# aurianer/DLA-Future

Measured on AMD Instinct MI355X. Metric: fp64 Cholesky TFlop/s, higher is better.
Workload: dtype f64

## Files before the change

### dla_future_amd/__init__.py

```python
from .capi import (DLAFDescriptor, LibraryNotBuilt, lib, lib_path, type_char, version)
from .cholesky import (DeviceMatrix, GeneralDeviceMatrix, Grid, cholesky_factorization, finalize, generalized_to_standard,
                       initialize, make_descriptor, potrf_trace, pxhegst, pxpotrf, pxpotrs, pxtrsm, set_random_hermitian_positive_definite, tile_gemm, tile_herk, tile_potrf,
                       tile_trsm, triangular_solver, triangular_solver_device, potrs_device, release_workspace_pool, solver_profile,
                       update_launch_stats)
from . import distribution
from .eigensolver import (band_to_tridiagonal, bt_band_to_tridiagonal, bt_reduction_to_band,
                          bt_reduction_to_band_device, eigensolver_min_band, eigensolver_profile, get_band_size, hermitian_eigensolver,
                          hermitian_generalized_eigensolver, red2band_panel_stats, red2band_profile, reduction_to_band,
                          reduction_to_band_device, tridiagonal_eigensolver)

__all__ = ["band_to_tridiagonal", "bt_band_to_tridiagonal", "eigensolver_profile", "hermitian_eigensolver",
           "hermitian_generalized_eigensolver", "tridiagonal_eigensolver", "bt_reduction_to_band", "bt_reduction_to_band_device", "get_band_size", "eigensolver_min_band", "red2band_profile",
           "reduction_to_band", "reduction_to_band_device", "DLAFDescriptor", "DeviceMatrix", "GeneralDeviceMatrix", "Grid", "LibraryNotBuilt", "cholesky_factorization", "distribution",
           "finalize", "generalized_to_standard", "initialize", "lib", "lib_path", "make_descriptor", "pxhegst", "pxpotrf", "pxpotrs", "pxtrsm",
           "set_random_hermitian_positive_definite", "solver_profile", "tile_gemm", "tile_herk", "tile_potrf", "tile_trsm",
           "triangular_solver", "triangular_solver_device", "potrs_device", "type_char", "version"]
```

### dla_future_amd/capi.py

```python
from __future__ import annotations

import ctypes as C
import os

import numpy as np

_HERE = os.path.dirname(os.path.abspath(__file__))


class LibraryNotBuilt(RuntimeError):
    pass


def lib_path() -> str:
    return os.environ.get("DLAF_MI355X_LIB") or os.path.join(_HERE, "lib", "libdlaf_mi355x.so")


class DLAFDescriptor(C.Structure):
    _fields_ = [("m", C.c_int), ("n", C.c_int), ("mb", C.c_int), ("nb", C.c_int), ("isrc", C.c_int),
                ("jsrc", C.c_int), ("i", C.c_int), ("j", C.c_int), ("ld", C.c_int)]


BCAST_FN = C.CFUNCTYPE(C.c_int, C.c_void_p, C.c_int, C.c_int, C.c_void_p, C.c_size_t)
BARRIER_FN = C.CFUNCTYPE(C.c_int, C.c_void_p)

_TYPE_CHARS = {np.dtype(np.float32): "s", np.dtype(np.float64): "d", np.dtype(np.complex64): "c",
               np.dtype(np.complex128): "z"}


def type_char(dtype) -> str:
    try:
        return _TYPE_CHARS[np.dtype(dtype)]
    except KeyError:
        raise TypeError(f"unsupported element type {dtype}: expected float32/64 or complex64/128") from None


_vp, _i, _l, _ch = C.c_void_p, C.c_int, C.c_long, C.c_char
_IP = C.POINTER(C.c_int)
SIGNATURES = {
    "dlaf_initialize": (None, [_i, C.POINTER(C.c_char_p), _i, C.POINTER(C.c_char_p)]),
    "dlaf_finalize": (None, []),
    "dlaf_free_grid": (None, [_i]),
    "make_dlaf_descriptor": (DLAFDescriptor, [_i, _i, _i, _i, _IP]),
    "dlaf_cholesky_factorization_s": (_i, [_i, _ch, _vp, DLAFDescriptor]),
    "dlaf_cholesky_factorization_d": (_i, [_i, _ch, _vp, DLAFDescriptor]),
    "dlaf_cholesky_factorization_c": (_i, [_i, _ch, _vp, DLAFDescriptor]),
    "dlaf_cholesky_factorization_z": (_i, [_i, _ch, _vp, DLAFDescriptor]),
    "dlaf_pspotrf": (None, [_ch, _i, _vp, _i, _i, _IP, _IP]),
    "dlaf_pdpotrf": (None, [_ch, _i, _vp, _i, _i, _IP, _IP]),
    "dlaf_pcpotrf": (None, [_ch, _i, _vp, _i, _i, _IP, _IP]),
    "dlaf_pzpotrf": (None, [_ch, _i, _vp, _i, _i, _IP, _IP]),
    "dlaf_mi355x_version": (C.c_char_p, []),
    "dlaf_mi355x_create_grid_single": (_i, []),
    "dlaf_mi355x_rccl_unique_id": (None, [_vp]),
    "dlaf_mi355x_create_grid_rccl": (_i, [_vp, _i, _i, _i, _i, _ch]),
    "dlaf_mi355x_create_grid_host": (_i, [_i, _i, _i, _i, _ch, BCAST_FN, BARRIER_FN, _vp]),
    "dlaf_mi355x_grid_host_bcast": (_i, [_i, _i, _i, _vp, C.c_size_t]),
    "dlaf_mi355x_grid_info": (_i, [_i, _IP, _IP, _IP, _IP]),
    "dlaf_mi355x_grid_barrier": (_i, [_i]),
    "dlaf_mi355x_grid_selftest": (_i, [_i, C.c_size_t]),
    "dlaf_mi355x_matrix_create": (_i, [_i, _ch, _ch, DLAFDescriptor, C.POINTER(_vp)]),
    "dlaf_mi355x_matrix_destroy": (None, [_vp]),
    "dlaf_mi355x_matrix_upload": (_i, [_vp, _vp, _i]),
    "dlaf_mi355x_matrix_download": (_i, [_vp, _vp, _i]),
    "dlaf_mi355x_matrix_copy": (_i, [_vp, _vp]),
    "dlaf_mi355x_matrix_fetch_tile": (_i, [_vp, _l, _l, _vp, _i]),
    "dlaf_mi355x_grid_on_free": (_i, [_i, _vp, _vp]),
    "dlaf_mi355x_grid_rekey": (_i, [_i, _i]),
    "dlaf_mi355x_grid_comm_log": (_i, [_i, _i]),
    "dlaf_mi355x_grid_comm_log_read": (_l, [_i, C.POINTER(C.c_long), _l]),
    "dlaf_mi355x_matrix_local_info": (_i, [_vp]),
    "dlaf_mi355x_potrf_trace": (_i, [C.POINTER(C.c_ulonglong)]),
    "dlaf_mi355x_update_launch_stats": (_i, [C.POINTER(C.c_long), C.POINTER(C.c_long)]),
    "dlaf_mi355x_cholesky_start": (_i, [_vp]),
    "dlaf_mi355x_cholesky_wait": (_i, [_vp]),
    "dlaf_mi355x_cholesky_factorization_device": (_i, [_vp]),
    "dlaf_mi355x_cholesky_residual": (_i, [_vp, _vp, C.POINTER(C.c_double), C.POINTER(C.c_double)]),
    "dlaf_mi355x_matrix_trsm_profile": (_i, [_vp, _i, C.POINTER(C.c_double), C.POINTER(C.c_double), C.POINTER(C.c_double)]),
    "dlaf_mi355x_matrix_profile": (_i, [_vp, _i, C.POINTER(C.c_double), C.POINTER(C.c_long),
                                        C.POINTER(C.c_double), C.POINTER(C.c_double)]),
    "dlaf_mi355x_triangular_solver_s": (_i, [_i, _ch, _ch, _ch, _ch, _vp, _vp, DLAFDescriptor, _vp, DLAFDescriptor]),
    "dlaf_mi355x_triangular_solver_d": (_i, [_i, _ch, _ch, _ch, _ch, _vp, _vp, DLAFDescriptor, _vp, DLAFDescriptor]),
    "dlaf_mi355x_triangular_solver_c": (_i, [_i, _ch, _ch, _ch, _ch, _vp, _vp, DLAFDescriptor, _vp, DLAFDescriptor]),
    "dlaf_mi355x_triangular_solver_z": (_i, [_i, _ch, _ch, _ch, _ch, _vp, _vp, DLAFDescriptor, _vp, DLAFDescriptor]),
    "dlaf_mi355x_pstrsm": (None, [_ch, _ch, _ch, _ch, _i, _i, _vp, _vp, _i, _i, _IP, _vp, _i, _i, _IP]),
    "dlaf_mi355x_pdtrsm": (None, [_ch, _ch, _ch, _ch, _i, _i, _vp, _vp, _i, _i, _IP, _vp, _i, _i, _IP]),
    "dlaf_mi355x_pctrsm": (None, [_ch, _ch, _ch, _ch, _i, _i, _vp, _vp, _i, _i, _IP, _vp, _i, _i, _IP]),
    "dlaf_mi355x_pztrsm": (None, [_ch, _ch, _ch, _ch, _i, _i, _vp, _vp, _i, _i, _IP, _vp, _i, _i, _IP]),
    "dlaf_mi355x_pspotrs": (None, [_ch, _i, _i, _vp, _i, _i, _IP, _vp, _i, _i, _IP, _IP]),
    "dlaf_mi355x_pdpotrs": (None, [_ch, _i, _i, _vp, _i, _i, _IP, _vp, _i, _i, _IP, _IP]),
    "dlaf_mi355x_pcpotrs": (None, [_ch, _i, _i, _vp, _i, _i, _IP, _vp, _i, _i, _IP, _IP]),
    "dlaf_mi355x_pzpotrs": (None, [_ch, _i, _i, _vp, _i, _i, _IP, _vp, _i, _i, _IP, _IP]),
    "dlaf_mi355x_solver_profile": (_i, [C.POINTER(C.c_double), C.POINTER(C.c_double)]),
    "dlaf_mi355x_gmatrix_create": (_i, [_i, _ch, DLAFDescriptor, C.POINTER(_vp)]),
    "dlaf_mi355x_gmatrix_destroy": (None, [_vp]),
    "dlaf_mi355x_gmatrix_upload": (_i, [_vp, _vp, _i]),
    "dlaf_mi355x_gmatrix_download": (_i, [_vp, _vp, _i]),
    "dlaf_mi355x_triangular_solver_device": (_i, [_ch, _ch, _ch, _ch, _vp, _vp, _vp]),
    "dlaf_mi355x_potrs_device": (_i, [_ch, _vp, _vp]),
    "dlaf_mi355x_generalized_to_standard_s": (_i, [_i, _ch, _vp, DLAFDescriptor, _vp, DLAFDescriptor]),
    "dlaf_mi355x_generalized_to_standard_d": (_i, [_i, _ch, _vp, DLAFDescriptor, _vp, DLAFDescriptor]),
    "dlaf_mi355x_generalized_to_standard_c": (_i, [_i, _ch, _vp, DLAFDescriptor, _vp, DLAFDescriptor]),
    "dlaf_mi355x_generalized_to_standard_z": (_i, [_i, _ch, _vp, DLAFDescriptor, _vp, DLAFDescriptor]),
    "dlaf_mi355x_pshegst": (None, [_i, _ch, _i, _vp, _i, _i, _IP, _vp, _i, _i, _IP, _vp, _IP]),
    "dlaf_mi355x_pdhegst": (None, [_i, _ch, _i, _vp, _i, _i, _IP, _vp, _i, _i, _IP, _vp, _IP]),
    "dlaf_mi355x_pchegst": (None, [_i, _ch, _i, _vp, _i, _i, _IP, _vp, _i, _i, _IP, _vp, _IP]),
    "dlaf_mi355x_pzhegst": (None, [_i, _ch, _i, _vp, _i, _i, _IP, _vp, _i, _i, _IP, _vp, _IP]),
    "dlaf_mi355x_generalized_to_standard_device": (_i, [_vp, _vp]),
    "dlaf_mi355x_reduction_to_band_s": (_i, [_i, _vp, DLAFDescriptor, _i, _vp]),
    "dlaf_mi355x_reduction_to_band_d": (_i, [_i, _vp, DLAFDescriptor, _i, _vp]),
    "dlaf_mi355x_reduction_to_band_c": (_i, [_i, _vp, DLAFDescriptor, _i, _vp]),
    "dlaf_mi355x_reduction_to_band_z": (_i, [_i, _vp, DLAFDescriptor, _i, _vp]),
    "dlaf_mi355x_reduction_to_band_device": (_i, [_vp, _i, _vp]),
    "dlaf_mi355x_bt_reduction_to_band_s": (_i, [_i, _i, _vp, DLAFDescriptor, _vp, DLAFDescriptor, _vp]),
    "dlaf_mi355x_bt_reduction_to_band_d": (_i, [_i, _i, _vp, DLAFDescriptor, _vp, DLAFDescriptor, _vp]),
    "dlaf_mi355x_bt_reduction_to_band_c": (_i, [_i, _i, _vp, DLAFDescriptor, _vp, DLAFDescriptor, _vp]),
    "dlaf_mi355x_bt_reduction_to_band_z": (_i, [_i, _i, _vp, DLAFDescriptor, _vp, DLAFDescriptor, _vp]),
    "dlaf_mi355x_bt_reduction_to_band_device": (_i, [_i, _vp, _vp, _vp]),
    "dlaf_mi355x_band_to_tridiagonal_s": (_i, [_i, _vp, DLAFDescriptor, _i, _vp, _vp, _vp, _i]),
    "dlaf_mi355x_bt_band_to_tridiagonal_s": (_i, [_i, _i, _i, _vp, _i, _vp, _i]),
    "dlaf_mi355x_band_to_tridiagonal_d": (_i, [_i, _vp, DLAFDescriptor, _i, _vp, _vp, _vp, _i]),
    "dlaf_mi355x_bt_band_to_tridiagonal_d": (_i, [_i, _i, _i, _vp, _i, _vp, _i]),
    "dlaf_mi355x_band_to_tridiagonal_c": (_i, [_i, _vp, DLAFDescriptor, _i, _vp, _vp, _vp, _i]),
    "dlaf_mi355x_bt_band_to_tridiagonal_c": (_i, [_i, _i, _i, _vp, _i, _vp, _i]),
    "dlaf_mi355x_band_to_tridiagonal_z": (_i, [_i, _vp, DLAFDescriptor, _i, _vp, _vp, _vp, _i]),
    "dlaf_mi355x_bt_band_to_tridiagonal_z": (_i, [_i, _i, _i, _vp, _i, _vp, _i]),
    "dlaf_symmetric_eigensolver_s": (_i, [_i, _ch, _vp, DLAFDescriptor, _vp, _vp, DLAFDescriptor]),
    "dlaf_symmetric_generalized_eigensolver_s": (_i, [_i, _ch, _vp, DLAFDescriptor, _vp, DLAFDescriptor, _vp, _vp, DLAFDescriptor]),
    "dlaf_symmetric_generalized_eigensolver_factorized_s": (_i, [_i, _ch, _vp, DLAFDescriptor, _vp, DLAFDescriptor, _vp, _vp, DLAFDescriptor]),
    "dlaf_symmetric_eigensolver_d": (_i, [_i, _ch, _vp, DLAFDescriptor, _vp, _vp, DLAFDescriptor]),
    "dlaf_symmetric_generalized_eigensolver_d": (_i, [_i, _ch, _vp, DLAFDescriptor, _vp, DLAFDescriptor, _vp, _vp, DLAFDescriptor]),
    "dlaf_symmetric_generalized_eigensolver_factorized_d": (_i, [_i, _ch, _vp, DLAFDescriptor, _vp, DLAFDescriptor, _vp, _vp, DLAFDescriptor]),
    "dlaf_hermitian_eigensolver_c": (_i, [_i, _ch, _vp, DLAFDescriptor, _vp, _vp, DLAFDescriptor]),
    "dlaf_hermitian_generalized_eigensolver_c": (_i, [_i, _ch, _vp, DLAFDescriptor, _vp, DLAFDescriptor, _vp, _vp, DLAFDescriptor]),
    "dlaf_hermitian_generalized_eigensolver_factorized_c": (_i, [_i, _ch, _vp, DLAFDescriptor, _vp, DLAFDescriptor, _vp, _vp, DLAFDescriptor]),
    "dlaf_hermitian_eigensolver_z": (_i, [_i, _ch, _vp, DLAFDescriptor, _vp, _vp, DLAFDescriptor]),
    "dlaf_hermitian_generalized_eigensolver_z": (_i, [_i, _ch, _vp, DLAFDescriptor, _vp, DLAFDescriptor, _vp, _vp, DLAFDescriptor]),
    "dlaf_hermitian_generalized_eigensolver_factorized_z": (_i, [_i, _ch, _vp, DLAFDescriptor, _vp, DLAFDescriptor, _vp, _vp, DLAFDescriptor]),
    "dlaf_pssyevd": (None, [_ch, _i, _vp, _i, _i, _IP, _vp, _vp, _i, _i, _IP, _IP]),
    "dlaf_pdsyevd": (None, [_ch, _i, _vp, _i, _i, _IP, _vp, _vp, _i, _i, _IP, _IP]),
    "dlaf_pcheevd": (None, [_ch, _i, _vp, _i, _i, _IP, _vp, _vp, _i, _i, _IP, _IP]),
    "dlaf_pzheevd": (None, [_ch, _i, _vp, _i, _i, _IP, _vp, _vp, _i, _i, _IP, _IP]),
    "dlaf_pssygvd": (None, [_ch, _i, _vp, _i, _i, _IP, _vp, _i, _i, _IP, _vp, _vp, _i, _i, _IP, _IP]),
    "dlaf_pssygvd_factorized": (None, [_ch, _i, _vp, _i, _i, _IP, _vp, _i, _i, _IP, _vp, _vp, _i, _i, _IP, _IP]),
    "dlaf_pdsygvd": (None, [_ch, _i, _vp, _i, _i, _IP, _vp, _i, _i, _IP, _vp, _vp, _i, _i, _IP, _IP]),
    "dlaf_pdsygvd_factorized": (None, [_ch, _i, _vp, _i, _i, _IP, _vp, _i, _i, _IP, _vp, _vp, _i, _i, _IP, _IP]),
    "dlaf_pchegvd": (None, [_ch, _i, _vp, _i, _i, _IP, _vp, _i, _i, _IP, _vp, _vp, _i, _i, _IP, _IP]),
    "dlaf_pchegvd_factorized": (None, [_ch, _i, _vp, _i, _i, _IP, _vp, _i, _i, _IP, _vp, _vp, _i, _i, _IP, _IP]),
    "dlaf_pzhegvd": (None, [_ch, _i, _vp, _i, _i, _IP, _vp, _i, _i, _IP, _vp, _vp, _i, _i, _IP, _IP]),
    "dlaf_pzhegvd_factorized": (None, [_ch, _i, _vp, _i, _i, _IP, _vp, _i, _i, _IP, _vp, _vp, _i, _i, _IP, _IP]),
    "dlaf_mi355x_tridiagonal_eigensolver_s": (_i, [_i, _i, _vp, _vp, _vp, _vp, _i]),
    "dlaf_mi355x_tridiagonal_eigensolver_d": (_i, [_i, _i, _vp, _vp, _vp, _vp, _i]),
    "dlaf_mi355x_eigensolver_profile": (_i, [C.POINTER(C.c_double)]),
    "dlaf_mi355x_get_band_size": (_i, [_i]),
    "dlaf_mi355x_red2band_panel_stats": (_i, [C.POINTER(C.c_long), C.POINTER(C.c_long)]),
    "dlaf_mi355x_workspace_pool_release": (C.c_long, []),
    "dlaf_mi355x_get_eigensolver_min_band": (_i, []),
    "dlaf_mi355x_set_eigensolver_min_band": (None, [_i]),
    "dlaf_mi355x_red2band_profile": (_i, [C.POINTER(C.c_double), C.POINTER(C.c_double)]),
    "dlaf_mi355x_set_random_hpd": (_i, [_i, _ch, _vp, DLAFDescriptor, _i]),
    "dlaf_mi355x_tile_potrf": (_i, [_ch, _ch, _i, _vp, _i]),
    "dlaf_mi355x_tile_trsm": (_i, [_ch, _ch, _i, _i, _vp, _i, _vp, _i]),
    "dlaf_mi355x_tile_herk": (_i, [_ch, _ch, _i, _i, _vp, _i, _vp, _i]),
    "dlaf_mi355x_tile_gemm": (_i, [_ch, _ch, _i, _i, _i, _vp, _i, _vp, _i, _vp, _i]),
    "dlaf_mi355x_dist_owner": (_i, [_l, _i, _i]),
    "dlaf_mi355x_dist_local_tile": (_l, [_l, _i, _i, _i]),
    "dlaf_mi355x_dist_next_local_tile": (_l, [_l, _i, _i, _i]),
    "dlaf_mi355x_dist_global_tile": (_l, [_l, _i, _i, _i]),
    "dlaf_mi355x_dist_local_size": (_l, [_l, _i, _i, _i, _i]),
    "dlaf_mi355x_dist_local_tiles": (_l, [_l, _i, _i, _i, _i]),
}

_lib = None


def lib() -> C.CDLL:
    global _lib
    if _lib is not None:
        return _lib
    if os.environ.get("DLAF_MI355X_NO_TORCH", "0") != "1":
        try:
            import torch
        except Exception:
            pass
    path = lib_path()
    if not os.path.exists(path):
        raise LibraryNotBuilt(f"{path} is missing: run `python -c 'import __graft_entry__ as g; g.build()'` "
                              "(hipcc --offload-arch=gfx950); dla_future_amd has no CPU fallback")
    L = C.CDLL(path, mode=C.RTLD_GLOBAL)
    for name, (res, args) in SIGNATURES.items():
        f = getattr(L, name)
        f.restype = res
        f.argtypes = args
    _lib = L
    return L


def version() -> str:
    return lib().dlaf_mi355x_version().decode()
```

### dla_future_amd/cholesky.py

```python
from __future__ import annotations

import ctypes as C

import numpy as np

from .capi import BARRIER_FN, BCAST_FN, DLAFDescriptor, lib, type_char


def initialize(print_config: bool = False) -> None:
    args = [b"dlaf"] + ([b"--dlaf:print-config"] if print_config else [])
    argv = (C.c_char_p * len(args))(*args)
    lib().dlaf_initialize(0, None, len(args), argv)


def finalize() -> None:
    lib().dlaf_finalize()


def make_descriptor(n: int, nb: int, ld: int, isrc: int = 0, jsrc: int = 0) -> DLAFDescriptor:
    return DLAFDescriptor(n, n, nb, nb, isrc, jsrc, 0, 0, max(1, ld))


def _ld_of(a: np.ndarray) -> int:
    if a.ndim != 2:
        raise ValueError("expected a 2-D array")
    if a.size and a.strides[0] != a.itemsize:
        raise ValueError("local matrices must be column-major (Fortran order)")
    return max(1, a.strides[1] // a.itemsize) if a.shape[1] > 1 else max(1, a.shape[0])


def _ptr(a):
    return a.ctypes.data_as(C.c_void_p) if a is not None and a.size else None


class Grid:

    def __init__(self, context: int, nranks: int, rank: int, keep=None):
        if context < 0:
            raise ValueError("grid creation failed (bad shape/rank?)")
        self.context = context
        self.nranks = nranks
        self.rank = rank
        self._keep = keep
        r = [C.c_int() for _ in range(4)]
        lib().dlaf_mi355x_grid_info(context, *(C.byref(x) for x in r))
        self.nprow, self.npcol, self.myrow, self.mycol = (x.value for x in r)

    @classmethod
    def single(cls) -> "Grid":
        return cls(lib().dlaf_mi355x_create_grid_single(), 1, 0)

    @classmethod
    def rccl(cls, unique_id: bytes, nranks: int, rank: int, nprow: int, npcol: int, order: str = "R") -> "Grid":
        buf = C.create_string_buffer(bytes(unique_id), 128)
        ctx = lib().dlaf_mi355x_create_grid_rccl(buf, nranks, rank, nprow, npcol, order.encode())
        return cls(ctx, nranks, rank)

    @staticmethod
    def rccl_unique_id() -> bytes:
        buf = C.create_string_buffer(128)
        lib().dlaf_mi355x_rccl_unique_id(buf)
        return buf.raw

    @classmethod
    def from_torch(cls, nprow: int, npcol: int, order: str = "R") -> "Grid":
        import torch.distributed as dist
        rank, world = dist.get_rank(), dist.get_world_size()
        if world == 1:
            return cls.single()
        box = [cls.rccl_unique_id() if rank == 0 else None]
        dist.broadcast_object_list(box, src=0)
        return cls.rccl(box[0], world, rank, nprow, npcol, order)

    @classmethod
    def host(cls, nranks: int, rank: int, nprow: int, npcol: int, order: str, bcast, barrier=None) -> "Grid":

        def _bcast(_user, axis, root, buf, nbytes):
            try:
                mv = (C.c_char * nbytes).from_address(buf)
                bcast(axis, root, memoryview(mv).cast("B"))
                return 0
            except Exception as e:
                print(f"[dla_future_amd] host broadcast failed: {e!r}")
                return 1

        def _barrier(_user):
            if barrier is not None:
                barrier()
            return 0

        cb, cbar = BCAST_FN(_bcast), BARRIER_FN(_barrier)
        ctx = lib().dlaf_mi355x_create_grid_host(nranks, rank, nprow, npcol, order.encode(), cb, cbar, None)
        return cls(ctx, nranks, rank, keep=(cb, cbar))

    def barrier(self) -> None:
        lib().dlaf_mi355x_grid_barrier(self.context)

    def selftest(self, nbytes: int = 1 << 20) -> int:
        return int(lib().dlaf_mi355x_grid_selftest(self.context, nbytes))

    def comm_log(self, enable: bool = True) -> None:
        lib().dlaf_mi355x_grid_comm_log(self.context, 1 if enable else 0)

    def comm_log_events(self):
        n = lib().dlaf_mi355x_grid_comm_log_read(self.context, None, 0)
        buf = (C.c_long * (4 * max(1, n)))()
        lib().dlaf_mi355x_grid_comm_log_read(self.context, buf, n)
        return [tuple(buf[4 * i:4 * i + 4]) for i in range(n)]

    def free(self) -> None:
        if self.context >= 0:
            lib().dlaf_free_grid(self.context)
            self.context = -1

    def local_shape(self, n: int, nb: int, isrc: int = 0, jsrc: int = 0):
        from . import distribution as d
        return (d.local_size(n, nb, self.nprow, self.myrow, isrc), d.local_size(n, nb, self.npcol, self.mycol, jsrc))


def cholesky_factorization(grid: Grid, uplo: str, a: np.ndarray, nb: int, isrc: int = 0, jsrc: int = 0,
                           n: int | None = None) -> int:
    t = type_char(a.dtype)
    if n is None:
        if grid.nranks != 1:
            raise ValueError("the global size n is required on a distributed grid")
        n = a.shape[0]
    desc = make_descriptor(n, nb, _ld_of(a), isrc, jsrc)
    fn = getattr(lib(), f"dlaf_cholesky_factorization_{t}")
    return fn(grid.context, uplo.encode(), _ptr(a), desc)


def pxpotrf(uplo: str, n: int, a: np.ndarray, ia: int, ja: int, desca) -> int:
    t = type_char(a.dtype)
    d = (C.c_int * 9)(*[int(x) for x in desca])
    info = C.c_int(-999)
    getattr(lib(), f"dlaf_p{t}potrf")(uplo.encode(), n, _ptr(a), ia, ja, d, C.byref(info))
    return info.value


def triangular_solver(grid: Grid, side: str, uplo: str, op: str, diag: str, alpha, a: np.ndarray, b: np.ndarray,
                      nb: int, m: int | None = None, n: int | None = None, a_src=(0, 0), b_src=(0, 0),
                      b_block: tuple[int, int] | None = None) -> None:
    t = type_char(b.dtype)
    if a.dtype != b.dtype:
        raise ValueError("A and B must have the same element type")
    if m is None or n is None:
        if grid.nranks != 1:
            raise ValueError("the global size m x n of B is required on a distributed grid")
        m, n = b.shape
    na = m if side.upper() == "L" else n
    da = DLAFDescriptor(na, na, nb, nb, a_src[0], a_src[1], 0, 0, _ld_of(a))
    mb_b, nb_b = b_block if b_block is not None else (nb, nb)
    db = DLAFDescriptor(m, n, mb_b, nb_b, b_src[0], b_src[1], 0, 0, _ld_of(b))
    al = np.array([alpha], dtype=b.dtype)
    fn = getattr(lib(), f"dlaf_mi355x_triangular_solver_{t}")
    r = fn(grid.context, side.encode(), uplo.encode(), op.encode(), diag.encode(), _ptr(al), _ptr(a), da, _ptr(b), db)
    if r != 0:
        raise ValueError(f"dlaf_mi355x_triangular_solver_{t} failed with {r}")


def pxpotrs(uplo: str, n: int, nrhs: int, a: np.ndarray, ia: int, ja: int, desca, b: np.ndarray, ib: int, jb: int,
            descb) -> int:
    t = type_char(b.dtype)
    da = (C.c_int * 9)(*[int(x) for x in desca])
    db = (C.c_int * 9)(*[int(x) for x in descb])
    info = C.c_int(-999)
    getattr(lib(), f"dlaf_mi355x_p{t}potrs")(uplo.encode(), n, nrhs, _ptr(a), ia, ja, da, _ptr(b), ib, jb, db,
                                             C.byref(info))
    return info.value


def generalized_to_standard(grid: Grid, uplo: str, a: np.ndarray, b: np.ndarray, nb: int, isrc: int = 0, jsrc: int = 0,
                            n: int | None = None) -> int:
    t = type_char(a.dtype)
    if a.dtype != b.dtype:
        raise ValueError("A and B must have the same element type")
    if n is None:
        if grid.nranks != 1:
            raise ValueError("the global size n is required on a distributed grid")
        n = a.shape[0]
    da = make_descriptor(n, nb, _ld_of(a), isrc, jsrc)
    db = make_descriptor(n, nb, _ld_of(b), isrc, jsrc)
    return getattr(lib(), f"dlaf_mi355x_generalized_to_standard_{t}")(grid.context, uplo.encode(), _ptr(a), da, _ptr(b), db)


def pxhegst(ibtype: int, uplo: str, n: int, a: np.ndarray, ia: int, ja: int, desca, b: np.ndarray, ib: int, jb: int,
            descb):
    t = type_char(a.dtype)
    da = (C.c_int * 9)(*[int(x) for x in desca])
    db = (C.c_int * 9)(*[int(x) for x in descb])
    scale = (C.c_float if t in "sc" else C.c_double)(-1)
    info = C.c_int(-999)
    getattr(lib(), f"dlaf_mi355x_p{t}hegst")(ibtype, uplo.encode(), n, _ptr(a), ia, ja, da, _ptr(b), ib, jb, db,
                                             C.byref(scale), C.byref(info))
    return scale.value, info.value


def solver_profile():
    ms, fl = C.c_double(0), C.c_double(0)
    lib().dlaf_mi355x_solver_profile(C.byref(ms), C.byref(fl))
    return ms.value, fl.value


def pxtrsm(side: str, uplo: str, op: str, diag: str, m: int, n: int, alpha, a: np.ndarray, ia: int, ja: int, desca,
           b: np.ndarray, ib: int, jb: int, descb) -> None:
    t = type_char(b.dtype)
    da = (C.c_int * 9)(*[int(x) for x in desca])
    db = (C.c_int * 9)(*[int(x) for x in descb])
    al = np.array([alpha], dtype=b.dtype)
    getattr(lib(), f"dlaf_mi355x_p{t}trsm")(side.encode(), uplo.encode(), op.encode(), diag.encode(), m, n, _ptr(al),
                                            _ptr(a), ia, ja, da, _ptr(b), ib, jb, db)


def set_random_hermitian_positive_definite(grid: Grid, a: np.ndarray, n: int, nb: int, isrc: int = 0,
                                           jsrc: int = 0, nthreads: int = 0) -> None:
    desc = make_descriptor(n, nb, _ld_of(a), isrc, jsrc)
    r = lib().dlaf_mi355x_set_random_hpd(grid.context, type_char(a.dtype).encode(), _ptr(a), desc, nthreads)
    if r != 0:
        raise ValueError(f"dlaf_mi355x_set_random_hpd failed with {r}")


def potrf_trace():
    out = (C.c_ulonglong * 32)()
    return list(out) if lib().dlaf_mi355x_potrf_trace(out) == 0 else None


def release_workspace_pool() -> int:
    return int(lib().dlaf_mi355x_workspace_pool_release())


def update_launch_stats():
    a, b = C.c_long(0), C.c_long(0)
    lib().dlaf_mi355x_update_launch_stats(C.byref(a), C.byref(b))
    return a.value, b.value


class DeviceMatrix:

    def __init__(self, grid: Grid, dtype, uplo: str, n: int, nb: int, isrc: int = 0, jsrc: int = 0):
        self.grid, self.dtype, self.uplo, self.n, self.nb = grid, np.dtype(dtype), uplo, n, nb
        self._h = C.c_void_p()
        desc = make_descriptor(n, nb, 1, isrc, jsrc)
        r = lib().dlaf_mi355x_matrix_create(grid.context, type_char(dtype).encode(), uplo.encode(), desc,
                                            C.byref(self._h))
        if r != 0:
            raise ValueError(f"dlaf_mi355x_matrix_create failed with {r}")

    def upload(self, a: np.ndarray) -> None:
        assert a.dtype == self.dtype
        lib().dlaf_mi355x_matrix_upload(self._h, _ptr(a), _ld_of(a))

    def download(self, a: np.ndarray) -> None:
        assert a.dtype == self.dtype
        lib().dlaf_mi355x_matrix_download(self._h, _ptr(a), _ld_of(a))

    def fetch_tile(self, gi: int, gj: int):
        rows = min(self.nb, self.n - gi * self.nb)
        cols = min(self.nb, self.n - gj * self.nb)
        out = np.zeros((rows, cols), dtype=self.dtype, order="F")
        r = lib().dlaf_mi355x_matrix_fetch_tile(self._h, gi, gj, _ptr(out), max(1, rows))
        if r < 0:
            raise ValueError(f"dlaf_mi355x_matrix_fetch_tile failed with {r}")
        return out if r == 0 else None

    def copy_from(self, other: "DeviceMatrix") -> None:
        r = lib().dlaf_mi355x_matrix_copy(self._h, other._h)
        if r != 0:
            raise ValueError("matrices are not conformable")

    def factorize(self) -> int:
        return lib().dlaf_mi355x_cholesky_factorization_device(self._h)

    def generalized_to_standard(self, factor_of_b: "DeviceMatrix") -> int:
        return lib().dlaf_mi355x_generalized_to_standard_device(self._h, factor_of_b._h)

    def start(self) -> None:
        lib().dlaf_mi355x_cholesky_start(self._h)

    def wait(self) -> int:
        return lib().dlaf_mi355x_cholesky_wait(self._h)

    def local_info(self) -> int:
        return lib().dlaf_mi355x_matrix_local_info(self._h)

    def residual_against(self, factor: "DeviceMatrix"):
        d, a = C.c_double(), C.c_double()
        r = lib().dlaf_mi355x_cholesky_residual(self._h, factor._h, C.byref(d), C.byref(a))
        if r != 0:
            raise ValueError("matrices are not conformable")
        return d.value, a.value

    PROFILE_KINDS = {"update_bulk": 0, "update_lookahead": 1, "trsm_panel": 2, "potrf_tile": 3}

    def profile(self, kind: str) -> dict:
        ms, n, fl, by = C.c_double(), C.c_long(), C.c_double(), C.c_double()
        lib().dlaf_mi355x_matrix_profile(self._h, self.PROFILE_KINDS[kind], C.byref(ms), C.byref(n), C.byref(fl),
                                         C.byref(by))
        return {"ms": ms.value, "launches": n.value, "flops": fl.value, "bytes": by.value}

    def trsm_profile(self, reps: int = 5) -> dict:
        ms, fl, by = C.c_double(), C.c_double(), C.c_double()
        lib().dlaf_mi355x_matrix_trsm_profile(self._h, reps, C.byref(ms), C.byref(fl), C.byref(by))
        return {"ms": ms.value, "flops": fl.value, "bytes": by.value}

    def close(self) -> None:
        if self._h:
            lib().dlaf_mi355x_matrix_destroy(self._h)
            self._h = C.c_void_p()

    def __del__(self):
        try:
            self.close()
        except Exception:
            pass


class GeneralDeviceMatrix:

    def __init__(self, grid: Grid, dtype, m: int, n: int, nb: int, isrc: int = 0, jsrc: int = 0):
        self.grid, self.dtype, self.m, self.n, self.nb = grid, np.dtype(dtype), m, n, nb
        self._h = C.c_void_p()
        desc = DLAFDescriptor(m, n, nb, nb, isrc, jsrc, 0, 0, 1)
        r = lib().dlaf_mi355x_gmatrix_create(grid.context, type_char(dtype).encode(), desc, C.byref(self._h))
        if r != 0:
            raise ValueError(f"dlaf_mi355x_gmatrix_create failed with {r}")

    def upload(self, a: np.ndarray) -> None:
        assert a.dtype == self.dtype
        lib().dlaf_mi355x_gmatrix_upload(self._h, _ptr(a), _ld_of(a))

    def download(self, a: np.ndarray) -> None:
        assert a.dtype == self.dtype
        lib().dlaf_mi355x_gmatrix_download(self._h, _ptr(a), _ld_of(a))

    def close(self) -> None:
        if self._h:
            lib().dlaf_mi355x_gmatrix_destroy(self._h)
            self._h = C.c_void_p()

    def __del__(self):
        try:
            self.close()
        except Exception:
            pass


def triangular_solver_device(side: str, uplo: str, op: str, diag: str, alpha, a: DeviceMatrix, b: GeneralDeviceMatrix) -> None:
    al = np.array([alpha], dtype=b.dtype)
    r = lib().dlaf_mi355x_triangular_solver_device(side.encode(), uplo.encode(), op.encode(), diag.encode(), _ptr(al),
                                                   a._h, b._h)
    if r != 0:
        raise ValueError(f"dlaf_mi355x_triangular_solver_device failed with {r}")


def potrs_device(uplo: str, factor: DeviceMatrix, b: GeneralDeviceMatrix) -> None:
    r = lib().dlaf_mi355x_potrs_device(uplo.encode(), factor._h, b._h)
    if r != 0:
        raise ValueError(f"dlaf_mi355x_potrs_device failed with {r}")


def tile_potrf(uplo: str, a: np.ndarray) -> int:
    return lib().dlaf_mi355x_tile_potrf(type_char(a.dtype).encode(), uplo.encode(), a.shape[0], _ptr(a), _ld_of(a))


def tile_trsm(uplo: str, a: np.ndarray, b: np.ndarray) -> None:
    m, n = b.shape
    lib().dlaf_mi355x_tile_trsm(type_char(b.dtype).encode(), uplo.encode(), m, n, _ptr(a), _ld_of(a), _ptr(b),
                                _ld_of(b))


def tile_herk(uplo: str, a: np.ndarray, c: np.ndarray) -> None:
    n = c.shape[0]
    k = a.shape[1] if uplo in "Ll" else a.shape[0]
    lib().dlaf_mi355x_tile_herk(type_char(c.dtype).encode(), uplo.encode(), n, k, _ptr(a), _ld_of(a), _ptr(c),
                                _ld_of(c))


def tile_gemm(uplo: str, a: np.ndarray, b: np.ndarray, c: np.ndarray) -> None:
    m, n = c.shape
    k = a.shape[1] if uplo in "Ll" else a.shape[0]
    lib().dlaf_mi355x_tile_gemm(type_char(c.dtype).encode(), uplo.encode(), m, n, k, _ptr(a), _ld_of(a), _ptr(b),
                                _ld_of(b), _ptr(c), _ld_of(c))
```

### dla_future_amd/csrc/device/device_api.hpp

```cpp
#pragma once
#include <hip/hip_runtime.h>

#include "common.hpp"

namespace dlaf_mi355x {

inline hipError_t zero_device_now(void* p, size_t bytes) {
  hipError_t e = hipMemsetAsync(p, 0, bytes, nullptr);
  if (e == hipSuccess)
    e = hipStreamSynchronize(nullptr);
  return e;
}


constexpr int kDiagBlock = 64;
constexpr int kInfoSchedulingFailure = -1000000;

template <class T>
struct UpdateArgs {
  T* c;
  long c_tsr, c_tsc;
  int ldc;
  const T* a;
  long a_ts;
  int lda;
  const T* b;
  long b_ts;
  int ldb;
  int il0, il1, jl0, jl1;
  int nb, K;
  int pr, ri, pc, ci;
  int nt, last_rows;
  const int* info;
  int rect = 0;
  int nt_c = 0, last_cols = 0;
  int b_period = 1;
  long b_ts2 = 0;
  int b_jl0 = -1;
  int K1 = 0;
  const T* a2 = nullptr;
  const T* b2 = nullptr;
  int her2k = 0;
};
template <class T>
void launch_update(const UpdateArgs<T>& args, hipStream_t stream, int role = 0, long max_blocks = 0,
                   unsigned* counters = nullptr, bool counters_are_zero = false, long excl_slots = 0);
template <class T>
int update_blocks_per_cu();

template <class T>
struct TrsmArgs {
  T* b;
  long b_ts;
  int ldb;
  int il0, il1;
  int pr, ri;
  int nb, nt, last_rows;
  const T* l;
  int ldl;
  const T* winv;
  int n;
  const int* info;
  int upper = 0;
  int prio = 0;
};
template <class T>
void launch_trsm(const TrsmArgs<T>& args, hipStream_t stream);

template <class T>
void launch_potrf_diag(T* a, int lda, int jb, T* winv_block, int* info, int info_base, hipStream_t stream,
                       bool factor = true, bool upper = false, bool unit = false);

template <class T>
void launch_invert_diag_blocks(const T* tile, int ld, int kb, T* winv, int* info, hipStream_t stream, bool upper,
                               bool unit);

template <class T>
void launch_potrf_coop(T* tile, int ld, int kb, T* winv, int* info, int info_base, unsigned* sync,
                       hipStream_t stream, bool sync_is_zero = false, bool count_strips = true);
void update_launch_stats(long* persistent, long* exclusive);
unsigned long long* potrf_coop_trace_buffer();
inline size_t potrf_coop_sync_words(int kb) {
  const size_t g = (size_t) ((kb + kDiagBlock - 1) / kDiagBlock);
  return g + g * g;
}

template <class T>
struct LayoutArgs {
  T* tiles;
  T* cm;
  long ld_cm;
  int ltr, ltc;
  int nb;
  long rows, cols;
  int pr, ri, pc, ci;
  int transpose;
  int full = 0, conj = 0, scale = 0;
  T alpha{};
  int jl_first = 0, jl_count = 0;
  int rev_rows = 0, rev_cols = 0;
};
template <class T>
void launch_to_tiles(const LayoutArgs<T>& args, hipStream_t stream);
template <class T>
void launch_from_tiles(const LayoutArgs<T>& args, hipStream_t stream);

template <class T>
void launch_copy2d(T* dst, long ldd, const T* src, long lds, int rows, int cols, int transpose, int mask,
                   hipStream_t stream);

template <class T>
void launch_tile_xform(T* dst, long ldd, long dstride, const T* src, long lds, long sstride, int rows, int cols,
                       int count, int mode, double scale, hipStream_t stream);

template <class T>
void launch_tile_xform_alpha(T* dst, long ldd, long dstride, const T* src, long lds, long sstride, int rows, int cols,
                             int count, int mode, T alpha, bool use_alpha, hipStream_t stream);

template <class T>
void launch_max_norm(const T* tiles, int ltr, int ltc, int nb, long rows, long cols, int pr, int ri, int pc, int ci,
                     double* out, hipStream_t stream);
template <class T>
void launch_zero_upper_diag(T* tiles, int ltr, int ltc, int nb, int pr, int ri, int pc, int ci, hipStream_t stream);

void device_kernels_init();

}
```

### dla_future_amd/csrc/device/kernels_update.hip

```cpp
#include <algorithm>
#include <cstdio>
#include <cstdlib>
#include <cstring>
#include <type_traits>
#include <utility>
#include <vector>

#include "device_api.hpp"
#include "mma_core.hpp"

namespace dlaf_mi355x {

template <class T>
struct UpdateCfg;
template <>
struct UpdateCfg<float> {
  using type = BlockCfg<float, 128, 128, 64, 64, 16>;
  static constexpr int min_waves = 2;
};
template <>
struct UpdateCfg<double> {
#if defined(DLAF_UPD_BIG)
  using type = BlockCfg<double, 256, 128, 64, 64, 16, true, DLAF_UPD_BIG, 512>;
  static constexpr int min_waves = 2;
#elif defined(DLAF_UPD_WIDE4)
  using type = BlockCfg<double, 256, 128, 128, 64, 16, true, DLAF_UPD_WIDE4, 256>;
  static constexpr int min_waves = 1;
#elif defined(DLAF_UPD_BK) && defined(DLAF_UPD_ST)
  using type = BlockCfg<double, 128, 128, 64, 64, DLAF_UPD_BK, true, DLAF_UPD_ST>;
  static constexpr int min_waves = 2;
#else
  using type = BlockCfg<double, 128, 128, 64, 64, 16, true, 2>;
  static constexpr int min_waves = 2;
#endif
};
template <>
struct UpdateCfg<cfloat> {
  using type = BlockCfg<cfloat, 128, 128, 64, 64, 16>;
  static constexpr int min_waves = 2;
};
template <>
struct UpdateCfg<cdouble> {
  using type = BlockCfg<cdouble, 128, 64, 64, 32, 8, true, 3>;
  static constexpr int min_waves = 2;
};

constexpr int kMaxPatchCols = 256;

struct UpdateMap {
  int ps;
  int psc;
  int PR;
  int tri;
  int PC;
  int colstart[kMaxPatchCols + 1];
  int xcd;
  int RB, CB;
  int bpt_m, bpt_n;
  long total;
  int persist;
  unsigned* counters;
  int lockstep;
  unsigned kphase_ticks;
  int excl_rank;
  unsigned excl_budget;
  int steal;
  int* cu_busy;
};

__device__ unsigned char g_cu_rank[8][256];

__global__ void cu_probe_kernel(unsigned* seen) {
  extern __shared__ unsigned char probe_lds[];
  if (threadIdx.x == 0) {
    unsigned xcc;
    const unsigned key = phys_cu_key(xcc);
    atomicOr(&seen[xcc * 8 + (key >> 5)], 1u << (key & 31));
    probe_lds[0] = (unsigned char) key;
  }
  for (int i = 0; i < 64; ++i)
    __builtin_amdgcn_s_sleep(64);
}

template <class T, bool VEC, bool UTAIL = false, int PART = 0>
__device__ __forceinline__ void update_block(const UpdateArgs<T>& p, const UpdateMap& mp, long w,
                                             real_t<T>* __restrict__ lds, int s0 = 0) {
  using Cfg = typename UpdateCfg<T>::type;
  using R = real_t<T>;

  const int ps = mp.ps, psc = mp.psc;
  const long patch = w >> (ps + psc);
  const int q = (int) (w & ((1 << (ps + psc)) - 1));
  int pi, pj;
  if (mp.tri) {
    int lo = 0, hi = mp.PC;
    while (hi - lo > 1) {
      const int mid = (lo + hi) >> 1;
      if (mp.colstart[mid] <= patch)
        lo = mid;
      else
        hi = mid;
    }
    pj = lo;
    const int cnt = mp.colstart[pj + 1] - mp.colstart[pj];
    pi = mp.PR - cnt + (int) (patch - mp.colstart[pj]);
  }
  else {
    pi = (int) (patch % mp.PR);
    pj = (int) (patch / mp.PR);
  }
  const int br = (pi << ps) + (q & ((1 << ps) - 1));
  const int bc = (pj << psc) + (q >> ps);
  if (br >= mp.RB || bc >= mp.CB)
    return;
  const int il = p.il0 + br / mp.bpt_m, sbr = br % mp.bpt_m;
  const int jl = p.jl0 + bc / mp.bpt_n, sbc = bc % mp.bpt_n;
  const int gi = il * p.pr + p.ri, gj = jl * p.pc + p.ci;
  if (!p.rect && gi < gj)
    return;
  const int rows_tile = (gi == p.nt - 1) ? p.last_rows : p.nb;
  const int cols_tile = p.rect ? ((gj == p.nt_c - 1) ? p.last_cols : p.nb) : ((gj == p.nt - 1) ? p.last_rows : p.nb);
  const int m0 = sbr * Cfg::BM, n0 = sbc * Cfg::BN;
  if (m0 >= rows_tile || n0 >= cols_tile)
    return;
  const bool diag = !p.rect && (gi == gj);
  const int mrows = min(Cfg::BM, rows_tile - m0), ncols = min(Cfg::BN, cols_tile - n0);
  if (diag && m0 + mrows - 1 < n0)
    return;

  const T* A = p.a + (long) (il - p.il0) * p.a_ts + m0;
  const int jt = jl - (p.b_jl0 >= 0 ? p.b_jl0 : p.jl0);
  const long boff = (long) (jt % p.b_period) * p.b_ts2 + (long) (jt / p.b_period) * p.b_ts;
  const long aoff = (long) (il - p.il0) * p.a_ts;
  const T* B;
  const T* B2 = nullptr;
  const long ldb = diag ? p.lda : p.ldb;
  if (!diag) {
    B = p.b + boff + n0;
    if (p.K1 > 0)
      B2 = p.b2 + boff + n0;
  }
  else if (!p.her2k) {
    B = p.a + aoff + n0;
    if (p.K1 > 0)
      B2 = p.a2 + aoff + n0;
  }
  else {
    B = p.a2 + aoff + n0;
    B2 = p.a + aoff + n0;
  }
  int K1 = 1 << 30;
  const T* A2 = nullptr;
  if (p.K1 > 0) {
    K1 = p.K1;
    A2 = p.a2 + aoff + m0 - (long) K1 * p.lda;
    B2 -= (long) K1 * ldb;
  }
#ifdef DLAF_DBG_STRIP_PACKED
  const long lda_x = Cfg::BM, ldb_x = Cfg::BN;
  A = p.a + aoff + (long) (m0 / Cfg::BM) * Cfg::BM * p.nb;
  B = (diag ? p.a + aoff : p.b + boff) + (long) (n0 / Cfg::BN) * Cfg::BN * p.nb;
#define DLAF_LDA_X lda_x
#define DLAF_LDB_X ldb_x
#else
#define DLAF_LDA_X p.lda
#define DLAF_LDB_X ldb
#endif
#ifdef DLAF_DBG_SAME_STRIPS
  A = p.a;
  B = p.b;
#endif
  T* C = p.c + (long) il * p.c_tsr + (long) jl * p.c_tsc + m0 + (long) n0 * p.ldc;

  auto uniform = [](const T* q) {
    const unsigned long long v = reinterpret_cast<unsigned long long>(q);
    const unsigned lo = (unsigned) __builtin_amdgcn_readfirstlane((int) (unsigned) v);
    const unsigned hi = (unsigned) __builtin_amdgcn_readfirstlane((int) (unsigned) (v >> 32));
    return reinterpret_cast<const T*>(((unsigned long long) hi << 32) | lo);
  };
#if DLAF_GLDS_SCALAR_ADDR
  A = uniform(A);
  B = uniform(B);
  A2 = uniform(A2);
  B2 = uniform(B2);
#endif
  const bool full = (mrows == Cfg::BM) && (ncols == Cfg::BN) && (p.K % Cfg::BK == 0) && (p.K1 % Cfg::BK == 0);
  if constexpr (PART != 0) {
    const bool interior = full && !(diag && m0 < n0 + ncols - 1) && VEC && ((p.ldc * (long) sizeof(T)) % 16 == 0) &&
                          (reinterpret_cast<uintptr_t>(C) % 16 == 0);
    if ((PART == 1) != interior)
      return;
  }
  Acc<Cfg> acc;
#ifndef DLAF_UPD_PRELOAD
#define DLAF_UPD_PRELOAD 1
#endif
  if constexpr (DLAF_UPD_PRELOAD && Cfg::PAIRED && !Cfg::CX && sizeof(R) == 8 && VEC && !UTAIL) {
    const bool unmasked = full && !(diag && m0 < n0 + ncols - 1);
    if (unmasked && ((p.ldc * (long) sizeof(T)) % 16 == 0) && (reinterpret_cast<uintptr_t>(C) % 16 == 0)) {
      typedef R r2 __attribute__((ext_vector_type(2)));
      const int lane_ = threadIdx.x & 63, wave_ = __builtin_amdgcn_readfirstlane(threadIdx.x >> 6);
      const int wm_ = wave_ % Cfg::WAVES_M, wn_ = wave_ / Cfg::WAVES_M;
      const int g_ = lane_ >> 4, c_ = lane_ & 15;
      const unsigned lane_off = (unsigned) sizeof(T) * (unsigned) (2 * c_ + 2 * g_ * (int) p.ldc);
      T* Cw = C + wm_ * Cfg::WM + (long) (wn_ * Cfg::WN) * p.ldc;
      auto at = [](T* base, unsigned byte_off) {
        return reinterpret_cast<r2*>(reinterpret_cast<char*>(base) + byte_off);
      };
      static_assert(Cfg::TN % 2 == 0, "paired accumulator columns");
#pragma unroll
      for (int j = 0; j < Cfg::TN; ++j)
#pragma unroll
        for (int v = 0; v < 4; ++v) {
          T* col = Cw + (long) ((j >> 1) * 32 + 8 * v + (j & 1)) * p.ldc;
#pragma unroll
          for (int q = 0; q < Cfg::TM / 2; ++q) {
            const r2 cv = *at(col + q * 32, lane_off);
            acc.re[2 * q][j][v] = cv[0];
            acc.re[2 * q + 1][j][v] = cv[1];
          }
        }
      gemm_nt_block<Cfg, T, VEC, false, UTAIL, true>(A, DLAF_LDA_X, mrows, B, DLAF_LDB_X, ncols, p.K, lds, acc, K1, A2,
                                                     B2);
#pragma unroll
      for (int j = 0; j < Cfg::TN; ++j)
#pragma unroll
        for (int v = 0; v < 4; ++v) {
          T* col = Cw + (long) ((j >> 1) * 32 + 8 * v + (j & 1)) * p.ldc;
#pragma unroll
          for (int q = 0; q < Cfg::TM / 2; ++q)
            *at(col + q * 32, lane_off) = r2{acc.re[2 * q][j][v], acc.re[2 * q + 1][j][v]};
        }
      return;
    }
  }
  acc.clear();
  if constexpr (PART == 1) {
    gemm_nt_block<Cfg, T, VEC, false, UTAIL>(A, DLAF_LDA_X, mrows, B, DLAF_LDB_X, ncols, p.K, lds, acc, K1, A2, B2,
                                             s0);
  }
  else {
    if (full)
      gemm_nt_block<Cfg, T, VEC, false, UTAIL>(A, DLAF_LDA_X, mrows, B, DLAF_LDB_X, ncols, p.K, lds, acc, K1, A2, B2,
                                               s0);
    else
      gemm_nt_block<Cfg, T, false, true>(A, p.lda, mrows, B, ldb, ncols, p.K, lds, acc, K1, A2, B2);
  }

#ifdef DLAF_DBG_SKIP_EPILOGUE
  {
    R sum = 0;
    for (int i = 0; i < Cfg::TM; ++i)
      for (int j = 0; j < Cfg::TN; ++j)
        for (int v = 0; v < 4; ++v)
          sum += acc.re[i][j][v];
    if (sum == R(12345.678))
      C[0] = make_el<T>(sum, 0);
    return;
  }
#endif
  const int lane = threadIdx.x & 63, wave = threadIdx.x >> 6;
  const int wm = wave % Cfg::WAVES_M, wn = wave / Cfg::WAVES_M;
  const int g = lane >> 4, c = lane & 15;
  const bool masked = PART == 1 ? false : (!full || (diag && m0 < n0 + ncols - 1));
  if constexpr (Cfg::PAIRED) {
    typedef R r2 __attribute__((ext_vector_type(2)));
    const bool wide = PART == 1 ? true
                                : (!masked && VEC && ((p.ldc * (long) sizeof(T)) % 16 == 0) &&
                                   (reinterpret_cast<uintptr_t>(C) % 16 == 0));
#ifndef DLAF_EPI_COLS
#define DLAF_EPI_COLS 4
#endif
    if (wide) {
      constexpr int NB = DLAF_EPI_COLS;
#pragma unroll
      for (int i0 = 0; i0 < Cfg::TN * 4; i0 += NB) {
        r2 cv[NB][Cfg::TM / 2];
#pragma unroll
        for (int ii = 0; ii < NB; ++ii) {
          const int j = (i0 + ii) / 4, v = (i0 + ii) % 4;
          const T* col = C + (long) (wn * Cfg::WN + acc_n<Cfg>(j, g, v)) * p.ldc;
#pragma unroll
          for (int q = 0; q < Cfg::TM / 2; ++q)
            cv[ii][q] = *reinterpret_cast<const r2*>(col + wm * Cfg::WM + q * 32 + 2 * c);
        }
#pragma unroll
        for (int ii = 0; ii < NB; ++ii) {
          const int j = (i0 + ii) / 4, v = (i0 + ii) % 4;
          T* col = C + (long) (wn * Cfg::WN + acc_n<Cfg>(j, g, v)) * p.ldc;
#pragma unroll
          for (int q = 0; q < Cfg::TM / 2; ++q) {
            cv[ii][q][0] -= acc.re[2 * q][j][v];
            cv[ii][q][1] -= acc.re[2 * q + 1][j][v];
            *reinterpret_cast<r2*>(col + wm * Cfg::WM + q * 32 + 2 * c) = cv[ii][q];
          }
        }
      }
    }
    else {
#pragma unroll
      for (int j = 0; j < Cfg::TN; ++j) {
#pragma unroll
        for (int v = 0; v < 4; ++v) {
          const int nl = wn * Cfg::WN + acc_n<Cfg>(j, g, v);
          T* col = C + (long) nl * p.ldc;
#pragma unroll
          for (int i = 0; i < Cfg::TM; ++i) {
            const int ml = wm * Cfg::WM + acc_m<Cfg>(i, c);
            if (!masked || (ml < mrows && nl < ncols && (!diag || (m0 + ml) >= (n0 + nl))))
              col[ml] = col[ml] - acc.re[i][j][v];
          }
        }
      }
    }
  }
  else if (!masked) {
#pragma unroll
    for (int j = 0; j < Cfg::TN; ++j) {
      T cv[4][Cfg::TM];
#pragma unroll
      for (int v = 0; v < 4; ++v) {
        const T* col = C + (long) (wn * Cfg::WN + acc_n<Cfg>(j, g, v)) * p.ldc;
#pragma unroll
        for (int i = 0; i < Cfg::TM; ++i)
          cv[v][i] = col[wm * Cfg::WM + acc_m<Cfg>(i, c)];
      }
#pragma unroll
      for (int v = 0; v < 4; ++v) {
        T* col = C + (long) (wn * Cfg::WN + acc_n<Cfg>(j, g, v)) * p.ldc;
#pragma unroll
        for (int i = 0; i < Cfg::TM; ++i) {
          if constexpr (Cfg::CX)
            col[wm * Cfg::WM + acc_m<Cfg>(i, c)] = T{cv[v][i].re - acc.re[i][j][v], cv[v][i].im - acc.im[i][j][v]};
          else
            col[wm * Cfg::WM + acc_m<Cfg>(i, c)] = cv[v][i] - acc.re[i][j][v];
        }
      }
    }
  }
  else {
#pragma unroll
    for (int j = 0; j < Cfg::TN; ++j) {
#pragma unroll
      for (int v = 0; v < 4; ++v) {
        const int nl = wn * Cfg::WN + acc_n<Cfg>(j, g, v);
        T* col = C + (long) nl * p.ldc;
#pragma unroll
        for (int i = 0; i < Cfg::TM; ++i) {
          const int ml = wm * Cfg::WM + acc_m<Cfg>(i, c);
          if (ml < mrows && nl < ncols && (!diag || (m0 + ml) >= (n0 + nl))) {
            const T cv = col[ml];
            if constexpr (Cfg::CX) {
              T r{cv.re - acc.re[i][j][v], cv.im - acc.im[i][j][v]};
              if (diag && (m0 + ml) == (n0 + nl))
                r.im = R(0);
              col[ml] = r;
            }
            else {
              col[ml] = cv - acc.re[i][j][v];
            }
          }
        }
      }
    }
  }
}

template <class T, bool VEC, int ROLE>
__global__ __launch_bounds__(UpdateCfg<T>::type::THREADS, UpdateCfg<T>::min_waves) void update_kernel(UpdateArgs<T> p,
                                                                                                     UpdateMap mp) {
  using R = real_t<T>;
  extern __shared__ __attribute__((aligned(16))) unsigned char lds_raw[];
  R* lds = reinterpret_cast<R*>(lds_raw);
  if (*p.info != 0)
    return;
  if (!mp.persist) {
    const long v = blockIdx.x;
    const long w = mp.xcd ? (v & 7) * (mp.total >> 3) + (v >> 3) : v;
#ifdef DLAF_UPD_LEAN
    update_block<T, VEC, false, (ROLE == 0 ? 1 : 0)>(p, mp, w, lds);
#else
    update_block<T, VEC>(p, mp, w, lds);
#endif
    return;
  }
  __shared__ unsigned next_item;
  const int nq = mp.xcd ? 8 : 1;
  const long per_q = mp.total / nq;
  const int q0 = mp.xcd ? (int) (blockIdx.x & 7) : 0;
  const unsigned W = gridDim.x / nq;
  if (mp.excl_rank > 0) {
    __shared__ int leave;
    if (threadIdx.x == 0) {
      unsigned xcc;
      const unsigned key = phys_cu_key(xcc);
      leave = 0;
      if ((int) g_cu_rank[xcc][key] < mp.excl_rank)
        leave = atomicAdd(&mp.counters[15], 1u) < mp.excl_budget ? 1 : 0;
    }
    __syncthreads();
    if (leave)
      return;
  }
  __shared__ int next_s0;
  const int nslab = p.K / UpdateCfg<T>::type::BK;
  int q = q0, tried = 1;
  int* my_busy = nullptr;
  if (mp.cu_busy != nullptr && threadIdx.x == 0) {
    unsigned xcc;
    const unsigned key = phys_cu_key(xcc);
    my_busy = mp.cu_busy + (xcc * 256u + key);
  }
  for (;;) {
    if (threadIdx.x == 0) {
      if (my_busy != nullptr) {
        int spins = 0;
        while (__hip_atomic_load(my_busy, __ATOMIC_RELAXED, __HIP_MEMORY_SCOPE_AGENT) > 0 && ++spins < 4000)
          __builtin_amdgcn_s_sleep(64);
      }
      next_item = atomicAdd(&mp.counters[q], 1u);
      next_s0 = (mp.kphase_ticks != 0 && nslab > 1) ? (int) ((wall_clock64() / mp.kphase_ticks) % (unsigned) nslab) : 0;
    }
    __syncthreads();
#if DLAF_GLDS_SCALAR_ADDR
    const long i = (long) (unsigned) __builtin_amdgcn_readfirstlane((int) next_item);
    const int s0 = __builtin_amdgcn_readfirstlane(next_s0);
#else
    const long i = next_item;
    const int s0 = next_s0;
#endif
    __syncthreads();
    if (i >= per_q) {
      if (!mp.steal || tried >= nq)
        break;
      ++tried;
      q = (q + 1) % nq;
      continue;
    }
    if (mp.lockstep) {
      if (threadIdx.x == 0) {
        const unsigned need = (unsigned) (i / W) * W;
        long spins = 0;
        while (__hip_atomic_load(&mp.counters[8 + q], __ATOMIC_RELAXED, __HIP_MEMORY_SCOPE_AGENT) < need && ++spins < 2000000)
          __builtin_amdgcn_s_sleep(8);
      }
      __syncthreads();
    }
#ifdef DLAF_UPD_LEAN
    update_block<T, VEC, ROLE == 0, (ROLE == 0 ? 1 : 0)>(p, mp, (long) q * per_q + i, lds, s0);
#else
    update_block<T, VEC, ROLE == 0>(p, mp, (long) q * per_q + i, lds, s0);
#endif
    if (mp.lockstep && threadIdx.x == 0)
      __hip_atomic_fetch_add(&mp.counters[8 + q], 1u, __ATOMIC_RELAXED, __HIP_MEMORY_SCOPE_AGENT);
  }
}

static bool update_lockstep() {
  static const bool on = [] {
    const char* e = std::getenv("DLAF_MI355X_LOCKSTEP");
    return e ? std::atoi(e) != 0 : false;
  }();
  return on;
}

template <class T>
static unsigned kphase_ticks(int resident) {
  using Cfg = typename UpdateCfg<T>::type;
  static const double rate = [] {
    const char* on = std::getenv("DLAF_MI355X_KPHASE");
    if (on == nullptr || std::atoi(on) == 0)
      return 0.0;
    if (const char* e = std::getenv("DLAF_MI355X_KPHASE_RATE"))
      return std::atof(e) * 1e12;
    return (sizeof(real_t<T>) == 8 ? 66.5e12 : 120e12);
  }();
  static const double khz = [] {
    int dev = 0, v = 0;
    (void) hipGetDevice(&dev);
    if (hipDeviceGetAttribute(&v, hipDeviceAttributeWallClockRate, dev) != hipSuccess || v <= 0)
      v = 100000;
    return (double) v;
  }();
  if (rate <= 0 || resident <= 0)
    return 0;
  const double flops = (TypeInfo<T>::is_complex ? 8.0 : 2.0) * Cfg::BM * Cfg::BN * Cfg::BK;
  const double seconds = flops / (rate / resident);
  const double ticks = seconds * khz * 1e3;
  return ticks < 1 ? 1u : (unsigned) (ticks + 0.5);
}

template <class T>
static bool aligned16(const void* ptr, long stride_elems) {
  return (reinterpret_cast<uintptr_t>(ptr) % 16 == 0) && ((stride_elems * (long) sizeof(T)) % 16 == 0);
}

static int* g_cu_busy = nullptr;
int* cu_busy_table() {
  static const bool on = [] {
    const char* e = std::getenv("DLAF_MI355X_POTRF_YIELD");
    return e ? std::atoi(e) != 0 : true;
  }();
  if (on && g_cu_busy == nullptr) {
    if (hipMalloc(reinterpret_cast<void**>(&g_cu_busy), 8 * 256 * sizeof(int)) != hipSuccess ||
        zero_device_now(g_cu_busy, 8 * 256 * sizeof(int)) != hipSuccess) {
      (void) hipGetLastError();
      g_cu_busy = nullptr;
    }
  }
  return g_cu_busy;
}

static int g_probe_xcds = 0, g_probe_cus_per_xcd = 0, g_probe_engines = 1;

static long g_launch_stats[2] = {0, 0};
void update_launch_stats(long* persistent, long* exclusive) {
  *persistent = g_launch_stats[0];
  *exclusive = g_launch_stats[1];
}

static bool update_steal() {
  static const bool on = [] {
    const char* e = std::getenv("DLAF_MI355X_STEAL");
    return e ? std::atoi(e) != 0 : true;
  }();
  return on;
}

template <class T>
void launch_update(const UpdateArgs<T>& a, hipStream_t stream, int role, long max_blocks, unsigned* counters,
                   bool counters_are_zero, long excl_slots) {
  using Cfg = typename UpdateCfg<T>::type;
  if (a.il1 <= a.il0 || a.jl1 <= a.jl0 || a.K <= 0 || a.nb <= 0)
    return;
  UpdateMap mp;
  mp.bpt_m = (a.nb + Cfg::BM - 1) / Cfg::BM;
  mp.bpt_n = (a.nb + Cfg::BN - 1) / Cfg::BN;
  mp.RB = (a.il1 - a.il0) * mp.bpt_m;
  mp.CB = (a.jl1 - a.jl0) * mp.bpt_n;
  static_assert(Cfg::BM % Cfg::BN == 0 && ((Cfg::BM / Cfg::BN) & (Cfg::BM / Cfg::BN - 1)) == 0, "BM = 2^s * BN");
  constexpr int kAspectShift = (Cfg::BM / Cfg::BN == 1) ? 0 : (Cfg::BM / Cfg::BN == 2) ? 1 : 2;
  const bool big = (mp.RB >= 16 && mp.CB >= 16);
  mp.ps = big ? 3 : 0;
  mp.psc = big ? 3 + kAspectShift : 0;
  mp.PR = (mp.RB + (1 << mp.ps) - 1) >> mp.ps;
  mp.PC = (mp.CB + (1 << mp.psc) - 1) >> mp.psc;
  long npatch = (long) mp.PR * mp.PC;
  mp.tri = 0;
  if (mp.PC <= kMaxPatchCols) {
    mp.tri = 1;
    mp.colstart[0] = 0;
    for (int pj = 0; pj < mp.PC; ++pj) {
      const int jl_min = a.jl0 + (pj << mp.psc) / mp.bpt_n;
      const long gj_min = (long) jl_min * a.pc + a.ci;
      long il_first = (gj_min - a.ri + a.pr - 1) / a.pr;
      if (gj_min <= a.ri || a.rect)
        il_first = 0;
      if (il_first < a.il0)
        il_first = a.il0;
      int cnt = 0;
      if (il_first < a.il1) {
        const int pi0 = (int) (((il_first - a.il0) * mp.bpt_m) >> mp.ps);
        cnt = mp.PR - pi0;
      }
      mp.colstart[pj + 1] = mp.colstart[pj] + cnt;
    }
    npatch = mp.colstart[mp.PC];
    if (npatch == 0)
      return;
  }
  mp.total = npatch << (mp.ps + mp.psc);
  mp.xcd = (mp.ps > 0) ? 1 : 0;
  long grid = mp.total;
  mp.persist = 0;
  mp.lockstep = 0;
  mp.kphase_ticks = 0;
  mp.counters = nullptr;
  mp.excl_rank = 0;
  mp.excl_budget = 0;
  mp.steal = 0;
  long excl_rank = 0;
  if (excl_slots > 0) {
    static const int per_cu = update_blocks_per_cu<T>();
    const long round = (long) per_cu * g_probe_xcds * g_probe_engines;
    if (g_probe_xcds > 0 && !update_lockstep() && excl_slots % round == 0 &&
        (excl_slots / round) * g_probe_engines <= g_probe_cus_per_xcd / 2)
      excl_rank = (excl_slots / round) * g_probe_engines;
    else {
      max_blocks = std::max<long>(8, max_blocks - excl_slots);
      excl_slots = 0;
    }
  }
  if (max_blocks > 0 && counters != nullptr && mp.total > max_blocks) {
    grid = mp.xcd ? (max_blocks / 8) * 8 : max_blocks;
    if (grid < 8)
      grid = 8;
    mp.persist = 1;
    mp.counters = counters;
    mp.lockstep = update_lockstep() ? 1 : 0;
    mp.kphase_ticks = kphase_ticks<T>((int) (grid));
    mp.steal = (update_steal() && !mp.lockstep) ? 1 : 0;
    mp.cu_busy = (role == 0) ? g_cu_busy : nullptr;
    ++g_launch_stats[0];
    if (excl_rank > 0) {
      mp.excl_rank = (int) excl_rank;
      mp.excl_budget = (unsigned) excl_slots;
      ++g_launch_stats[1];
    }
    if (!counters_are_zero)
      (void) hipMemsetAsync(counters, 0, 16 * sizeof(unsigned), stream);
  }
  const bool vec = aligned16<T>(a.a, a.lda) && aligned16<T>(a.a, a.a_ts) && aligned16<T>(a.b, a.ldb) &&
                   aligned16<T>(a.b, a.b_ts) && aligned16<T>(a.b, a.b_ts2) &&
                   (a.K1 == 0 || (aligned16<T>(a.a2, 0) && aligned16<T>(a.b2, 0)));
  auto go = [&](auto vtag, auto rtag) {
    constexpr bool V = decltype(vtag)::value;
    constexpr int RL = decltype(rtag)::value;
    hipLaunchKernelGGL((update_kernel<T, V, RL>), dim3((unsigned) grid), dim3(Cfg::THREADS), Cfg::LDS_BYTES, stream, a, mp);
  };
  auto by_role = [&](auto vtag) {
    switch (role) {
      case 0: go(vtag, std::integral_constant<int, 0>{}); break;
      case 1: go(vtag, std::integral_constant<int, 1>{}); break;
      case 3: go(vtag, std::integral_constant<int, 3>{}); break;
      default: go(vtag, std::integral_constant<int, 2>{}); break;
    }
  };
  if (vec)
    by_role(std::true_type{});
  else
    by_role(std::false_type{});
}

template <class T>
int update_blocks_per_cu() {
  using Cfg = typename UpdateCfg<T>::type;
  int n = 0;
  if (hipOccupancyMaxActiveBlocksPerMultiprocessor(&n, reinterpret_cast<const void*>(&update_kernel<T, true, 0>), Cfg::THREADS,
                                                   Cfg::LDS_BYTES) != hipSuccess || n < 1)
    n = 1;
  return n;
}

template <class T>
static void update_init_one() {
  using Cfg = typename UpdateCfg<T>::type;
#define SET_ONE(V, RL)                                                                         \
  (void) hipFuncSetAttribute(reinterpret_cast<const void*>(&update_kernel<T, V, RL>),           \
                             hipFuncAttributeMaxDynamicSharedMemorySize, Cfg::LDS_BYTES)
  SET_ONE(true, 0);
  SET_ONE(true, 1);
  SET_ONE(true, 2);
  SET_ONE(true, 3);
  SET_ONE(false, 0);
  SET_ONE(false, 1);
  SET_ONE(false, 2);
  SET_ONE(false, 3);
#undef SET_ONE
}

static void probe_compute_units() {
  const bool verbose = [] {
    const char* e = std::getenv("DLAF_MI355X_PROBE_VERBOSE");
    return e && std::atoi(e) != 0;
  }();
  auto note = [&](const char* what, hipError_t err) {
    if (verbose)
      std::fprintf(stderr, "[dlaf_mi355x] compute-unit probe: %s: %s\n", what, hipGetErrorString(err));
    (void) hipGetLastError();
  };
  unsigned* seen = nullptr;
  hipError_t err = hipMalloc(reinterpret_cast<void**>(&seen), 64 * sizeof(unsigned));
  if (err != hipSuccess)
    return note("hipMalloc", err);
  unsigned h[64] = {};
  err = hipMemset(seen, 0, sizeof(h));
  if (err == hipSuccess) {
    hipLaunchKernelGGL(cu_probe_kernel, dim3(8192), dim3(64), 48 * 1024, nullptr, seen);
    err = hipGetLastError();
  }
  if (err == hipSuccess)
    err = hipMemcpy(h, seen, sizeof(h), hipMemcpyDeviceToHost);
  (void) hipFree(seen);
  if (err != hipSuccess)
    return note("probe launch", err);
  static unsigned char rank[8][256];
  std::memset(rank, 255, sizeof(rank));
  int xcds = 0, min_cus = 1 << 30, max_engines = 0;
  for (int x = 0; x < 8; ++x) {
    std::vector<unsigned> keys;
    for (unsigned key = 0; key < 256; ++key)
      if (h[x * 8 + (key >> 5)] >> (key & 31) & 1u)
        keys.push_back(key);
    if (keys.empty())
      continue;
    ++xcds;
    min_cus = std::min<int>(min_cus, (int) keys.size());
    std::vector<unsigned> ord(keys.size());
    int engines = 0;
    for (size_t i = 0; i < keys.size(); ++i) {
      unsigned n = 0;
      bool first = true;
      for (size_t j = 0; j < keys.size(); ++j)
        if ((keys[j] >> 4) == (keys[i] >> 4)) {
          if ((keys[j] & 15u) < (keys[i] & 15u))
            ++n;
          if (j < i)
            first = false;
        }
      ord[i] = n;
      engines += first ? 1 : 0;
    }
    std::vector<size_t> idx(keys.size());
    for (size_t i = 0; i < idx.size(); ++i)
      idx[i] = i;
    std::sort(idx.begin(), idx.end(), [&](size_t a, size_t b) {
      return std::make_pair(ord[a], keys[a] >> 4) < std::make_pair(ord[b], keys[b] >> 4);
    });
    for (size_t r = 0; r < idx.size(); ++r)
      rank[x][keys[idx[r]]] = (unsigned char) std::min<size_t>(r, 254);
    max_engines = std::max(max_engines, engines);
    {
      std::vector<unsigned> sorted(keys.size());
      for (size_t r = 0; r < idx.size(); ++r)
        sorted[r] = keys[idx[r]];
      keys.swap(sorted);
    }
    if (verbose) {
      std::fprintf(stderr, "[dlaf_mi355x] compute-unit probe: XCD %d: %zu compute units:", x, keys.size());
      for (unsigned k : keys)
        std::fprintf(stderr, " %u.%u.%u", k >> 5, (k >> 4) & 1u, k & 15u);
      std::fprintf(stderr, "\n");
    }
  }
  if (xcds == 0)
    return note("no compute unit seen", hipSuccess);
  err = hipMemcpyToSymbol(HIP_SYMBOL(g_cu_rank), rank, sizeof(rank));
  if (err != hipSuccess)
    return note("hipMemcpyToSymbol", err);
  g_probe_xcds = xcds;
  g_probe_cus_per_xcd = min_cus;
  g_probe_engines = std::max(1, max_engines);
}

void update_kernels_init() {
  update_init_one<float>();
  update_init_one<double>();
  update_init_one<cfloat>();
  update_init_one<cdouble>();
  probe_compute_units();
  (void) cu_busy_table();
}

template void launch_update<float>(const UpdateArgs<float>&, hipStream_t, int, long, unsigned*, bool, long);
template int update_blocks_per_cu<float>();
template void launch_update<double>(const UpdateArgs<double>&, hipStream_t, int, long, unsigned*, bool, long);
template int update_blocks_per_cu<double>();
template void launch_update<cfloat>(const UpdateArgs<cfloat>&, hipStream_t, int, long, unsigned*, bool, long);
template int update_blocks_per_cu<cfloat>();
template void launch_update<cdouble>(const UpdateArgs<cdouble>&, hipStream_t, int, long, unsigned*, bool, long);
template int update_blocks_per_cu<cdouble>();

}
```

### dla_future_amd/csrc/host/c_api.cpp

```cpp
#define DLAF_MI355X_NO_MPI 1
#include <dlfcn.h>

#include <climits>
#include <complex>
#include <cstdio>
#include <cstdlib>
#include <cstring>
#include <memory>
#include <string>
#include <unordered_map>

#include <dlaf_c/eigensolver/eigensolver.h>
#include <dlaf_c/eigensolver/gen_eigensolver.h>
#include <dlaf_c/factorization/cholesky.h>
#include <dlaf_c/grid.h>
#include <dlaf_c/init.h>
#include <dlaf_mi355x/dlaf_mi355x.h>

#include "eigensolver.hpp"
#include "red2band.hpp"
#include "runtime.hpp"
#include "tile_matrix.hpp"

using namespace dlaf_mi355x;
// ... 573 lines not shown
    return -1;
  Grid& g = *it->second;
  if (!g.host_bcast)
    return g.nranks == 1 ? 0 : -2;
  return g.host_bcast(g.host_user, axis, root, host_buf, bytes);
}

#define DLAF_MI355X_TRSM_ENTRY(S, HT, CT)                                                                        \
  int dlaf_mi355x_triangular_solver_##S(int ctx, char side, char uplo, char op, char diag, const CT* alpha,      \
                                        const CT* a, DLAF_descriptor desca, CT* b, DLAF_descriptor descb) noexcept { \
    return triangular_solver_c<HT>(ctx, side, uplo, op, diag, reinterpret_cast<const HT*>(alpha),               \
                                   reinterpret_cast<const HT*>(a), desca, reinterpret_cast<HT*>(b), descb);     \
  }                                                                                                             \
  void dlaf_mi355x_p##S##trsm(char side, char uplo, char op, char diag, int m, int n, const CT* alpha, const CT* a, \
                              int ia, int ja, const int desca[9], CT* b, int ib, int jb, const int descb[9]) noexcept { \
    pxtrsm<HT>(side, uplo, op, diag, m, n, reinterpret_cast<const HT*>(alpha), reinterpret_cast<const HT*>(a), ia, \
               ja, desca, reinterpret_cast<HT*>(b), ib, jb, descb);                                              \
  }
#define DLAF_MI355X_POTRS_ENTRY(S, HT, CT)                                                                       \
  void dlaf_mi355x_p##S##potrs(char uplo, int n, int nrhs, const CT* a, int ia, int ja, const int desca[9], CT* b,  \
                               int ib, int jb, const int descb[9], int* info) noexcept {                        \
    pxpotrs<HT>(uplo, n, nrhs, reinterpret_cast<const HT*>(a), ia, ja, desca, reinterpret_cast<HT*>(b), ib, jb,  \
                descb, info);                                                                                   \
  }
DLAF_MI355X_POTRS_ENTRY(s, float, float)
DLAF_MI355X_POTRS_ENTRY(d, double, double)
DLAF_MI355X_POTRS_ENTRY(c, std::complex<float>, dlaf_complex_c)
DLAF_MI355X_POTRS_ENTRY(z, std::complex<double>, dlaf_complex_z)
#undef DLAF_MI355X_POTRS_ENTRY
DLAF_MI355X_TRSM_ENTRY(s, float, float)
DLAF_MI355X_TRSM_ENTRY(d, double, double)
DLAF_MI355X_TRSM_ENTRY(c, std::complex<float>, dlaf_complex_c)
DLAF_MI355X_TRSM_ENTRY(z, std::complex<double>, dlaf_complex_z)
#undef DLAF_MI355X_TRSM_ENTRY

#define DLAF_MI355X_HEGST_ENTRY(S, HT, CT, RT)                                                                    \
  int dlaf_mi355x_generalized_to_standard_##S(int ctx, char uplo, CT* a, DLAF_descriptor desca, const CT* b,       \
                                              DLAF_descriptor descb) noexcept {                                  \
    return gen_to_std_c<HT>(ctx, uplo, reinterpret_cast<HT*>(a), desca, reinterpret_cast<const HT*>(b), descb);    \
  }                                                                                                              \
  void dlaf_mi355x_p##S##hegst(int ibtype, char uplo, int n, CT* a, int ia, int ja, const int desca[9], const CT* b, \
                               int ib, int jb, const int descb[9], RT* scale, int* info) noexcept {               \
    pxhegst<HT, RT>(ibtype, uplo, n, reinterpret_cast<HT*>(a), ia, ja, desca, reinterpret_cast<const HT*>(b), ib, \
                    jb, descb, scale, info);                                                                     \
  }
DLAF_MI355X_HEGST_ENTRY(s, float, float, float)
DLAF_MI355X_HEGST_ENTRY(d, double, double, double)
DLAF_MI355X_HEGST_ENTRY(c, std::complex<float>, dlaf_complex_c, float)
DLAF_MI355X_HEGST_ENTRY(z, std::complex<double>, dlaf_complex_z, double)
#undef DLAF_MI355X_HEGST_ENTRY

#define DLAF_MI355X_R2B_ENTRY(S, HT, CT)                                                                          \
  int dlaf_mi355x_reduction_to_band_##S(int ctx, CT* a, DLAF_descriptor desca, int band, CT* taus) noexcept {     \
    return red2band_c<HT>(ctx, reinterpret_cast<HT*>(a), desca, band, reinterpret_cast<HT*>(taus));               \
  }                                                                                                              \
  int dlaf_mi355x_bt_reduction_to_band_##S(int ctx, int band, CT* c, DLAF_descriptor descc, const CT* v,          \
                                           DLAF_descriptor descv, const CT* taus) noexcept {                     \
    return bt_red2band_c<HT>(ctx, band, reinterpret_cast<HT*>(c), descc, reinterpret_cast<const HT*>(v), descv,   \
                             reinterpret_cast<const HT*>(taus));                                                 \
  }
DLAF_MI355X_R2B_ENTRY(s, float, float)
DLAF_MI355X_R2B_ENTRY(d, double, double)
DLAF_MI355X_R2B_ENTRY(c, std::complex<float>, dlaf_complex_c)
DLAF_MI355X_R2B_ENTRY(z, std::complex<double>, dlaf_complex_z)
#undef DLAF_MI355X_R2B_ENTRY


#define DLAF_MI355X_EIG_ENTRY(S, KIND, HT, CT, RT, PEV, PGV)                                                          \
  int dlaf_mi355x_band_to_tridiagonal_##S(int ctx, const CT* a, DLAF_descriptor desca, int band, RT* d, RT* e, CT* v, \
                                          int ldv) noexcept {                                                       \
    return band_to_tridiag_c<HT>(ctx, reinterpret_cast<const HT*>(a), desca, band, d, e, reinterpret_cast<HT*>(v), ldv); \
  }                                                                                                                  \
  int dlaf_mi355x_bt_band_to_tridiagonal_##S(int band, int n, int ncols, const CT* v, int ldv, CT* e, int lde) noexcept { \
    using DT = typename DevType<HT>::type;                                                                           \
    runtime_init();                                                                                                  \
    if (band < 2 || ldv < std::max(1, n) || lde < std::max(1, n))                                                    \
      fatal("[dlaf_mi355x] bt_band_to_tridiagonal: bad band_size / leading dimensions\n");                           \
    return bt_band_to_tridiag_host<DT>(n, band, reinterpret_cast<const DT*>(v), ldv, reinterpret_cast<DT*>(e), lde,   \
                                       ncols);                                                                       \
  }                                                                                                                  \
  int dlaf_##KIND##_eigensolver_##S(const int ctx, const char uplo, CT* a, const DLAF_descriptor desca, RT* w, CT* z, \
                                    const DLAF_descriptor descz) noexcept {                                          \
    return eigensolver_c<HT>(ctx, uplo, reinterpret_cast<HT*>(a), desca, w, reinterpret_cast<HT*>(z), descz);        \
  }                                                                                                                  \
  int dlaf_##KIND##_generalized_eigensolver_##S(const int ctx, const char uplo, CT* a, const DLAF_descriptor desca,   \
                                                CT* b, const DLAF_descriptor descb, RT* w, CT* z,                    \
                                                const DLAF_descriptor descz) noexcept {                              \
    return gen_eigensolver_c<HT>(ctx, uplo, reinterpret_cast<HT*>(a), desca, reinterpret_cast<HT*>(b), descb, w,      \
                                 reinterpret_cast<HT*>(z), descz, false);                                            \
  }                                                                                                                  \
  int dlaf_##KIND##_generalized_eigensolver_factorized_##S(const int ctx, const char uplo, CT* a,                     \
                                                           const DLAF_descriptor desca, CT* b,                       \
                                                           const DLAF_descriptor descb, RT* w, CT* z,                \
                                                           const DLAF_descriptor descz) noexcept {                   \
    return gen_eigensolver_c<HT>(ctx, uplo, reinterpret_cast<HT*>(a), desca, reinterpret_cast<HT*>(b), descb, w,      \
                                 reinterpret_cast<HT*>(z), descz, true);                                             \
  }                                                                                                                  \
  void dlaf_##PEV(const char uplo, const int n, CT* a, const int ia, const int ja, const int desca[9], RT* w, CT* z,  \
                  const int iz, const int jz, const int descz[9], int* info) noexcept {                              \
    pxheevd<HT>(uplo, n, reinterpret_cast<HT*>(a), ia, ja, desca, w, reinterpret_cast<HT*>(z), iz, jz, descz, info);  \
  }                                                                                                                  \
  void dlaf_##PGV(const char uplo, const int n, CT* a, const int ia, const int ja, const int desca[9], CT* b,         \
                  const int ib, const int jb, const int descb[9], RT* w, CT* z, const int iz, const int jz,          \
                  const int descz[9], int* info) noexcept {                                                          \
    pxhegvd<HT>(uplo, n, reinterpret_cast<HT*>(a), ia, ja, desca, reinterpret_cast<HT*>(b), ib, jb, descb, w,         \
                reinterpret_cast<HT*>(z), iz, jz, descz, info, false);                                               \
  }                                                                                                                  \
  void dlaf_##PGV##_factorized(const char uplo, const int n, CT* a, const int ia, const int ja, const int desca[9],   \
                               CT* b, const int ib, const int jb, const int descb[9], RT* w, CT* z, const int iz,    \
                               const int jz, const int descz[9], int* info) noexcept {                               \
    pxhegvd<HT>(uplo, n, reinterpret_cast<HT*>(a), ia, ja, desca, reinterpret_cast<HT*>(b), ib, jb, descb, w,         \
                reinterpret_cast<HT*>(z), iz, jz, descz, info, true);                                                \
  }
DLAF_MI355X_EIG_ENTRY(s, symmetric, float, float, float, pssyevd, pssygvd)
DLAF_MI355X_EIG_ENTRY(d, symmetric, double, double, double, pdsyevd, pdsygvd)
DLAF_MI355X_EIG_ENTRY(c, hermitian, std::complex<float>, dlaf_complex_c, float, pcheevd, pchegvd)
DLAF_MI355X_EIG_ENTRY(z, hermitian, std::complex<double>, dlaf_complex_z, double, pzheevd, pzhegvd)
#undef DLAF_MI355X_EIG_ENTRY

int dlaf_mi355x_tridiagonal_eigensolver_s(int n, int nb, const float* d, const float* e, float* w, float* z,
                                          int ldz) noexcept {
  runtime_init();
  return tridiag_solver_host<float>(n, nb, d, e, w, z, ldz);
}
int dlaf_mi355x_tridiagonal_eigensolver_d(int n, int nb, const double* d, const double* e, double* w, double* z,
                                          int ldz) noexcept {
  runtime_init();
  return tridiag_solver_host<double>(n, nb, d, e, w, z, ldz);
}
int dlaf_mi355x_eigensolver_profile(double ms[5]) noexcept {
  eigensolver_last_profile(ms);
  return 0;
}

int dlaf_mi355x_red2band_panel_stats(long* blocked, long* fallback) noexcept {
  red2band_last_panels(blocked, fallback);
  return 0;
}
long dlaf_mi355x_workspace_pool_release(void) noexcept {
  const long held = (long) pool_idle_bytes();
  pool_release();
  return held;
}
int dlaf_mi355x_get_eigensolver_min_band(void) noexcept {
  return eigensolver_min_band();
}
void dlaf_mi355x_set_eigensolver_min_band(int b_min) noexcept {
  set_eigensolver_min_band(b_min);
}
int dlaf_mi355x_get_band_size(int nb) noexcept {
  return get_band_size(nb);
}
int dlaf_mi355x_red2band_profile(double* ms, double* flops) noexcept {
  red2band_last_profile(ms, flops);
  return 0;
}

struct dlaf_mi355x_gmatrix_s {
  std::unique_ptr<MatrixBase> m;
  int ctx;
};

int dlaf_mi355x_gmatrix_create(int ctx, char type, DLAF_descriptor d, dlaf_mi355x_gmatrix_t* out) noexcept {
  if (!out)
    return -1;
  auto it = g_grids.find(ctx);
  if (it == g_grids.end())
    return -1;
  Grid* g = it->second.get();
  if (d.i != 0 || d.j != 0 || d.m < 0 || d.n < 0 || d.mb != d.nb || d.nb < 1)
    return -3;
  if (d.isrc < 0 || d.isrc >= g->nprow || d.jsrc < 0 || d.jsrc >= g->npcol)
    return -3;
  MatrixBase* m = general_matrix_create(g, type, d.m, d.n, d.nb, d.isrc, d.jsrc);
  if (!m)
    return -2;
  auto* h = new dlaf_mi355x_gmatrix_s;
  h->m.reset(m);
  h->ctx = ctx;
  *out = h;
  return 0;
}
void dlaf_mi355x_gmatrix_destroy(dlaf_mi355x_gmatrix_t h) noexcept {
  delete h;
}
int dlaf_mi355x_gmatrix_upload(dlaf_mi355x_gmatrix_t h, const void* host, int ld) noexcept {
  if (!h || !h->m)
    return -1;
  general_matrix_transfer(h->m.get(), const_cast<void*>(host), ld, true);
  return 0;
}
int dlaf_mi355x_gmatrix_download(dlaf_mi355x_gmatrix_t h, void* host, int ld) noexcept {
  if (!h || !h->m)
    return -1;
  general_matrix_transfer(h->m.get(), host, ld, false);
  return 0;
}
int dlaf_mi355x_triangular_solver_device(char side, char uplo, char op, char diag, const void* alpha,
                                         dlaf_mi355x_matrix_t a, dlaf_mi355x_gmatrix_t b) noexcept {
  if (!a || !a->m || !b || !b->m || a->ctx != b->ctx)
    return -1;
  auto is = [](char c, const char* set) { return c != 0 && std::strchr(set, c) != nullptr; };
  if (!is(side, "LlRr") || !is(uplo, "LlUu") || !is(op, "NnTtCc") || !is(diag, "NnUu"))
    fatal("[dlaf_mi355x] triangular solver: bad side/uplo/op/diag '%c' '%c' '%c' '%c'\n", side, uplo, op, diag);
  return triangular_solver_device(side, uplo, op, diag, alpha, a->m.get(), b->m.get());
}
int dlaf_mi355x_potrs_device(char uplo, dlaf_mi355x_matrix_t factor, dlaf_mi355x_gmatrix_t b) noexcept {
  if (!factor || !factor->m || !b || !b->m)
    return -1;
  const bool lower = (uplo == 'L' || uplo == 'l');
  const double one_d[2] = {1.0, 0.0};
  const float one_f[2] = {1.0f, 0.0f};
  const void* one = (factor->type == 's' || factor->type == 'c') ? (const void*) one_f : (const void*) one_d;
  int r = dlaf_mi355x_triangular_solver_device('L', uplo, lower ? 'N' : 'C', 'N', one, factor, b);
  if (r != 0)
    return r;
  return dlaf_mi355x_triangular_solver_device('L', uplo, lower ? 'C' : 'N', 'N', one, factor, b);
}

int dlaf_mi355x_solver_profile(double* ms, double* flops) noexcept {
  solver_last_profile(ms, flops);
  return 0;
}

int dlaf_mi355x_matrix_create(int ctx, char type, char uplo, DLAF_descriptor d, dlaf_mi355x_matrix_t* out) noexcept {
  if (!out)
    return -1;
  auto it = g_grids.find(ctx);
  if (it == g_grids.end())
    return -1;
  Grid* g = it->second.get();
  if (d.i != 0 || d.j != 0 || d.m != d.n || d.mb != d.nb || d.nb < 1 || d.m < 0)
    return -3;
  if (d.isrc < 0 || d.isrc >= g->nprow || d.jsrc < 0 || d.jsrc >= g->npcol)
    return -3;
  if (!(uplo == 'L' || uplo == 'l' || uplo == 'U' || uplo == 'u'))
    return -4;
  auto* h = new dlaf_mi355x_matrix_s;
  h->type = type;
  h->ctx = ctx;
  const int r = dispatch_type(type, [&](auto* tag) {
    using DT = std::remove_pointer_t<decltype(tag)>;
    auto m = std::make_unique<DeviceMatrix<DT>>();
    m->create(g, uplo, d.m, d.nb, d.isrc, d.jsrc);
    h->m = std::move(m);
    return 0;
  });
  if (r != 0) {
    delete h;
    return r;
  }
  *out = h;
  return 0;
}

void dlaf_mi355x_matrix_destroy(dlaf_mi355x_matrix_t m) noexcept {
  delete m;
}

#define WITH_MATRIX(handle, body)                                       \
  if (!(handle) || !(handle)->m)                                        \
    return -1;                                                          \
  return dispatch_type((handle)->type, [&](auto* tag) -> int {         \
    using DT = std::remove_pointer_t<decltype(tag)>;                    \
    auto& M = static_cast<DeviceMatrix<DT>&>(*(handle)->m);             \
    body                                                                \
  });

int dlaf_mi355x_matrix_upload(dlaf_mi355x_matrix_t h, const void* host, int ld) noexcept {
  WITH_MATRIX(h, M.upload(static_cast<const DT*>(host), ld); return 0;)
}
int dlaf_mi355x_matrix_download(dlaf_mi355x_matrix_t h, void* host, int ld) noexcept {
  WITH_MATRIX(h, M.download(static_cast<DT*>(host), ld); return 0;)
}
int dlaf_mi355x_matrix_copy(dlaf_mi355x_matrix_t dst, dlaf_mi355x_matrix_t src) noexcept {
  if (!src || !dst || src->type != dst->type)
    return -1;
  WITH_MATRIX(dst, M.copy_from(static_cast<DeviceMatrix<DT>&>(*src->m)); return 0;)
}
int dlaf_mi355x_matrix_fetch_tile(dlaf_mi355x_matrix_t h, long gi, long gj, void* host, int ld) noexcept {
  WITH_MATRIX(h, return M.fetch_tile(gi, gj, static_cast<DT*>(host), ld) ? 0 : 1;)
}
int dlaf_mi355x_cholesky_start(dlaf_mi355x_matrix_t h) noexcept {
  WITH_MATRIX(h, M.factorize_async(); return 0;)
}
int dlaf_mi355x_cholesky_wait(dlaf_mi355x_matrix_t h) noexcept {
  WITH_MATRIX(h, return M.wait();)
}
int dlaf_mi355x_cholesky_factorization_device(dlaf_mi355x_matrix_t h) noexcept {
  WITH_MATRIX(h, return M.factorize();)
}
int dlaf_mi355x_matrix_local_info(dlaf_mi355x_matrix_t h) noexcept {
  WITH_MATRIX(h, return M.local_info;)
}
int dlaf_mi355x_update_launch_stats(long* persistent, long* exclusive) noexcept {
  long a = 0, b = 0;
  update_launch_stats(&a, &b);
  if (persistent)
    *persistent = a;
  if (exclusive)
    *exclusive = b;
  return 0;
}
int dlaf_mi355x_potrf_trace(unsigned long long* out) noexcept {
  unsigned long long* tb = potrf_coop_trace_buffer();
  if (tb == nullptr || out == nullptr)
    return 1;
  (void) hipDeviceSynchronize();
  return hipMemcpy(out, tb, 32 * sizeof(unsigned long long), hipMemcpyDeviceToHost) == hipSuccess ? 0 : -1;
}

int dlaf_mi355x_cholesky_residual(dlaf_mi355x_matrix_t original, dlaf_mi355x_matrix_t factor, double* max_diff,
                                  double* max_a) noexcept {
  if (!original || !factor || original->type != factor->type)
    return -1;
  WITH_MATRIX(original, M.residual_of(static_cast<DeviceMatrix<DT>&>(*factor->m), max_diff, max_a); return 0;)
}

int dlaf_mi355x_generalized_to_standard_device(dlaf_mi355x_matrix_t a, dlaf_mi355x_matrix_t l) noexcept {
  if (!a || !l || a->type != l->type)
    return -1;
  WITH_MATRIX(a, return gen_to_std_device(M, static_cast<DeviceMatrix<DT>&>(*l->m));)
}

int dlaf_mi355x_reduction_to_band_device(dlaf_mi355x_matrix_t a, int band, void* taus) noexcept {
  WITH_MATRIX(a, return reduction_to_band_device(M, band, static_cast<DT*>(taus));)
}
int dlaf_mi355x_bt_reduction_to_band_device(int band, dlaf_mi355x_gmatrix_t c, dlaf_mi355x_matrix_t v,
                                            const void* taus) noexcept {
  if (!c || !c->m || !v || !v->m || c->m->type != v->type)
    return -1;
  WITH_MATRIX(v, return bt_reduction_to_band_device(band, static_cast<GeneralMatrix<DT>&>(*c->m).m, M,
                                                    static_cast<const DT*>(taus));)
}

int dlaf_mi355x_matrix_trsm_profile(dlaf_mi355x_matrix_t h, int reps, double* ms, double* flops, double* bytes) noexcept {
  WITH_MATRIX(h, const double t = M.trsm_profile(reps, flops, bytes); if (ms) *ms = t; return 0;)
}

int dlaf_mi355x_matrix_profile(dlaf_mi355x_matrix_t h, int kind, double* ms, long* launches, double* flops,
                               double* bytes) noexcept {
  if (kind < 0 || kind > 3)
    return -2;
  WITH_MATRIX(h, const auto& p = M.prof[kind]; if (ms) *ms = p.ms; if (launches) *launches = p.launches;
              if (flops) *flops = p.flops; if (bytes) *bytes = p.bytes; return 0;)
}

int dlaf_mi355x_set_random_hpd(int ctx, char type, void* host, DLAF_descriptor d, int nthreads) noexcept {
  auto it = g_grids.find(ctx);
  if (it == g_grids.end())
    return -1;
  const Grid& g = *it->second;
  if (d.m != d.n || d.mb != d.nb || d.nb < 1)
    return -3;
  Axis rows{d.m, d.nb, g.nprow, g.myrow, d.isrc}, cols{d.n, d.nb, g.npcol, g.mycol, d.jsrc};
  switch (type) {
    case 's': set_random_hpd_local(static_cast<float*>(host), d.ld, d.m, d.nb, rows, cols, nthreads); break;
    case 'd': set_random_hpd_local(static_cast<double*>(host), d.ld, d.m, d.nb, rows, cols, nthreads); break;
    case 'c': set_random_hpd_local(static_cast<std::complex<float>*>(host), d.ld, d.m, d.nb, rows, cols, nthreads); break;
    case 'z': set_random_hpd_local(static_cast<std::complex<double>*>(host), d.ld, d.m, d.nb, rows, cols, nthreads); break;
    default: return -2;
  }
  return 0;
}

int dlaf_mi355x_tile_potrf(char type, char uplo, int n, void* a, int lda) noexcept {
  return dispatch_type(type, [&](auto* tag) {
    using DT = std::remove_pointer_t<decltype(tag)>;
    return tile_potrf<DT>(uplo, n, static_cast<DT*>(a), lda);
  });
}
int dlaf_mi355x_tile_trsm(char type, char uplo, int m, int n, const void* a, int lda, void* b, int ldb) noexcept {
  return dispatch_type(type, [&](auto* tag) {
    using DT = std::remove_pointer_t<decltype(tag)>;
    tile_trsm<DT>(uplo, m, n, static_cast<const DT*>(a), lda, static_cast<DT*>(b), ldb);
    return 0;
  });
}
int dlaf_mi355x_tile_herk(char type, char uplo, int n, int k, const void* a, int lda, void* c, int ldc) noexcept {
  return dispatch_type(type, [&](auto* tag) {
    using DT = std::remove_pointer_t<decltype(tag)>;
    tile_herk<DT>(uplo, n, k, static_cast<const DT*>(a), lda, static_cast<DT*>(c), ldc);
    return 0;
  });
}
int dlaf_mi355x_tile_gemm(char type, char uplo, int m, int n, int k, const void* a, int lda, const void* b, int ldb,
                          void* c, int ldc) noexcept {
  return dispatch_type(type, [&](auto* tag) {
    using DT = std::remove_pointer_t<decltype(tag)>;
    tile_gemm<DT>(uplo, m, n, k, static_cast<const DT*>(a), lda, static_cast<const DT*>(b), ldb, static_cast<DT*>(c), ldc);
    return 0;
  });
}

int dlaf_mi355x_dist_owner(long gt, int gs, int src) noexcept {
  return Axis{0, 1, gs, 0, src}.owner(gt);
}
long dlaf_mi355x_dist_local_tile(long gt, int gs, int rank, int src) noexcept {
  return Axis{0, 1, gs, rank, src}.local_of(gt);
}
long dlaf_mi355x_dist_next_local_tile(long gt, int gs, int rank, int src) noexcept {
  return Axis{0, 1, gs, rank, src}.next_local(gt);
}
long dlaf_mi355x_dist_global_tile(long lt, int gs, int rank, int src) noexcept {
  return Axis{0, 1, gs, rank, src}.global_of(lt);
}
long dlaf_mi355x_dist_local_size(long n, int nb, int gs, int rank, int src) noexcept {
  return Axis{n, nb, gs, rank, src}.local_size();
}
long dlaf_mi355x_dist_local_tiles(long n, int nb, int gs, int rank, int src) noexcept {
  return Axis{n, nb, gs, rank, src}.local_tiles();
}


int dlaf_create_grid(void* comm, int nprow, int npcol, char order) noexcept {
  using fn = int (*)(void*, int, int, char);
  static const fn f = mpi_shim_symbol<fn>("dlaf_create_grid", &dlaf_create_grid);
  return f(comm, nprow, npcol, order);
}
char grid_ordering(void* comm, int nprow, int npcol, int myprow, int mypcol) noexcept {
  using fn = char (*)(void*, int, int, int, int);
  static const fn f = mpi_shim_symbol<fn>("grid_ordering", &grid_ordering);
  return f(comm, nprow, npcol, myprow, mypcol);
}
void dlaf_create_grid_from_blacs(int blacs_ctxt) noexcept {
  using fn = void (*)(int);
  static const fn f = mpi_shim_symbol<fn>("dlaf_create_grid_from_blacs", &dlaf_create_grid_from_blacs);
  f(blacs_ctxt);
}

}
```

### dla_future_amd/csrc/host/cholesky.cpp

```cpp
#include "runtime.hpp"

#include <algorithm>
#include <cstdlib>
#include <cstring>
#include <vector>

namespace dlaf_mi355x {

static bool potrf_use_chain() {
  static const bool chain = [] {
    const char* e = std::getenv("DLAF_MI355X_POTRF");
    return e && std::strcmp(e, "chain") == 0;
  }();
  return chain;
}

template <class T>
void potrf_tile(T* t, int ld, int kb, T* winv, int* info, int info_base, unsigned* sync, hipStream_t s) {
  constexpr int JB = kDiagBlock;
  if (!potrf_use_chain()) {
    launch_potrf_coop(t, ld, kb, winv, info, info_base, sync, s,  true,  true);
    return;
  }
  for (int j0 = 0; j0 < kb; j0 += JB) {
    const int jb = std::min(JB, kb - j0);
    T* djj = t + j0 + (size_t) j0 * ld;
    T* wj = winv + (size_t) (j0 / JB) * JB * JB;
    launch_potrf_diag(djj, ld, jb, wj, info, info_base + j0, s);
    const int rem = kb - j0 - jb;
    if (rem <= 0)
      break;
    T* sub = t + (j0 + jb) + (size_t) j0 * ld;
    TrsmArgs<T> ta;
    ta.b = sub;
    ta.b_ts = 0;
    ta.ldb = ld;
    ta.il0 = 0;
    ta.il1 = 1;
    ta.pr = 1;
    ta.ri = 0;
    ta.nb = rem;
    ta.nt = 1;
    ta.last_rows = rem;
    ta.l = djj;
    ta.ldl = ld;
    ta.winv = wj;
    ta.n = jb;
    ta.info = info;
    launch_trsm(ta, s);
    UpdateArgs<T> ua;
    ua.c = t + (j0 + jb) + (size_t) (j0 + jb) * ld;
    ua.c_tsr = ua.c_tsc = 0;
    ua.ldc = ld;
    ua.a = sub;
    ua.a_ts = 0;
    ua.lda = ld;
    ua.b = sub;
    ua.b_ts = 0;
    ua.ldb = ld;
    ua.il0 = ua.jl0 = 0;
    ua.il1 = ua.jl1 = 1;
    ua.nb = rem;
    ua.K = jb;
    ua.pr = ua.pc = 1;
    ua.ri = ua.ci = 0;
    ua.nt = 1;
    ua.last_rows = rem;
    ua.info = info;
    launch_update(ua, s, 2);
  }
}

static long gcd_l(long a, long b) {
  while (b) {
    const long t = a % b;
    a = b;
    b = t;
  }
  return a;
}

template <class T>
int DeviceMatrix<T>::bcast_transposed_panel(Transport* tr, CommAxis ax_col, const T* a_base, long il_n, long jl_n,
                                            T* dst, hipStream_t s, int& period, long& ts2) {
  const size_t tile_bytes = tile_elems * sizeof(T);
  const long ncols = ltc - jl_n;
  const long g = gcd_l(rows.P, cols.P);
  period = (int) (rows.P / g);
  const long lstep = cols.P / g;
  const long cap = ncols > 0 ? (ncols + period - 1) / period : 0;
  ts2 = cap * (long) tile_elems;
  int issued = 0;
  tr->group_begin();
  for (long c = 0; c < period && c < ncols; ++c) {
    const long jl_first = jl_n + c;
    const long gj_first = cols.global_of(jl_first);
    const int root_r = rows.owner(gj_first);
    long cnt = (ncols - c + period - 1) / period;
    if (cols.global_of(jl_first + (cnt - 1) * period) == nt - 1)
      --cnt;
    if (cnt <= 0)
      continue;
    T* d = dst + c * ts2;
    if (rows.rank == root_r) {
      const T* src = a_base + (size_t) (rows.local_of(gj_first) - il_n) * tile_elems;
      DLAF_HIP_CHECK(hipMemcpy2DAsync(d, tile_bytes, src, (size_t) lstep * tile_bytes, tile_bytes, (size_t) cnt,
                                      hipMemcpyDeviceToDevice, s));
    }
    tr->bcast(ax_col, root_r, rows.rank, d, d, (size_t) cnt * tile_bytes, s);
    ++issued;
  }
  tr->group_end();
  return issued;
}

namespace {

enum class Schedule { Pairs, Sidecar, Early, Classic };

Schedule choose_schedule(bool dist, int nb, bool complex_type) {
  const char* e = std::getenv("DLAF_MI355X_SCHEDULE");
  if (e == nullptr) {
    if (dist)
      return Schedule::Early;
    if (nb % 16 == 0)
      return Schedule::Pairs;
    return !complex_type && nb <= 768 ? Schedule::Sidecar : Schedule::Classic;
  }
  if (std::strcmp(e, "early") == 0)
    return Schedule::Early;
  if (!dist && std::strcmp(e, "pairs") == 0)
    return Schedule::Pairs;
  if (!dist && std::strcmp(e, "sidecar") == 0)
    return Schedule::Sidecar;
  return Schedule::Classic;
}

constexpr long kSidecarSlots = 32;

template <class T>
struct PairRates {
  static constexpr bool dbl = sizeof(real_t<T>) == 8;
  static constexpr double r_bulk = dbl ? 66e12 : 118e12;
  static constexpr double r_trsm_slot = (dbl ? 5e12 : 8e12) / 32.0;
  static constexpr double t_potrf_blk2 = 11.3e-6 * (TypeInfo<T>::is_complex ? 2.0 : 1.0);
};

template <class T>
struct Step {
  const T* a_base = nullptr;
  const T* b_base = nullptr;
  long b_ts = 0, il_n = 0, jl_n = 0;
  int b_period = 1;
  long b_ts2 = 0;
  const T* a2_base = nullptr;
  const T* b2_base = nullptr;
  int k1 = 0;
  int kb = 0;
  long rest0 = 0, split = 0;
  bool valid = false;

  static Step one_panel(int kb, long il_n, long jl_n, const T* a_base, size_t tile_elems) {
    Step st;
    st.valid = true;
    st.kb = kb;
    st.il_n = il_n;
    st.jl_n = jl_n;
    st.a_base = st.b_base = a_base;
    st.b_ts = (long) tile_elems;
    return st;
  }
  static Step two_panels(int k1, int k2, long n0, const T* a_base, const T* a2_base, size_t tile_elems) {
    Step st = one_panel(k1 + k2, n0, n0, a_base, tile_elems);
    st.k1 = k1;
    st.a2_base = st.b2_base = a2_base;
    return st;
  }
};

template <class T>
struct CholeskyIssue {
  using StepT = Step<T>;
  DeviceMatrix<T>& m;
  Transport* tr;
  const bool dist;
  const size_t tile_bytes;
  const int last_rows;
  const CommAxis ax_row, ax_col;
  const hipStream_t s_main, s_panel, s_comm;
  long potrf_slots = 0, comm_slots = 0;
  long grid_reserve = 0;
  size_t next_update_slice = 0;

  explicit CholeskyIssue(DeviceMatrix<T>& mat)
      : m(mat), tr(grid_transport(*mat.grid)), dist(mat.grid->nranks > 1), tile_bytes(mat.tile_elems * sizeof(T)),
        last_rows(mat.rows.last_extent()), ax_row(mat.transposed ? CommAxis::Col : CommAxis::Row),
        ax_col(mat.transposed ? CommAxis::Row : CommAxis::Col), s_main(mat.s_low), s_panel(mat.s_high),
        s_comm(mat.s_comm) {
    if (dist && !tr)
      fatal("[dlaf_mi355x] grid with %d ranks has no transport\n", m.grid->nranks);
    if (const char* e = std::getenv("DLAF_MI355X_POTRF_SLOTS"))
      potrf_slots = std::atol(e);
    else
      potrf_slots = potrf_use_chain() ? 0 : 2 * ((m.nb + kDiagBlock - 1) / kDiagBlock);
    if (const char* e = std::getenv("DLAF_MI355X_COMM_SLOTS"))
      comm_slots = std::atol(e);
    else
      comm_slots = (dist && tr->device_side()) ? 32 : 0;
    grid_reserve = potrf_slots + comm_slots;
  }

  StepT one_panel(long k, long il_n, long jl_n, const T* a_base) const {
    return StepT::one_panel(m.rows.tile_extent(k), il_n, jl_n, a_base, m.tile_elems);
  }

  void update_work(long il0, long il1, long j0, long j1, int kb, double& flops, double& bytes) const {
    flops = bytes = 0;
    const double cx = TypeInfo<T>::is_complex ? 4.0 : 1.0;
    for (long jl = j0; jl < j1; ++jl) {
      const long gj = m.cols.global_of(jl);
      const double nj = m.rows.tile_extent(gj);
      for (long il = std::max(il0, m.rows.next_local(gj)); il < il1; ++il) {
        const long gi = m.rows.global_of(il);
        const double mi = m.rows.tile_extent(gi);
        if (gi == gj) {
          flops += cx * mi * (mi + 1) * kb;
          bytes += (mi * kb + mi * mi) * sizeof(T);
        }
        else {
          flops += cx * 2.0 * mi * nj * kb;
          bytes += (mi * kb + nj * kb + 2.0 * mi * nj) * sizeof(T);
        }
      }
    }
  }

  double column_flops(const StepT& st, long jl) const {
    double f, by;
    update_work(std::max(st.il_n, m.rows.next_local(m.cols.global_of(jl))), m.ltr, jl, jl + 1, st.kb, f, by);
    return f;
  }

  void update(const StepT& st, long j0, long j1, hipStream_t s, int role, long reserve, long il_from = -1,
              long il_to = -1, int kind = -1) {
    if (!st.valid || j0 >= j1)
      return;
    const long il0 = std::max(std::max(st.il_n, il_from), m.rows.next_local(m.cols.global_of(j0)));
    const long il1 = il_to < 0 ? m.ltr : std::min(il_to, m.ltr);
    if (il0 >= il1)
      return;
    UpdateArgs<T> ua;
    ua.c = m.tiles;
    ua.c_tsr = (long) m.tile_elems;
    ua.c_tsc = (long) (m.tile_elems * m.ltr);
    ua.ldc = m.nb;
    ua.a = st.a_base + (size_t) (il0 - st.il_n) * m.tile_elems;
    ua.a_ts = (long) m.tile_elems;
    ua.lda = m.nb;
    ua.b = st.b_base;
    ua.b_ts = st.b_ts;
    ua.b_period = st.b_period;
    ua.b_ts2 = st.b_ts2;
    ua.b_jl0 = (int) st.jl_n;
    if (st.k1 > 0) {
      ua.K1 = st.k1;
      ua.a2 = st.a2_base + (size_t) (il0 - st.il_n) * m.tile_elems;
      ua.b2 = st.b2_base;
    }
    ua.ldb = m.nb;
    ua.il0 = (int) il0;
    ua.il1 = (int) il1;
    ua.jl0 = (int) j0;
    ua.jl1 = (int) j1;
    ua.nb = m.nb;
    ua.K = st.kb;
    ua.pr = m.rows.P;
    ua.ri = m.rows.shift();
    ua.pc = m.cols.P;
    ua.ci = m.cols.shift();
    ua.nt = (int) m.nt;
    ua.last_rows = last_rows;
    ua.info = m.info;
    double fl, by;
    update_work(il0, il1, j0, j1, st.kb, fl, by);
    const int pk = kind < 0 ? role : kind;
    m.prof_begin(pk, s);
    unsigned* cnt = m.coop_sync;
    bool zero = false;
    if (reserve > 0) {
      const size_t sl = std::min(next_update_slice, m.coop_sync_update_slices - 1);
      cnt = m.coop_sync + 16 * sl;
      zero = next_update_slice < m.coop_sync_update_slices - 1;
      ++next_update_slice;
    }
    static const bool exclusive = [] {
      const char* e = std::getenv("DLAF_MI355X_EXCLUSIVE_CUS");
      return e ? std::atoi(e) != 0 : true;
    }();
    if (reserve > 0 && exclusive)
      launch_update(ua, s, role, m.bulk_slots, cnt, zero, reserve);
    else
      launch_update(ua, s, role, reserve > 0 ? std::max<long>(8, m.bulk_slots - reserve) : 0, cnt, zero);
    DLAF_HIP_CHECK(hipGetLastError());
    m.prof_end(pk, s, fl, by);
  }

  void trsm(long il0, long il1, long klc, const T* Lkk, const T* Wkk, int kb, hipStream_t ts = nullptr) {
    if (ts == nullptr)
      ts = s_main;
    if (il0 >= il1)
      return;
    TrsmArgs<T> ta;
    ta.b = m.tile(il0, klc);
    ta.b_ts = (long) m.tile_elems;
    ta.ldb = m.nb;
    ta.il0 = (int) il0;
    ta.il1 = (int) il1;
    ta.pr = m.rows.P;
    ta.ri = m.rows.shift();
    ta.nb = m.nb;
    ta.nt = (int) m.nt;
    ta.last_rows = last_rows;
    ta.l = Lkk;
    ta.ldl = m.nb;
    ta.winv = Wkk;
    ta.n = kb;
    ta.info = m.info;
    ta.prio = (ts != s_main) ? 1 : 0;
    double fl = 0, by = 0;
    for (long il = il0; il < il1; ++il) {
      const double mi = m.rows.tile_extent(m.rows.global_of(il));
      fl += (TypeInfo<T>::is_complex ? 4.0 : 1.0) * (double) kb * kb * mi;
      by += (0.5 * kb * kb + 2.0 * mi * kb) * sizeof(T);
    }
    m.prof_begin(2, ts);
    launch_trsm(ta, ts);
    DLAF_HIP_CHECK(hipGetLastError());
    m.prof_end(2, ts, fl, by);
  }

  T* winv_of(long k) const { return m.winv + (size_t) (k & 1) * m.winv_elems(); }
  T* diag_ws_of(long k) const { return m.diag_ws + (size_t) (k & 1) * (m.tile_elems + m.winv_elems()); }
  void potrf(long k) {
    if (m.rows.rank != m.rows.owner(k) || m.cols.rank != m.cols.owner(k))
      return;
    const int kb = m.rows.tile_extent(k);
    const double cxf = TypeInfo<T>::is_complex ? 4.0 : 1.0;
    m.prof_begin(3, s_panel);
    potrf_tile(m.tile(m.rows.local_of(k), m.cols.local_of(k)), m.nb, kb, winv_of(k), m.info, (int) (k * m.nb),
               m.coop_sync + 16 * m.coop_sync_update_slices + m.coop_sync_potrf_words * (size_t) k, s_panel);
    DLAF_HIP_CHECK(hipGetLastError());
    m.prof_end(3, s_panel, cxf * (double) kb * kb * kb / 3.0, (double) kb * kb * sizeof(T));
  }

  void diag_bcast(long k, bool in_row, bool in_col, const T*& Lkk, const T*& Wkk) {
    Lkk = Wkk = nullptr;
    if (in_row && in_col) {
      Lkk = m.tile(m.rows.local_of(k), m.cols.local_of(k));
      Wkk = winv_of(k);
    }
    if (in_col && m.rows.P > 1) {
      T* ws = diag_ws_of(k);
      if (in_row) {
        DLAF_HIP_CHECK(hipMemcpyAsync(ws, Lkk, tile_bytes, hipMemcpyDeviceToDevice, s_panel));
        DLAF_HIP_CHECK(hipMemcpyAsync(ws + m.tile_elems, Wkk, m.winv_elems() * sizeof(T), hipMemcpyDeviceToDevice, s_panel));
      }
      DLAF_HIP_CHECK(hipEventRecord(m.ev_diag[k], s_panel));
      DLAF_HIP_CHECK(hipStreamWaitEvent(s_comm, m.ev_diag[k], 0));
      tr->bcast(ax_col, m.rows.owner(k), m.rows.rank, ws, ws, tile_bytes + m.winv_elems() * sizeof(T), s_comm);
      DLAF_HIP_CHECK(hipEventRecord(m.ev_diag[k], s_comm));
      Lkk = ws;
      Wkk = ws + m.tile_elems;
    }
    else {
      DLAF_HIP_CHECK(hipEventRecord(m.ev_diag[k], s_panel));
    }
  }

  void transposed_panel(StepT& cur, int buf) {
    if (m.rows.P > 1) {
      m.bcast_transposed_panel(tr, ax_col, cur.a_base, cur.il_n, cur.jl_n, m.panelT[buf], s_comm, cur.b_period,
                               cur.b_ts2);
      cur.b_base = m.panelT[buf];
      cur.b_ts = (long) m.tile_elems;
    }
    else {
      cur.b_base = cur.a_base + (m.cols.global_of(cur.jl_n) - cur.il_n) * (long) m.tile_elems;
      cur.b_ts = (long) m.tile_elems * m.cols.P;
    }
  }

  void join_last_diag(long k) {
    DLAF_HIP_CHECK(hipEventRecord(m.ev_diag[k], s_panel));
    DLAF_HIP_CHECK(hipStreamWaitEvent(s_main, m.ev_diag[k], 0));
  }

  void panel_done(long k, hipStream_t s) {
    DLAF_HIP_CHECK(hipEventRecord(m.ev_panel[k], s));
    m.panels_issued.store(k, std::memory_order_release);
  }

  long pair_slots(long k, double bulk_flops) const {
    using R = PairRates<T>;
    const long nb = m.nb, bulk_slots = m.bulk_slots;
    const double cxf = TypeInfo<T>::is_complex ? 4.0 : 1.0;
    const double below = (double) std::max<long>(0, m.n - (k + 1) * nb) + (double) std::max<long>(0, m.n - (k + 2) * nb);
    const double fl_t = cxf * (double) nb * nb * below;
    const double nblk = (double) nb / kDiagBlock;
    const double t_potrf = 2.0 * nblk * nblk * R::t_potrf_blk2;
    auto t_of = [&](long sl) {
      const double share = (double) sl / (double) bulk_slots;
      return std::max(bulk_flops / (R::r_bulk * (1.0 - share)), t_potrf + fl_t / (R::r_trsm_slot * (double) sl));
    };
    long best = kSidecarSlots;
    double best_t = t_of(best);
    if (bulk_flops / (R::r_bulk * (1.0 - (double) best / (double) bulk_slots)) >= best_t)
      return best;
    for (long cand : {48L, 64L, 96L, 128L, 192L, 256L}) {
      if (cand <= kSidecarSlots || cand * 2 > bulk_slots)
        continue;
      const double t = t_of(cand);
      if (t < best_t) {
        best_t = t;
        best = cand;
      }
    }
    return best;
  }

  bool u1_on_main(long k, long slots, double bulk_flops) const {
    using R = PairRates<T>;
    const long nb = m.nb;
    const double cxf = TypeInfo<T>::is_complex ? 4.0 : 1.0;
    const double below1 = (double) std::max<long>(0, m.n - (k + 1) * nb), below2 = (double) std::max<long>(0, m.n - (k + 2) * nb);
    const double fl_chain = cxf * (double) nb * nb * (below1 + below2) + cxf * 2.0 * (double) nb * nb * below1;
    const double nblk = (double) nb / kDiagBlock;
    const double t_chain = 2.0 * nblk * nblk * R::t_potrf_blk2 + fl_chain / (R::r_trsm_slot * (double) slots);
    const double t_bulk = bulk_flops / (R::r_bulk * (1.0 - (double) slots / (double) m.bulk_slots));
    return t_bulk < t_chain;
  }

  void issue_pairs();
  void issue_sidecar();
  void issue_early();
  void issue_classic();
};

template <class T>
void CholeskyIssue<T>::issue_pairs() {
  constexpr double kSplitFrac = 0.3;
  const long nt = m.nt, ltr = m.ltr, ltc = m.ltc;
  StepT prev;
  for (long k = 0; k < nt; k += 2) {
    if (tr)
      tr->mark(k);
    if (k >= 2)
      DLAF_HIP_CHECK(hipStreamWaitEvent(s_panel, m.ev_high[k - 2], 0));
    potrf(k);
    const bool second = k + 1 < nt;
    const bool more = k + 2 < nt;
    if (second) {
      trsm(k + 1, ltr, k, m.tile(k, k), winv_of(k), m.rows.tile_extent(k), s_panel);
      panel_done(k, s_panel);
    }
    const bool bulk = prev.valid && prev.rest0 < ltc;
    std::vector<double> colfl;
    double bulk_flops = 0;
    for (long jl = bulk ? prev.rest0 : ltc; jl < ltc; ++jl) {
      colfl.push_back(column_flops(prev, jl));
      bulk_flops += colfl.back();
    }
    const long slots = bulk ? pair_slots(k, bulk_flops) : kSidecarSlots;
    const bool u1_main = second && (!bulk || u1_on_main(k, slots, bulk_flops));
    long splitA = prev.rest0;
    if (u1_main && bulk) {
      double acc = 0;
      while (splitA < ltc && acc < kSplitFrac * bulk_flops)
        acc += colfl[(size_t) (splitA++ - prev.rest0)];
    }
    update(prev, prev.rest0, splitA, s_main, 0, slots);
    if (second) {
      const StepT u1 = one_panel(k, k + 1, k + 1, m.tile(k + 1 < ltr ? k + 1 : 0, k));
      if (u1_main) {
        DLAF_HIP_CHECK(hipStreamWaitEvent(s_main, m.ev_panel[k], 0));
        update(u1, k + 1, k + 2, s_main, 1, 0);
        DLAF_HIP_CHECK(hipEventRecord(m.ev_head[k], s_main));
        DLAF_HIP_CHECK(hipStreamWaitEvent(s_panel, m.ev_head[k], 0));
      }
      else {
        update(u1, k + 1, k + 2, s_panel, 1, 0);
      }
      potrf(k + 1);
      if (more) {
        trsm(k + 2, ltr, k + 1, m.tile(k + 1, k + 1), winv_of(k + 1), m.rows.tile_extent(k + 1), s_panel);
        panel_done(k + 1, s_panel);
      }
    }
    update(prev, splitA, ltc, s_main, 0, slots);
    if (!more) {
      join_last_diag(k);
      break;
    }
    DLAF_HIP_CHECK(hipStreamWaitEvent(s_main, m.ev_panel[k + 1], 0));
    StepT cur = StepT::two_panels(m.rows.tile_extent(k), m.rows.tile_extent(k + 1), k + 2, m.tile(k + 2, k),
                                  m.tile(k + 2, k + 1), m.tile_elems);
    update(cur, k + 2, std::min<long>(k + 4, ltc), s_main, 1, 0);
    DLAF_HIP_CHECK(hipEventRecord(m.ev_high[k], s_main));
    cur.rest0 = std::min<long>(k + 4, ltc);
    prev = cur;
  }
}

template <class T>
void CholeskyIssue<T>::issue_sidecar() {
  const long nt = m.nt, ltr = m.ltr, ltc = m.ltc;
  StepT prev;
  for (long k = 0; k < nt; ++k) {
    const int kb = m.rows.tile_extent(k);
    if (tr)
      tr->mark(k);
    const long il_n = m.rows.next_local(k + 1), jl_n = m.cols.next_local(k + 1);
    const long klc = m.cols.local_of(k);
    if (k >= 1)
      DLAF_HIP_CHECK(hipStreamWaitEvent(s_panel, m.ev_high[k - 1], 0));
    potrf(k);
    if (k == nt - 1) {
      update(prev, prev.rest0, ltc, s_main, 0, kSidecarSlots);
      join_last_diag(k);
      break;
    }
    trsm(il_n, ltr, klc, m.tile(m.rows.local_of(k), klc), winv_of(k), kb, s_panel);
    panel_done(k, s_panel);
    update(prev, prev.rest0, ltc, s_main, 0, kSidecarSlots);
    DLAF_HIP_CHECK(hipStreamWaitEvent(s_main, m.ev_panel[k], 0));
    StepT cur = one_panel(k, il_n, jl_n, m.tile(il_n < ltr ? il_n : 0, klc));
    transposed_panel(cur, 0);
    cur.rest0 = jl_n;
    if (jl_n < ltc) {
      update(cur, jl_n, jl_n + 1, s_main, 1, 0);
      cur.rest0 = jl_n + 1;
    }
    DLAF_HIP_CHECK(hipEventRecord(m.ev_high[k], s_main));
    prev = cur;
  }
}

template <class T>
void CholeskyIssue<T>::issue_early() {
  const long nt = m.nt, ltr = m.ltr, ltc = m.ltc;
  StepT prev;
  potrf(0);
  for (long k = 0; k < nt; ++k) {
    const int kb = m.rows.tile_extent(k);
    if (tr)
      tr->mark(k);
    const int own_c = m.cols.owner(k);
    const bool in_row = m.rows.rank == m.rows.owner(k), in_col = m.cols.rank == own_c;
    const long il_n = m.rows.next_local(k + 1), jl_n = m.cols.next_local(k + 1);
    const int buf = (int) (k & 1);
    const long klc = in_col ? m.cols.local_of(k) : -1;
    if (k == nt - 1) {
      update(prev, prev.rest0, ltc, s_main, 0, 0);
      join_last_diag(k);
      break;
    }
    const T *Lkk, *Wkk;
    diag_bcast(k, in_row, in_col, Lkk, Wkk);

    const bool head_row = m.rows.rank == m.rows.owner(k + 1);
    const long il_t = il_n + (head_row ? 1 : 0);
    DLAF_HIP_CHECK(hipStreamWaitEvent(s_main, m.ev_diag[k], 0));
    if (in_col && head_row)
      trsm(il_n, il_n + 1, klc, Lkk, Wkk, kb);
    DLAF_HIP_CHECK(hipEventRecord(m.ev_head[k], s_main));
    if (in_col)
      trsm(il_t, ltr, klc, Lkk, Wkk, kb);
    panel_done(k, s_main);

    T* dst = in_col ? m.tile(il_n < ltr ? il_n : 0, klc) : m.panel[buf];
    StepT cur = one_panel(k, il_n, jl_n, dst);
    if (dist)
      DLAF_HIP_CHECK(hipStreamWaitEvent(s_comm, m.ev_head[k], 0));
    if (m.cols.P > 1 && head_row)
      tr->bcast(ax_row, own_c, m.cols.rank, dst, dst, tile_bytes, s_comm);
    if (dist)
      DLAF_HIP_CHECK(hipEventRecord(m.ev_headb[k], s_comm));

    if (head_row && m.cols.rank == m.cols.owner(k + 1)) {
      if (k >= 1)
        DLAF_HIP_CHECK(hipStreamWaitEvent(s_panel, m.ev_high[k - 1], 0));
      DLAF_HIP_CHECK(hipStreamWaitEvent(s_panel, (dist && m.cols.P > 1) ? m.ev_headb[k] : m.ev_head[k], 0));
      update(cur, jl_n, jl_n + 1, s_panel, 2, 0, il_n, il_n + 1, 3);
      potrf(k + 1);
    }

    if (dist)
      DLAF_HIP_CHECK(hipStreamWaitEvent(s_comm, m.ev_panel[k], 0));
    if (m.cols.P > 1 && il_t < ltr)
      tr->bcast(ax_row, own_c, m.cols.rank, dst + (size_t) (il_t - il_n) * m.tile_elems,
                dst + (size_t) (il_t - il_n) * m.tile_elems, (size_t) (ltr - il_t) * tile_bytes, s_comm);
    transposed_panel(cur, buf);
    if (dist)
      DLAF_HIP_CHECK(hipEventRecord(m.ev_bcast[k], s_comm));

    update(prev, prev.rest0, ltc, s_main, 0, grid_reserve);
    if (dist)
      DLAF_HIP_CHECK(hipStreamWaitEvent(s_main, m.ev_bcast[k], 0));

    cur.rest0 = m.cols.next_local(k + 3);
    update(cur, jl_n, cur.rest0, s_main, 1, 0, m.rows.next_local(k + 2));
    DLAF_HIP_CHECK(hipEventRecord(m.ev_high[k], s_main));
    prev = cur;
  }
}

template <class T>
void CholeskyIssue<T>::issue_classic() {
  const double lookahead_flops = 270e-6 * ((double) m.nb / kDiagBlock) * 55e12;
  const long nt = m.nt, ltr = m.ltr, ltc = m.ltc;
  StepT prev;
  for (long k = 0; k < nt; ++k) {
    const int kb = m.rows.tile_extent(k);
    if (tr)
      tr->mark(k);
    const int own_c = m.cols.owner(k);
    const bool in_row = m.rows.rank == m.rows.owner(k), in_col = m.cols.rank == own_c;
    const long il_n = m.rows.next_local(k + 1), jl_n = m.cols.next_local(k + 1);
    const int buf = (int) (k & 1);
    const long klc = in_col ? m.cols.local_of(k) : -1;

    if (k >= 1)
      DLAF_HIP_CHECK(hipStreamWaitEvent(s_panel, m.ev_high[k - 1], 0));
    potrf(k);
    if (k == nt - 1) {
      update(prev, prev.rest0, prev.split, s_main, 0, potrf_slots);
      update(prev, prev.split, ltc, s_main, 0, comm_slots);
      join_last_diag(k);
      break;
    }
    const T *Lkk, *Wkk;
    diag_bcast(k, in_row, in_col, Lkk, Wkk);

    update(prev, prev.rest0, prev.split, s_main, 0, potrf_slots);

    DLAF_HIP_CHECK(hipStreamWaitEvent(s_main, m.ev_diag[k], 0));
    if (in_col)
      trsm(il_n, ltr, klc, Lkk, Wkk, kb);
    panel_done(k, s_main);

    T* dst = in_col ? m.tile(il_n < ltr ? il_n : 0, klc) : m.panel[buf];
    StepT cur = one_panel(k, il_n, jl_n, dst);
    if (dist)
      DLAF_HIP_CHECK(hipStreamWaitEvent(s_comm, m.ev_panel[k], 0));
    if (m.cols.P > 1 && il_n < ltr)
      tr->bcast(ax_row, own_c, m.cols.rank, dst, dst, (size_t) (ltr - il_n) * tile_bytes, s_comm);
    transposed_panel(cur, buf);
    if (dist)
      DLAF_HIP_CHECK(hipEventRecord(m.ev_bcast[k], s_comm));

    update(prev, prev.split, ltc, s_main, 0, comm_slots);
    if (dist)
      DLAF_HIP_CHECK(hipStreamWaitEvent(s_main, m.ev_bcast[k], 0));

    cur.rest0 = jl_n;
    if (m.cols.mine(k + 1) && jl_n < ltc) {
      update(cur, jl_n, jl_n + 1, s_main, 1, 0);
      cur.rest0 = jl_n + 1;
    }
    DLAF_HIP_CHECK(hipEventRecord(m.ev_high[k], s_main));
    cur.split = cur.rest0;
    for (double acc = 0; cur.split < ltc && acc < lookahead_flops; ++cur.split)
      acc += column_flops(cur, cur.split);
    prev = cur;
  }
}

}

template <class T>
void DeviceMatrix<T>::factorize_async() {
  CholeskyIssue<T> f(*this);
  const Schedule schedule = choose_schedule(f.dist, nb, TypeInfo<T>::is_complex);

  for (auto& ps : prof) {
    ps.used = 0;
    ps.flops = ps.bytes = ps.ms = 0;
    ps.launches = 0;
  }
  DLAF_HIP_CHECK(hipMemsetAsync(info, 0, sizeof(int), f.s_panel));
  DLAF_HIP_CHECK(hipMemsetAsync(coop_sync, 0, sizeof(unsigned) * coop_sync_words, f.s_panel));
  if (unsigned long long* tb = potrf_coop_trace_buffer())
    DLAF_HIP_CHECK(hipMemsetAsync(tb, 0, 32 * sizeof(unsigned long long), f.s_panel));
  DLAF_HIP_CHECK(hipEventRecord(ev_start[0], f.s_panel));
  DLAF_HIP_CHECK(hipStreamWaitEvent(f.s_main, ev_start[0], 0));
  DLAF_HIP_CHECK(hipStreamWaitEvent(f.s_comm, ev_start[0], 0));

  switch (schedule) {
    case Schedule::Pairs: f.issue_pairs(); break;
    case Schedule::Sidecar: f.issue_sidecar(); break;
    case Schedule::Early: f.issue_early(); break;
    case Schedule::Classic: f.issue_classic(); break;
  }

  DLAF_HIP_CHECK(hipEventRecord(ev_done[0], f.s_main));
  DLAF_HIP_CHECK(hipStreamWaitEvent(f.s_panel, ev_done[0], 0));
  DLAF_HIP_CHECK(hipMemcpyAsync(info_host, info, sizeof(int), hipMemcpyDeviceToHost, f.s_panel));
}

#define INST(T)                                                                                     \
  template void DeviceMatrix<T>::factorize_async();                                                 \
  template int DeviceMatrix<T>::bcast_transposed_panel(Transport*, CommAxis, const T*, long, long, T*, \
                                                       hipStream_t, int&, long&);                   \
  template void potrf_tile<T>(T*, int, int, T*, int*, int, unsigned*, hipStream_t);
INST(float)
INST(double)
INST(cfloat)
INST(cdouble)
#undef INST

}
```

### dla_future_amd/csrc/host/runtime.cpp

```cpp
#include "runtime.hpp"

#include <cstdarg>
#include <cstdio>
#include <cstdlib>
#include <algorithm>
#include <cstring>
#include <map>
#include <mutex>
#include <exception>
#include <thread>

namespace dlaf_mi355x {

void fatal(const char* fmt, ...) {
  va_list ap;
  va_start(ap, fmt);
  std::vfprintf(stderr, fmt, ap);
  va_end(ap);
  std::fflush(stderr);
  std::terminate();
}

static bool g_initialized = false;

// ... 109 lines not shown
  std::vector<void*> drop;
  {
    std::lock_guard<std::mutex> lk(pl.mu);
    for (auto& kv : pl.idle)
      drop.push_back(kv.second);
    pl.idle.clear();
    pl.idle_bytes = 0;
  }
  for (void* q : drop)
    (void) hipFree(q);
}

size_t pool_idle_bytes() {
  Pool& pl = pool();
  std::lock_guard<std::mutex> lk(pl.mu);
  return pl.idle_bytes;
}

bool runtime_initialized() {
  return g_initialized;
}

namespace {
class HostTransport final : public Transport {
public:
  HostTransport(dlaf_host_bcast_fn b, dlaf_host_barrier_fn bar, void* user) : bcast_(b), barrier_(bar), user_(user) {}
  ~HostTransport() override {
    if (pinned_)
      (void) hipHostFree(pinned_);
  }
  bool device_side() const override { return false; }
  void bcast(CommAxis axis, int root, int my_index, const void* send, void* recv, size_t bytes,
             hipStream_t stream) override {
    if (bytes == 0)
      return;
    reserve(bytes);
    if (my_index == root)
      DLAF_HIP_CHECK(hipMemcpyAsync(pinned_, send, bytes, hipMemcpyDeviceToHost, stream));
    DLAF_HIP_CHECK(hipStreamSynchronize(stream));
    if (bcast_(user_, (int) axis, root, pinned_, bytes) != 0)
      fatal("[dlaf_mi355x] host broadcast callback failed\n");
    DLAF_HIP_CHECK(hipMemcpyAsync(recv, pinned_, bytes, hipMemcpyHostToDevice, stream));
    DLAF_HIP_CHECK(hipStreamSynchronize(stream));
  }
  void barrier(hipStream_t stream) override {
    DLAF_HIP_CHECK(hipStreamSynchronize(stream));
    if (barrier_ && barrier_(user_) != 0)
      fatal("[dlaf_mi355x] host barrier callback failed\n");
  }
  void allreduce_max(double* v, int n, int nprow, int npcol, int myrow, int mycol) override {
    std::vector<double> tmp((size_t) n);
    for (int pass = 0; pass < 2; ++pass) {
      const int members = pass == 0 ? npcol : nprow, me = pass == 0 ? mycol : myrow;
      std::vector<double> best(v, v + n);
      for (int root = 0; root < members; ++root) {
        if (me == root)
          std::copy(v, v + n, tmp.begin());
        if (bcast_(user_, pass, root, tmp.data(), sizeof(double) * (size_t) n) != 0)
          fatal("[dlaf_mi355x] host broadcast callback failed\n");
        for (int i = 0; i < n; ++i)
          best[(size_t) i] = std::max(best[(size_t) i], tmp[(size_t) i]);
      }
      std::copy(best.begin(), best.end(), v);
    }
  }

  void allreduce_sum(void* dev, size_t count, char type, char scope, hipStream_t stream) override {
    if (count == 0)
      return;
    const bool dbl = (type == 'd' || type == 'z');
    const size_t nreal = count * ((type == 'c' || type == 'z') ? 2 : 1);
    const size_t bytes = nreal * (dbl ? sizeof(double) : sizeof(float));
    reserve(2 * bytes);
    DLAF_HIP_CHECK(hipMemcpyAsync(pinned_, dev, bytes, hipMemcpyDeviceToHost, stream));
    DLAF_HIP_CHECK(hipStreamSynchronize(stream));
    char* mine = static_cast<char*>(pinned_);
    char* tmp = mine + bytes;
    std::vector<char> acc(bytes);
    for (int pass = 0; pass < 2; ++pass) {
      if ((pass == 0 && scope == 'C') || (pass == 1 && scope == 'R'))
        continue;
      const int members = pass == 0 ? npcol : nprow, me = pass == 0 ? mycol : myrow;
      if (members <= 1)
        continue;
      for (int root = 0; root < members; ++root) {
        if (me == root)
          std::memcpy(tmp, mine, bytes);
        if (bcast_(user_, pass, root, tmp, bytes) != 0)
          fatal("[dlaf_mi355x] host broadcast callback failed\n");
        if (root == 0)
          std::memcpy(acc.data(), tmp, bytes);
        else if (dbl) {
          double* a = reinterpret_cast<double*>(acc.data());
          const double* t = reinterpret_cast<const double*>(tmp);
          for (size_t i = 0; i < nreal; ++i)
            a[i] += t[i];
        }
        else {
          float* a = reinterpret_cast<float*>(acc.data());
          const float* t = reinterpret_cast<const float*>(tmp);
          for (size_t i = 0; i < nreal; ++i)
            a[i] += t[i];
        }
      }
      std::memcpy(mine, acc.data(), bytes);
    }
    DLAF_HIP_CHECK(hipMemcpyAsync(dev, mine, bytes, hipMemcpyHostToDevice, stream));
    DLAF_HIP_CHECK(hipStreamSynchronize(stream));
  }

private:
  void reserve(size_t bytes) {
    if (bytes <= cap_)
      return;
    if (pinned_)
      DLAF_HIP_CHECK(hipHostFree(pinned_));
    DLAF_HIP_CHECK(hipHostMalloc(&pinned_, bytes, hipHostMallocDefault));
    cap_ = bytes;
  }
  dlaf_host_bcast_fn bcast_;
  dlaf_host_barrier_fn barrier_;
  void* user_;
  void* pinned_ = nullptr;
  size_t cap_ = 0;
};
}

std::unique_ptr<Transport> make_host_transport(dlaf_host_bcast_fn b, dlaf_host_barrier_fn bar, void* user) {
  return std::unique_ptr<Transport>(new HostTransport(b, bar, user));
}

namespace {
class RecordingTransport final : public Transport {
public:
  RecordingTransport(std::unique_ptr<Transport> inner, Grid* g) : inner_(std::move(inner)), g_(g) {}
  bool device_side() const override { return inner_->device_side(); }
  void bcast(CommAxis axis, int root, int my_index, const void* send, void* recv, size_t bytes,
             hipStream_t stream) override {
    if (bytes != 0 && g_->comm_log_on)
      g_->comm_log.push_back({(long) axis, (long) root, (long) bytes, (long) depth_});
    inner_->bcast(axis, root, my_index, send, recv, bytes, stream);
  }
  void group_begin() override {
    ++depth_;
    inner_->group_begin();
  }
  void group_end() override {
    --depth_;
    inner_->group_end();
  }
  void barrier(hipStream_t stream) override {
    if (g_->comm_log_on)
      g_->comm_log.push_back({3, 0, 0, 0});
    inner_->barrier(stream);
  }
  void allreduce_max(double* v, int n, int nprow, int npcol, int myrow, int mycol) override {
    if (g_->comm_log_on)
      g_->comm_log.push_back({4, 0, (long) (n * sizeof(double)), 0});
    inner_->allreduce_max(v, n, nprow, npcol, myrow, mycol);
  }
  void allreduce_sum(void* dev, size_t count, char type, char scope, hipStream_t stream) override {
    if (g_->comm_log_on)
      g_->comm_log.push_back({4, (long) scope, (long) count, 0});
    inner_->nprow = nprow;
    inner_->npcol = npcol;
    inner_->myrow = myrow;
    inner_->mycol = mycol;
    inner_->allreduce_sum(dev, count, type, scope, stream);
  }
  void mark(long step) override {
    if (g_->comm_log_on)
      g_->comm_log.push_back({2, step, 0, 0});
  }
  bool is_recorder() const { return true; }

private:
  std::unique_ptr<Transport> inner_;
  Grid* g_;
  int depth_ = 0;
};
}

std::unique_ptr<Transport> make_callback_transport(dlaf_host_bcast_fn b, dlaf_host_barrier_fn bar, void* user) {
  const char* e = std::getenv("DLAF_MI355X_TRANSPORT");
  if (e && std::strcmp(e, "peer") == 0)
    return make_peer_transport(b, bar, user);
  return make_host_transport(b, bar, user);
}

Transport* grid_transport(Grid& g) {
  if (g.nranks > 1 && !g.transport && g.host_bcast)
    g.transport = make_callback_transport(g.host_bcast, g.host_barrier, g.host_user);
  if (g.transport && g.comm_log_on && dynamic_cast<RecordingTransport*>(g.transport.get()) == nullptr)
    g.transport = std::unique_ptr<Transport>(new RecordingTransport(std::move(g.transport), &g));
  if (g.transport) {
    g.transport->nprow = g.nprow;
    g.transport->npcol = g.npcol;
    g.transport->myrow = g.myrow;
    g.transport->mycol = g.mycol;
  }
  return g.transport.get();
}

template <class T>
static T* dev_alloc(size_t elems) {
  T* p = nullptr;
  if (elems == 0)
    elems = 1;
  if (hipMalloc(reinterpret_cast<void**>(&p), elems * sizeof(T)) != hipSuccess) {
    (void) hipGetLastError();
    pool_release();
    DLAF_HIP_CHECK(hipMalloc(reinterpret_cast<void**>(&p), elems * sizeof(T)));
  }
  return p;
}

static std::vector<hipEvent_t> make_events(size_t n) {
  std::vector<hipEvent_t> v(n);
  for (auto& e : v)
    DLAF_HIP_CHECK(hipEventCreateWithFlags(&e, hipEventDisableTiming));
  return v;
}

template <class T>
void DeviceMatrix<T>::create(Grid* g, char uplo_, long n_, int nb_, int isrc, int jsrc) {
  runtime_init();
  type = TypeInfo<T>::tag;
  grid = g;
  (void) grid_transport(*g);
  uplo = (uplo_ == 'U' || uplo_ == 'u') ? 'U' : 'L';
  transposed = (uplo == 'U');
  n = n_;
  nb = nb_;
  Axis srow{n, nb, g->nprow, g->myrow, isrc};
  Axis scol{n, nb, g->npcol, g->mycol, jsrc};
  rows = transposed ? scol : srow;
  cols = transposed ? srow : scol;
  nt = rows.nt();
  ltr = rows.local_tiles();
  ltc = cols.local_tiles();
  tile_elems = (size_t) nb * nb;

  tiles = dev_alloc<T>((size_t) ltr * ltc * tile_elems);
  winv = dev_alloc<T>(2 * winv_elems());
  const bool dist = g->nranks > 1;
  if (dist) {
    diag_ws = dev_alloc<T>(2 * (tile_elems + winv_elems()));
    for (int b = 0; b < 2; ++b) {
      panel[b] = dev_alloc<T>((size_t) ltr * tile_elems);
      panelT[b] = dev_alloc<T>((size_t) (ltc + rows.P) * tile_elems);
    }
  }
  {
    hipDeviceProp_t prop;
    int dev = 0;
    DLAF_HIP_CHECK(hipGetDevice(&dev));
    DLAF_HIP_CHECK(hipGetDeviceProperties(&prop, dev));
    bulk_slots = (long) prop.multiProcessorCount * update_blocks_per_cu<T>();
  }
  DLAF_HIP_CHECK(hipMalloc(reinterpret_cast<void**>(&info), sizeof(int)));
  DLAF_HIP_CHECK(zero_device_now(info, sizeof(int)));
  {
    const size_t nt_ = (size_t) std::max<long>(1, (n + nb - 1) / nb);
    coop_sync_update_slices = 6 * nt_ + 8;
    coop_sync_potrf_words = potrf_coop_sync_words(nb);
    coop_sync_words = 16 * coop_sync_update_slices + coop_sync_potrf_words * nt_;
  }
  DLAF_HIP_CHECK(hipMalloc(reinterpret_cast<void**>(&coop_sync), sizeof(unsigned) * coop_sync_words));
  DLAF_HIP_CHECK(hipHostMalloc(reinterpret_cast<void**>(&info_host), sizeof(int), hipHostMallocDefault));
  *info_host = 0;

  int lo = 0, hi = 0;
  DLAF_HIP_CHECK(hipDeviceGetStreamPriorityRange(&lo, &hi));
  DLAF_HIP_CHECK(hipStreamCreateWithPriority(&s_high, hipStreamNonBlocking, hi));
  const char* serial = std::getenv("DLAF_MI355X_SERIAL");
  const char* rcu = std::getenv("DLAF_MI355X_RESERVED_CUS");
  const int reserved = rcu ? std::atoi(rcu) : 0;
  if (serial && std::atoi(serial) != 0) {
    s_low = s_high;
  }
  else if (reserved > 0) {
    hipDeviceProp_t prop;
    int dev = 0;
    DLAF_HIP_CHECK(hipGetDevice(&dev));
    DLAF_HIP_CHECK(hipGetDeviceProperties(&prop, dev));
    const int ncu = prop.multiProcessorCount;
    std::vector<uint32_t> mask((size_t) (ncu + 31) / 32, 0u);
    for (int cu = reserved; cu < ncu; ++cu)
      mask[(size_t) cu / 32] |= 1u << (cu % 32);
    DLAF_HIP_CHECK(hipExtStreamCreateWithCUMask(&s_low, (uint32_t) mask.size(), mask.data()));
  }
  else {
    DLAF_HIP_CHECK(hipStreamCreateWithPriority(&s_low, hipStreamNonBlocking, lo));
  }
  DLAF_HIP_CHECK(hipStreamCreateWithPriority(&s_comm, hipStreamNonBlocking, hi));
  const size_t ne = (size_t) (nt > 0 ? nt : 1);
  ev_panel = make_events(ne);
  ev_done = make_events(1);
  ev_high = make_events(ne);
  ev_diag = make_events(ne);
  ev_bcast = make_events(ne);
  ev_head = make_events(ne);
  ev_headb = make_events(ne);
  ev_start = make_events(2);
}

template <class T>
void DeviceMatrix<T>::destroy() {
  if (!tiles)
    return;
  (void) hipDeviceSynchronize();
  for (auto* v : {&ev_panel, &ev_done, &ev_high, &ev_diag, &ev_bcast, &ev_start, &ev_head, &ev_headb}) {
    for (auto e : *v)
      (void) hipEventDestroy(e);
    v->clear();
  }
  for (auto& ps : prof) {
    for (auto e : ps.start)
      (void) hipEventDestroy(e);
    for (auto e : ps.stop)
      (void) hipEventDestroy(e);
    ps.start.clear();
    ps.stop.clear();
  }
  if (s_low != s_high)
    (void) hipStreamDestroy(s_low);
  (void) hipStreamDestroy(s_high);
  (void) hipStreamDestroy(s_comm);
  (void) hipFree(tiles);
  (void) hipFree(winv);
  if (diag_ws)
    (void) hipFree(diag_ws);
  for (int b = 0; b < 2; ++b) {
    if (panel[b])
      (void) hipFree(panel[b]);
    if (panelT[b])
      (void) hipFree(panelT[b]);
  }
  if (staging)
    (void) hipFree(staging);
  (void) hipFree(info);
  (void) hipFree(coop_sync);
  (void) hipHostFree(info_host);
  tiles = nullptr;
}

template <class T>
static LayoutArgs<T> layout_args(const DeviceMatrix<T>& m, T* cm, long ld_cm) {
  LayoutArgs<T> a;
  a.tiles = m.tiles;
  a.cm = cm;
  a.ld_cm = ld_cm;
  a.ltr = (int) m.ltr;
  a.ltc = (int) m.ltc;
  a.nb = m.nb;
  a.rows = m.rows.local_size();
  a.cols = m.cols.local_size();
  a.pr = m.rows.P;
  a.ri = m.rows.shift();
  a.pc = m.cols.P;
  a.ci = m.cols.shift();
  a.transpose = m.transposed ? 1 : 0;
  return a;
}

template <class T>
static void source_extents(const DeviceMatrix<T>& m, long& srows, long& scols) {
  srows = m.transposed ? m.cols.local_size() : m.rows.local_size();
  scols = m.transposed ? m.rows.local_size() : m.cols.local_size();
}

template <class T>
static void ensure_staging(DeviceMatrix<T>& m, size_t elems) {
  if (m.staging && m.staging_elems >= elems)
    return;
  if (m.staging)
    DLAF_HIP_CHECK(hipFree(m.staging));
  m.staging = dev_alloc<T>(elems);
  m.staging_elems = elems;
}

template <class T, class F, class D>
static void for_each_triangle_block(const DeviceMatrix<T>& m, F&& f, D&& diag) {
  long srows, scols;
  source_extents(m, srows, scols);
  const Axis& srow_ax = m.transposed ? m.cols : m.rows;
  const Axis& scol_ax = m.transposed ? m.rows : m.cols;
  const long nlc = scol_ax.local_tiles();
  for (long jl = 0; jl < nlc; ++jl) {
    const long gj = scol_ax.global_of(jl);
    const long col0 = jl * m.nb, ncols = std::min<long>(m.nb, scols - col0);
    long row0, row1;
    if (!m.transposed) {
      row0 = std::min(srow_ax.next_local(gj) * m.nb, srows);
      row1 = srows;
    }
    else {
      row0 = 0;
      row1 = std::min(srow_ax.next_local(gj + 1) * m.nb, srows);
    }
    if (ncols > 0 && row1 > row0)
      f(row0, row1 - row0, col0, ncols);
    if (srow_ax.mine(gj)) {
      const long r0 = srow_ax.local_of(gj) * m.nb;
      diag(r0, col0, std::min<long>(m.nb, srows - r0), ncols);
    }
  }
}

template <class T>
void DeviceMatrix<T>::upload(const T* host, long ld) {
  long srows, scols;
  source_extents(*this, srows, scols);
  if (srows == 0 || scols == 0)
    return;
  const long lds = srows;
  ensure_staging(*this, (size_t) lds * scols);
  for_each_triangle_block(
      *this,
      [&](long r0, long nr, long c0, long nc) {
        DLAF_HIP_CHECK(hipMemcpy2DAsync(staging + r0 + c0 * lds, (size_t) lds * sizeof(T), host + r0 + c0 * ld,
                                        (size_t) ld * sizeof(T), (size_t) nr * sizeof(T), (size_t) nc,
                                        hipMemcpyHostToDevice, s_high));
      },
      [](long, long, long, long) {});
  launch_to_tiles(layout_args(*this, staging, lds), s_high);
  DLAF_HIP_CHECK(hipStreamSynchronize(s_high));
}

template <class T>
void DeviceMatrix<T>::download(T* host, long ld, bool staging_is_current) {
  long srows, scols;
  source_extents(*this, srows, scols);
  if (srows == 0 || scols == 0)
    return;
  const long lds = srows;
  ensure_staging(*this, (size_t) lds * scols);
  if (!staging_is_current) {
    for_each_triangle_block(
        *this, [](long, long, long, long) {},
        [&](long r0, long c0, long nr, long nc) {
          if (nr > 0 && nc > 0)
            DLAF_HIP_CHECK(hipMemcpy2DAsync(staging + r0 + c0 * lds, (size_t) lds * sizeof(T), host + r0 + c0 * ld,
                                            (size_t) ld * sizeof(T), (size_t) nr * sizeof(T), (size_t) nc,
                                            hipMemcpyHostToDevice, s_high));
        });
  }
  launch_from_tiles(layout_args(*this, staging, lds), s_high);
  for_each_triangle_block(
      *this,
      [&](long r0, long nr, long c0, long nc) {
        DLAF_HIP_CHECK(hipMemcpy2DAsync(host + r0 + c0 * ld, (size_t) ld * sizeof(T), staging + r0 + c0 * lds,
                                        (size_t) lds * sizeof(T), (size_t) nr * sizeof(T), (size_t) nc,
                                        hipMemcpyDeviceToHost, s_high));
      },
      [](long, long, long, long) {});
  DLAF_HIP_CHECK(hipStreamSynchronize(s_high));
}

template <class T>
void DeviceMatrix<T>::copy_from(const DeviceMatrix<T>& o) {
  if (o.n != n || o.nb != nb || o.ltr != ltr || o.ltc != ltc || o.transposed != transposed)
    fatal("[dlaf_mi355x] copy_from: matrices differ in shape or distribution\n");
  DLAF_HIP_CHECK(hipMemcpyAsync(tiles, o.tiles, (size_t) ltr * ltc * tile_elems * sizeof(T),
                                hipMemcpyDeviceToDevice, s_high));
  DLAF_HIP_CHECK(hipStreamSynchronize(s_high));
}

template <class T>
void DeviceMatrix<T>::prof_begin(int kind, hipStream_t s) {
  if (!profiling)
    return;
  ProfSlot& p = prof[kind];
  if (p.used == p.start.size()) {
    hipEvent_t a, b;
    DLAF_HIP_CHECK(hipEventCreate(&a));
    DLAF_HIP_CHECK(hipEventCreate(&b));
    p.start.push_back(a);
    p.stop.push_back(b);
  }
  DLAF_HIP_CHECK(hipEventRecord(p.start[p.used], s));
}

template <class T>
void DeviceMatrix<T>::prof_end(int kind, hipStream_t s, double flops, double bytes) {
  if (!profiling)
    return;
  ProfSlot& p = prof[kind];
  DLAF_HIP_CHECK(hipEventRecord(p.stop[p.used], s));
  ++p.used;
  p.flops += flops;
  p.bytes += bytes;
}

int grid_selftest(Grid& g, size_t bytes) {
  runtime_init();
  Transport* tr = grid_transport(g);
  if (!tr)
    return 0;
  const size_t words = std::max<size_t>(1, bytes / sizeof(unsigned));
  unsigned *src = nullptr, *dst = nullptr;
  DLAF_HIP_CHECK(hipMalloc(reinterpret_cast<void**>(&src), words * sizeof(unsigned)));
  DLAF_HIP_CHECK(hipMalloc(reinterpret_cast<void**>(&dst), 2 * words * sizeof(unsigned)));
  std::vector<unsigned> h(words), back(2 * words);
  hipStream_t s = nullptr;
  DLAF_HIP_CHECK(hipStreamCreateWithFlags(&s, hipStreamNonBlocking));
  int bad = 0;
  auto pattern = [&](int axis, int root, int fixed, int form, size_t i) {
    return (unsigned) (0x9E3779B1u * (unsigned) (i + 1)) ^ (unsigned) (axis << 28 | form << 24 | root << 12 | fixed);
  };
  for (int axis = 0; axis < 2; ++axis) {
    const CommAxis ax = axis == 0 ? CommAxis::Row : CommAxis::Col;
    const int members = axis == 0 ? g.npcol : g.nprow;
    const int me = axis == 0 ? g.mycol : g.myrow;
    const int fixed = axis == 0 ? g.myrow : g.mycol;
    for (int root = 0; root < members; ++root) {
      for (int form = 0; form < 3; ++form) {
        for (size_t i = 0; i < words; ++i)
          h[i] = (me == root) ? pattern(axis, root, fixed, form, i) : 0xDEADBEEFu;
        DLAF_HIP_CHECK(hipMemcpyAsync(src, h.data(), words * sizeof(unsigned), hipMemcpyHostToDevice, s));
        DLAF_HIP_CHECK(hipMemsetAsync(dst, 0, 2 * words * sizeof(unsigned), s));
        const void* send = (me == root) ? src : nullptr;
        if (form == 0)
          tr->bcast(ax, root, me, src, src, words * sizeof(unsigned), s);
        else if (form == 1)
          tr->bcast(ax, root, me, send, dst, words * sizeof(unsigned), s);
        else {
          tr->group_begin();
          tr->bcast(ax, root, me, send, dst, words * sizeof(unsigned), s);
          tr->bcast(ax, root, me, send, dst + words, words * sizeof(unsigned), s);
          tr->group_end();
        }
        DLAF_HIP_CHECK(hipMemcpyAsync(back.data(), form == 0 ? src : dst, (form == 2 ? 2 : 1) * words * sizeof(unsigned),
                                      hipMemcpyDeviceToHost, s));
        DLAF_HIP_CHECK(hipStreamSynchronize(s));
        for (size_t i = 0; i < (form == 2 ? 2 : 1) * words; ++i)
          if (back[i] != pattern(axis, root, fixed, form, i % words)) {
            ++bad;
            break;
          }
      }
    }
  }
  tr->barrier(s);
  double v[2] = {(double) (g.myrow * g.npcol + g.mycol), -(double) (g.myrow * g.npcol + g.mycol)};
  tr->allreduce_max(v, 2, g.nprow, g.npcol, g.myrow, g.mycol);
  if (v[0] != (double) (g.nprow * g.npcol - 1) || v[1] != 0.0)
    ++bad;
  DLAF_HIP_CHECK(hipStreamDestroy(s));
  (void) hipFree(src);
  (void) hipFree(dst);
  return bad;
}

template <class T>
void DeviceMatrix<T>::residual_of(DeviceMatrix<T>& L, double* max_diff, double* max_a) {
  if (L.n != n || L.nb != nb || L.ltr != ltr || L.ltc != ltc || L.transposed != transposed)
    fatal("[dlaf_mi355x] residual_of: matrices differ in shape or distribution\n");
  Transport* tr = grid_transport(*grid);
  const bool dist = grid->nranks > 1;
  const CommAxis ax_row = transposed ? CommAxis::Col : CommAxis::Row;
  const CommAxis ax_col = transposed ? CommAxis::Row : CommAxis::Col;
  const size_t tile_bytes = tile_elems * sizeof(T);
  hipStream_t s = s_low;
  double* dnorm = nullptr;
  DLAF_HIP_CHECK(hipMalloc(reinterpret_cast<void**>(&dnorm), 2 * sizeof(double)));
  DLAF_HIP_CHECK(hipMemsetAsync(info, 0, sizeof(int), s));
  launch_max_norm(tiles, (int) ltr, (int) ltc, nb, rows.local_size(), cols.local_size(), rows.P, rows.shift(), cols.P,
                  cols.shift(), dnorm + 1, s);
  launch_zero_upper_diag(L.tiles, (int) ltr, (int) ltc, nb, rows.P, rows.shift(), cols.P, cols.shift(), s);
  DLAF_HIP_CHECK(hipStreamSynchronize(s));
  for (long k = 0; k < nt; ++k) {
    const int kb = rows.tile_extent(k);
    const int own_c = cols.owner(k);
    const bool in_col = cols.rank == own_c;
    const long il_f = rows.next_local(k), jl_f = cols.next_local(k);
    const long klc = in_col ? cols.local_of(k) : -1;
    if (il_f >= ltr && !dist)
      continue;
    const T* a_base;
    const T* b_base;
    long b_ts = (long) tile_elems;
    if (cols.P > 1) {
      T* dst = in_col ? L.tile(il_f < ltr ? il_f : 0, klc) : panel[0];
      if (il_f < ltr)
        tr->bcast(ax_row, own_c, cols.rank, dst, dst, (size_t) (ltr - il_f) * tile_bytes, s);
      a_base = dst;
    }
    else {
      a_base = L.tile(il_f < ltr ? il_f : 0, klc);
    }
    int b_period = 1;
    long b_ts2 = 0;
    if (rows.P > 1) {
      bcast_transposed_panel(tr, ax_col, a_base, il_f, jl_f, panelT[0], s, b_period, b_ts2);
      b_base = panelT[0];
    }
    else {
      b_base = a_base + (cols.global_of(jl_f) - il_f) * (long) tile_elems;
      b_ts = (long) tile_elems * cols.P;
    }
    if (il_f >= ltr || jl_f >= ltc)
      continue;
    const long il0 = std::max(il_f, rows.next_local(cols.global_of(jl_f)));
    if (il0 >= ltr)
      continue;
    UpdateArgs<T> ua;
    ua.c = tiles;
    ua.c_tsr = (long) tile_elems;
    ua.c_tsc = (long) (tile_elems * ltr);
    ua.ldc = nb;
    ua.a = a_base + (size_t) (il0 - il_f) * tile_elems;
    ua.a_ts = (long) tile_elems;
    ua.lda = nb;
    ua.b = b_base;
// ... 446 lines not shown
```

### dla_future_amd/csrc/host/runtime.hpp

```cpp
#pragma once
#include <hip/hip_runtime.h>

#include <atomic>
#include <cstddef>
#include <cstdint>
#include <memory>
#include <vector>

#include "../device/device_api.hpp"
#include "distribution.hpp"

namespace dlaf_mi355x {

[[noreturn]] void fatal(const char* fmt, ...);

#define DLAF_HIP_CHECK(expr)                                                                     \
  do {                                                                                           \
    hipError_t e_ = (expr);                                                                      \
    if (e_ != hipSuccess)                                                                        \
      ::dlaf_mi355x::fatal("[dlaf_mi355x] HIP error %s at %s:%d: %s\n", hipGetErrorName(e_), __FILE__, \
                           __LINE__, #expr);                                                     \
  } while (0)

hipError_t pool_malloc(void** p, size_t bytes);
hipError_t pool_free(void* p);
void pool_release();
size_t pool_idle_bytes();

enum class CommAxis : int { Row = 0, Col = 1 };

typedef int (*dlaf_host_bcast_fn)(void* user, int axis, int root, void* host_buf, size_t bytes);
typedef int (*dlaf_host_barrier_fn)(void* user);

class Transport {
public:
  virtual ~Transport() = default;
  virtual bool device_side() const = 0;
  virtual void bcast(CommAxis axis, int root, int my_index, const void* send, void* recv, size_t bytes,
                     hipStream_t stream) = 0;
  virtual void group_begin() {}
  virtual void group_end() {}
  virtual void barrier(hipStream_t stream) = 0;
  virtual void allreduce_max(double* host_vals, int n, int nprow, int npcol, int myrow, int mycol) = 0;
  virtual void allreduce_sum(void* dev_buf, size_t count, char type, char scope, hipStream_t stream) = 0;
  virtual void mark(long ) {}
  int nprow = 1, npcol = 1, myrow = 0, mycol = 0;
};

struct CommEvent {
  long kind;
  long root;
  long bytes;
  long group;
};

struct Grid {
  int nprow = 1, npcol = 1;
  int myrow = 0, mycol = 0;
  int rank = 0, nranks = 1;
  char order = 'R';
  std::unique_ptr<Transport> transport;
  dlaf_host_bcast_fn host_bcast = nullptr;
  dlaf_host_barrier_fn host_barrier = nullptr;
  void* host_user = nullptr;
  void (*on_free)(void*) = nullptr;
  void* on_free_user = nullptr;
  bool comm_log_on = false;
  std::vector<CommEvent> comm_log;
  ~Grid() {
    transport.reset();
    if (on_free)
      on_free(on_free_user);
  }
};

std::unique_ptr<Transport> make_rccl_transport(const void* unique_id, int nranks, int rank, int nprow,
                                               int npcol, int myrow, int mycol);
void rccl_get_unique_id(void* out128);
Transport* grid_transport(Grid& g);
std::unique_ptr<Transport> make_host_transport(dlaf_host_bcast_fn bcast, dlaf_host_barrier_fn barrier,
                                               void* user);
std::unique_ptr<Transport> make_peer_transport(dlaf_host_bcast_fn bcast, dlaf_host_barrier_fn barrier,
                                               void* user);
std::unique_ptr<Transport> make_callback_transport(dlaf_host_bcast_fn bcast, dlaf_host_barrier_fn barrier,
                                                   void* user);

struct MatrixBase {
  virtual ~MatrixBase() = default;
  char type = 'd';
};

template <class T>
struct DeviceMatrix : MatrixBase {
  Grid* grid = nullptr;
  char uplo = 'L';
  bool transposed = false;
  Axis rows, cols;
  long n = 0;
  int nb = 1;
  long nt = 0;
  long ltr = 0, ltc = 0;
  size_t tile_elems = 0;

  T* tiles = nullptr;
  T* diag_ws = nullptr;
  T* winv = nullptr;
  T* panel[2] = {nullptr, nullptr};
  T* panelT[2] = {nullptr, nullptr};
  T* staging = nullptr;
  size_t staging_elems = 0;
  unsigned* coop_sync = nullptr;
  size_t coop_sync_words = 0, coop_sync_update_slices = 0, coop_sync_potrf_words = 0;
  int* info = nullptr;
  int* info_host = nullptr;

  hipStream_t s_high = nullptr, s_low = nullptr, s_comm = nullptr;
  std::vector<hipEvent_t> ev_panel, ev_high, ev_diag, ev_bcast, ev_head, ev_headb, ev_start, ev_done;

  struct ProfSlot {
    std::vector<hipEvent_t> start, stop;
    size_t used = 0;
    double flops = 0, bytes = 0;
    double ms = 0;
    long launches = 0;
  };
  ProfSlot prof[4];
  long bulk_slots = 0;
  bool profiling = true;
  void prof_begin(int kind, hipStream_t s);
  void prof_end(int kind, hipStream_t s, double flops, double bytes);

  int bcast_transposed_panel(Transport* tr, CommAxis ax_col, const T* a_base, long il_n, long jl_n, T* dst,
                             hipStream_t s, int& period, long& ts2);

  T* tile(long il, long jl) const { return tiles + (size_t) (il + jl * ltr) * tile_elems; }
  size_t winv_elems() const { return (size_t) ((nb + kDiagBlock - 1) / kDiagBlock) * kDiagBlock * kDiagBlock; }

  void create(Grid* g, char uplo_, long n_, int nb_, int isrc, int jsrc);
  void destroy();
  ~DeviceMatrix() override { destroy(); }

  void upload(const T* host, long ld);
  void download(T* host, long ld, bool staging_is_current = false);
  void copy_from(const DeviceMatrix<T>& other);
  void residual_of(DeviceMatrix<T>& factor, double* max_diff, double* max_a);
  int factorize();
  int factorize_and_download(T* host, long ld);
  std::atomic<long> panels_issued{-1};
  void factorize_async();
  int wait();
  int local_info = 0;
  bool fetch_tile(long gi, long gj, T* host, long ld);
  double trsm_profile(int reps, double* flops, double* bytes);
};

template <class T>
void potrf_tile(T* t, int ld, int kb, T* winv, int* info, int info_base, unsigned* sync, hipStream_t s);

template <class T>
int tile_potrf(char uplo, int n, T* a, int lda);
template <class T>
void tile_trsm(char uplo, int m, int n, const T* a, int lda, T* b, int ldb);
template <class T>
void tile_herk(char uplo, int n, int k, const T* a, int lda, T* c, int ldc);
template <class T>
void tile_gemm(char uplo, int m, int n, int k, const T* a, int lda, const T* b, int ldb, T* c, int ldc);

int grid_selftest(Grid& g, size_t bytes);

template <class T>
int triangular_solver_host(Grid* g, char side, char uplo, char op, char diag, T alpha, const T* a, long lda, int a_isrc,
                           int a_jsrc, T* b, long ldb, long m, long n, int nb, int b_isrc, int b_jsrc, int nb_free = 0);

void solver_last_profile(double* ms, double* flops);

MatrixBase* general_matrix_create(Grid* g, char type, long m, long n, int nb, int isrc, int jsrc);
void general_matrix_transfer(MatrixBase* h, void* host, long ld, bool upload);
int triangular_solver_device(char side, char uplo, char op, char diag, const void* alpha, MatrixBase* a, MatrixBase* b);

template <class T>
int gen_to_std_device(DeviceMatrix<T>& a, DeviceMatrix<T>& l);
template <class T>
int gen_to_std_host(Grid* g, char uplo, T* a, long lda, const T* l, long ldl, long n, int nb, int isrc, int jsrc);

void runtime_init();
void runtime_finalize();
bool runtime_initialized();

}
```

### include/dlaf_mi355x/dlaf_mi355x.h

```cpp
#pragma once
#include <stddef.h>

#include <dlaf_c/desc.h>
#include <dlaf_c/utils.h>

DLAF_EXTERN_C int dlaf_mi355x_create_grid_single(void) DLAF_NOEXCEPT;

#define DLAF_MI355X_UNIQUE_ID_BYTES 128
DLAF_EXTERN_C void dlaf_mi355x_rccl_unique_id(void* out_128_bytes) DLAF_NOEXCEPT;
DLAF_EXTERN_C int dlaf_mi355x_create_grid_rccl(const void* unique_id_128_bytes, int nranks, int rank, int nprow,
                                               int npcol, char order) DLAF_NOEXCEPT;

typedef int (*dlaf_mi355x_bcast_fn)(void* user, int axis, int root, void* host_buf, size_t bytes);
typedef int (*dlaf_mi355x_barrier_fn)(void* user);
DLAF_EXTERN_C int dlaf_mi355x_create_grid_host(int nranks, int rank, int nprow, int npcol, char order,
                                               dlaf_mi355x_bcast_fn bcast, dlaf_mi355x_barrier_fn barrier,
                                               void* user) DLAF_NOEXCEPT;

DLAF_EXTERN_C int dlaf_mi355x_grid_host_bcast(int context, int axis, int root, void* host_buf, size_t bytes) DLAF_NOEXCEPT;

DLAF_EXTERN_C int dlaf_mi355x_grid_on_free(int context, void (*fn)(void*), void* user) DLAF_NOEXCEPT;
DLAF_EXTERN_C int dlaf_mi355x_grid_rekey(int ctx, int new_ctx) DLAF_NOEXCEPT;

DLAF_EXTERN_C int dlaf_mi355x_grid_comm_log(int context, int enable) DLAF_NOEXCEPT;
DLAF_EXTERN_C long dlaf_mi355x_grid_comm_log_read(int context, long* out_4_longs_per_event,
                                                  long cap_events) DLAF_NOEXCEPT;

DLAF_EXTERN_C int dlaf_mi355x_grid_info(int context, int* nprow, int* npcol, int* myrow, int* mycol) DLAF_NOEXCEPT;

typedef struct dlaf_mi355x_matrix_s* dlaf_mi355x_matrix_t;

DLAF_EXTERN_C int dlaf_mi355x_matrix_create(int context, char type, char uplo, struct DLAF_descriptor desc,
                                            dlaf_mi355x_matrix_t* out) DLAF_NOEXCEPT;
DLAF_EXTERN_C void dlaf_mi355x_matrix_destroy(dlaf_mi355x_matrix_t m) DLAF_NOEXCEPT;
DLAF_EXTERN_C int dlaf_mi355x_matrix_upload(dlaf_mi355x_matrix_t m, const void* host_local, int ld) DLAF_NOEXCEPT;
DLAF_EXTERN_C int dlaf_mi355x_matrix_download(dlaf_mi355x_matrix_t m, void* host_local, int ld) DLAF_NOEXCEPT;
DLAF_EXTERN_C int dlaf_mi355x_matrix_copy(dlaf_mi355x_matrix_t dst, dlaf_mi355x_matrix_t src) DLAF_NOEXCEPT;
DLAF_EXTERN_C int dlaf_mi355x_matrix_fetch_tile(dlaf_mi355x_matrix_t m, long gi, long gj, void* host,
                                                int ld) DLAF_NOEXCEPT;
DLAF_EXTERN_C int dlaf_mi355x_cholesky_start(dlaf_mi355x_matrix_t m) DLAF_NOEXCEPT;
DLAF_EXTERN_C int dlaf_mi355x_cholesky_wait(dlaf_mi355x_matrix_t m) DLAF_NOEXCEPT;
DLAF_EXTERN_C int dlaf_mi355x_cholesky_factorization_device(dlaf_mi355x_matrix_t m) DLAF_NOEXCEPT;
DLAF_EXTERN_C int dlaf_mi355x_matrix_local_info(dlaf_mi355x_matrix_t m) DLAF_NOEXCEPT;
DLAF_EXTERN_C int dlaf_mi355x_update_launch_stats(long* persistent, long* exclusive) DLAF_NOEXCEPT;
DLAF_EXTERN_C int dlaf_mi355x_potrf_trace(unsigned long long* out_32_words) DLAF_NOEXCEPT;
DLAF_EXTERN_C int dlaf_mi355x_cholesky_residual(dlaf_mi355x_matrix_t original, dlaf_mi355x_matrix_t factor,
                                                double* max_diff, double* max_a) DLAF_NOEXCEPT;
DLAF_EXTERN_C int dlaf_mi355x_matrix_profile(dlaf_mi355x_matrix_t m, int kind, double* ms, long* launches,
                                             double* flops, double* bytes) DLAF_NOEXCEPT;
DLAF_EXTERN_C int dlaf_mi355x_matrix_trsm_profile(dlaf_mi355x_matrix_t m, int reps, double* ms, double* flops,
                                                  double* bytes) DLAF_NOEXCEPT;
DLAF_EXTERN_C int dlaf_mi355x_grid_barrier(int context) DLAF_NOEXCEPT;
DLAF_EXTERN_C int dlaf_mi355x_grid_selftest(int context, size_t bytes) DLAF_NOEXCEPT;

DLAF_EXTERN_C int dlaf_mi355x_triangular_solver_s(int context, char side, char uplo, char op, char diag,
                                                  const float* alpha, const float* a, struct DLAF_descriptor desca,
                                                  float* b, struct DLAF_descriptor descb) DLAF_NOEXCEPT;
DLAF_EXTERN_C int dlaf_mi355x_triangular_solver_d(int context, char side, char uplo, char op, char diag,
                                                  const double* alpha, const double* a, struct DLAF_descriptor desca,
                                                  double* b, struct DLAF_descriptor descb) DLAF_NOEXCEPT;
DLAF_EXTERN_C int dlaf_mi355x_triangular_solver_c(int context, char side, char uplo, char op, char diag,
                                                  const dlaf_complex_c* alpha, const dlaf_complex_c* a,
                                                  struct DLAF_descriptor desca, dlaf_complex_c* b,
                                                  struct DLAF_descriptor descb) DLAF_NOEXCEPT;
DLAF_EXTERN_C int dlaf_mi355x_triangular_solver_z(int context, char side, char uplo, char op, char diag,
                                                  const dlaf_complex_z* alpha, const dlaf_complex_z* a,
                                                  struct DLAF_descriptor desca, dlaf_complex_z* b,
                                                  struct DLAF_descriptor descb) DLAF_NOEXCEPT;
DLAF_EXTERN_C void dlaf_mi355x_pstrsm(char side, char uplo, char op, char diag, int m, int n, const float* alpha,
                                      const float* a, int ia, int ja, const int desca[9], float* b, int ib, int jb,
                                      const int descb[9]) DLAF_NOEXCEPT;
DLAF_EXTERN_C void dlaf_mi355x_pdtrsm(char side, char uplo, char op, char diag, int m, int n, const double* alpha,
                                      const double* a, int ia, int ja, const int desca[9], double* b, int ib, int jb,
                                      const int descb[9]) DLAF_NOEXCEPT;
DLAF_EXTERN_C void dlaf_mi355x_pctrsm(char side, char uplo, char op, char diag, int m, int n,
                                      const dlaf_complex_c* alpha, const dlaf_complex_c* a, int ia, int ja,
                                      const int desca[9], dlaf_complex_c* b, int ib, int jb,
                                      const int descb[9]) DLAF_NOEXCEPT;
DLAF_EXTERN_C void dlaf_mi355x_pztrsm(char side, char uplo, char op, char diag, int m, int n,
                                      const dlaf_complex_z* alpha, const dlaf_complex_z* a, int ia, int ja,
                                      const int desca[9], dlaf_complex_z* b, int ib, int jb,
                                      const int descb[9]) DLAF_NOEXCEPT;

DLAF_EXTERN_C void dlaf_mi355x_pspotrs(char uplo, int n, int nrhs, const float* a, int ia, int ja, const int desca[9],
                                       float* b, int ib, int jb, const int descb[9], int* info) DLAF_NOEXCEPT;
DLAF_EXTERN_C void dlaf_mi355x_pdpotrs(char uplo, int n, int nrhs, const double* a, int ia, int ja, const int desca[9],
                                       double* b, int ib, int jb, const int descb[9], int* info) DLAF_NOEXCEPT;
DLAF_EXTERN_C void dlaf_mi355x_pcpotrs(char uplo, int n, int nrhs, const dlaf_complex_c* a, int ia, int ja,
                                       const int desca[9], dlaf_complex_c* b, int ib, int jb, const int descb[9],
                                       int* info) DLAF_NOEXCEPT;
DLAF_EXTERN_C void dlaf_mi355x_pzpotrs(char uplo, int n, int nrhs, const dlaf_complex_z* a, int ia, int ja,
                                       const int desca[9], dlaf_complex_z* b, int ib, int jb, const int descb[9],
                                       int* info) DLAF_NOEXCEPT;

DLAF_EXTERN_C int dlaf_mi355x_generalized_to_standard_s(int context, char uplo, float* a, struct DLAF_descriptor desca,
                                                        const float* b, struct DLAF_descriptor descb) DLAF_NOEXCEPT;
DLAF_EXTERN_C int dlaf_mi355x_generalized_to_standard_d(int context, char uplo, double* a, struct DLAF_descriptor desca,
                                                        const double* b, struct DLAF_descriptor descb) DLAF_NOEXCEPT;
DLAF_EXTERN_C int dlaf_mi355x_generalized_to_standard_c(int context, char uplo, dlaf_complex_c* a,
                                                        struct DLAF_descriptor desca, const dlaf_complex_c* b,
                                                        struct DLAF_descriptor descb) DLAF_NOEXCEPT;
DLAF_EXTERN_C int dlaf_mi355x_generalized_to_standard_z(int context, char uplo, dlaf_complex_z* a,
                                                        struct DLAF_descriptor desca, const dlaf_complex_z* b,
                                                        struct DLAF_descriptor descb) DLAF_NOEXCEPT;
DLAF_EXTERN_C void dlaf_mi355x_pshegst(int ibtype, char uplo, int n, float* a, int ia, int ja, const int desca[9],
                                       const float* b, int ib, int jb, const int descb[9], float* scale,
                                       int* info) DLAF_NOEXCEPT;
DLAF_EXTERN_C void dlaf_mi355x_pdhegst(int ibtype, char uplo, int n, double* a, int ia, int ja, const int desca[9],
                                       const double* b, int ib, int jb, const int descb[9], double* scale,
                                       int* info) DLAF_NOEXCEPT;
DLAF_EXTERN_C void dlaf_mi355x_pchegst(int ibtype, char uplo, int n, dlaf_complex_c* a, int ia, int ja,
                                       const int desca[9], const dlaf_complex_c* b, int ib, int jb,
                                       const int descb[9], float* scale, int* info) DLAF_NOEXCEPT;
DLAF_EXTERN_C void dlaf_mi355x_pzhegst(int ibtype, char uplo, int n, dlaf_complex_z* a, int ia, int ja,
                                       const int desca[9], const dlaf_complex_z* b, int ib, int jb,
                                       const int descb[9], double* scale, int* info) DLAF_NOEXCEPT;
DLAF_EXTERN_C int dlaf_mi355x_generalized_to_standard_device(dlaf_mi355x_matrix_t a,
                                                             dlaf_mi355x_matrix_t cholesky_factor_of_b) DLAF_NOEXCEPT;

DLAF_EXTERN_C int dlaf_mi355x_reduction_to_band_s(int context, float* a, struct DLAF_descriptor desca, int band_size,
                                                  float* taus) DLAF_NOEXCEPT;
DLAF_EXTERN_C int dlaf_mi355x_reduction_to_band_d(int context, double* a, struct DLAF_descriptor desca, int band_size,
                                                  double* taus) DLAF_NOEXCEPT;
DLAF_EXTERN_C int dlaf_mi355x_reduction_to_band_c(int context, dlaf_complex_c* a, struct DLAF_descriptor desca,
                                                  int band_size, dlaf_complex_c* taus) DLAF_NOEXCEPT;
DLAF_EXTERN_C int dlaf_mi355x_reduction_to_band_z(int context, dlaf_complex_z* a, struct DLAF_descriptor desca,
                                                  int band_size, dlaf_complex_z* taus) DLAF_NOEXCEPT;
DLAF_EXTERN_C int dlaf_mi355x_reduction_to_band_device(dlaf_mi355x_matrix_t a, int band_size, void* taus) DLAF_NOEXCEPT;
DLAF_EXTERN_C int dlaf_mi355x_bt_reduction_to_band_s(int context, int band_size, float* c, struct DLAF_descriptor descc,
                                                     const float* v, struct DLAF_descriptor descv,
                                                     const float* taus) DLAF_NOEXCEPT;
DLAF_EXTERN_C int dlaf_mi355x_bt_reduction_to_band_d(int context, int band_size, double* c, struct DLAF_descriptor descc,
                                                     const double* v, struct DLAF_descriptor descv,
                                                     const double* taus) DLAF_NOEXCEPT;
DLAF_EXTERN_C int dlaf_mi355x_bt_reduction_to_band_c(int context, int band_size, dlaf_complex_c* c,
                                                     struct DLAF_descriptor descc, const dlaf_complex_c* v,
                                                     struct DLAF_descriptor descv, const dlaf_complex_c* taus) DLAF_NOEXCEPT;
DLAF_EXTERN_C int dlaf_mi355x_bt_reduction_to_band_z(int context, int band_size, dlaf_complex_z* c,
                                                     struct DLAF_descriptor descc, const dlaf_complex_z* v,
                                                     struct DLAF_descriptor descv, const dlaf_complex_z* taus) DLAF_NOEXCEPT;
DLAF_EXTERN_C int dlaf_mi355x_red2band_panel_stats(long* blocked, long* fallback) DLAF_NOEXCEPT;
DLAF_EXTERN_C long dlaf_mi355x_workspace_pool_release(void) DLAF_NOEXCEPT;
DLAF_EXTERN_C int dlaf_mi355x_get_eigensolver_min_band(void) DLAF_NOEXCEPT;
DLAF_EXTERN_C void dlaf_mi355x_set_eigensolver_min_band(int b_min) DLAF_NOEXCEPT;
DLAF_EXTERN_C int dlaf_mi355x_get_band_size(int nb) DLAF_NOEXCEPT;
DLAF_EXTERN_C int dlaf_mi355x_red2band_profile(double* ms, double* flops) DLAF_NOEXCEPT;

DLAF_EXTERN_C int dlaf_mi355x_band_to_tridiagonal_s(int context, const float* a, struct DLAF_descriptor desca, int band_size,
                                                  float* d, float* e, float* v, int ldv) DLAF_NOEXCEPT;
DLAF_EXTERN_C int dlaf_mi355x_band_to_tridiagonal_d(int context, const double* a, struct DLAF_descriptor desca, int band_size,
                                                  double* d, double* e, double* v, int ldv) DLAF_NOEXCEPT;
DLAF_EXTERN_C int dlaf_mi355x_band_to_tridiagonal_c(int context, const dlaf_complex_c* a, struct DLAF_descriptor desca, int band_size,
                                                  float* d, float* e, dlaf_complex_c* v, int ldv) DLAF_NOEXCEPT;
DLAF_EXTERN_C int dlaf_mi355x_band_to_tridiagonal_z(int context, const dlaf_complex_z* a, struct DLAF_descriptor desca, int band_size,
                                                  double* d, double* e, dlaf_complex_z* v, int ldv) DLAF_NOEXCEPT;
DLAF_EXTERN_C int dlaf_mi355x_bt_band_to_tridiagonal_s(int band_size, int n, int ncols, const float* v, int ldv, float* e,
                                                     int lde) DLAF_NOEXCEPT;
DLAF_EXTERN_C int dlaf_mi355x_bt_band_to_tridiagonal_d(int band_size, int n, int ncols, const double* v, int ldv, double* e,
                                                     int lde) DLAF_NOEXCEPT;
DLAF_EXTERN_C int dlaf_mi355x_bt_band_to_tridiagonal_c(int band_size, int n, int ncols, const dlaf_complex_c* v, int ldv, dlaf_complex_c* e,
                                                     int lde) DLAF_NOEXCEPT;
DLAF_EXTERN_C int dlaf_mi355x_bt_band_to_tridiagonal_z(int band_size, int n, int ncols, const dlaf_complex_z* v, int ldv, dlaf_complex_z* e,
                                                     int lde) DLAF_NOEXCEPT;
DLAF_EXTERN_C int dlaf_mi355x_tridiagonal_eigensolver_s(int n, int nb, const float* d, const float* e, float* w, float* z,
                                                        int ldz) DLAF_NOEXCEPT;
DLAF_EXTERN_C int dlaf_mi355x_tridiagonal_eigensolver_d(int n, int nb, const double* d, const double* e, double* w,
                                                        double* z, int ldz) DLAF_NOEXCEPT;
DLAF_EXTERN_C int dlaf_mi355x_eigensolver_profile(double ms[5]) DLAF_NOEXCEPT;

typedef struct dlaf_mi355x_gmatrix_s* dlaf_mi355x_gmatrix_t;
DLAF_EXTERN_C int dlaf_mi355x_gmatrix_create(int context, char type, struct DLAF_descriptor desc,
                                             dlaf_mi355x_gmatrix_t* out) DLAF_NOEXCEPT;
DLAF_EXTERN_C void dlaf_mi355x_gmatrix_destroy(dlaf_mi355x_gmatrix_t m) DLAF_NOEXCEPT;
DLAF_EXTERN_C int dlaf_mi355x_gmatrix_upload(dlaf_mi355x_gmatrix_t m, const void* host_local, int ld) DLAF_NOEXCEPT;
DLAF_EXTERN_C int dlaf_mi355x_gmatrix_download(dlaf_mi355x_gmatrix_t m, void* host_local, int ld) DLAF_NOEXCEPT;
DLAF_EXTERN_C int dlaf_mi355x_triangular_solver_device(char side, char uplo, char op, char diag, const void* alpha,
                                                       dlaf_mi355x_matrix_t a, dlaf_mi355x_gmatrix_t b) DLAF_NOEXCEPT;
DLAF_EXTERN_C int dlaf_mi355x_potrs_device(char uplo, dlaf_mi355x_matrix_t factor, dlaf_mi355x_gmatrix_t b) DLAF_NOEXCEPT;
DLAF_EXTERN_C int dlaf_mi355x_bt_reduction_to_band_device(int band_size, dlaf_mi355x_gmatrix_t c, dlaf_mi355x_matrix_t v,
                                                          const void* taus) DLAF_NOEXCEPT;

DLAF_EXTERN_C int dlaf_mi355x_solver_profile(double* ms, double* flops) DLAF_NOEXCEPT;

DLAF_EXTERN_C int dlaf_mi355x_set_random_hpd(int context, char type, void* host_local,
                                             struct DLAF_descriptor desc, int nthreads) DLAF_NOEXCEPT;

DLAF_EXTERN_C int dlaf_mi355x_tile_potrf(char type, char uplo, int n, void* a, int lda) DLAF_NOEXCEPT;
DLAF_EXTERN_C int dlaf_mi355x_tile_trsm(char type, char uplo, int m, int n, const void* a, int lda, void* b,
                                        int ldb) DLAF_NOEXCEPT;
DLAF_EXTERN_C int dlaf_mi355x_tile_herk(char type, char uplo, int n, int k, const void* a, int lda, void* c,
                                        int ldc) DLAF_NOEXCEPT;
DLAF_EXTERN_C int dlaf_mi355x_tile_gemm(char type, char uplo, int m, int n, int k, const void* a, int lda,
                                        const void* b, int ldb, void* c, int ldc) DLAF_NOEXCEPT;

DLAF_EXTERN_C int dlaf_mi355x_dist_owner(long global_tile, int grid_size, int src_rank) DLAF_NOEXCEPT;
DLAF_EXTERN_C long dlaf_mi355x_dist_local_tile(long global_tile, int grid_size, int rank, int src_rank) DLAF_NOEXCEPT;
DLAF_EXTERN_C long dlaf_mi355x_dist_next_local_tile(long global_tile, int grid_size, int rank,
                                                    int src_rank) DLAF_NOEXCEPT;
DLAF_EXTERN_C long dlaf_mi355x_dist_global_tile(long local_tile, int grid_size, int rank, int src_rank) DLAF_NOEXCEPT;
DLAF_EXTERN_C long dlaf_mi355x_dist_local_size(long n, int nb, int grid_size, int rank, int src_rank) DLAF_NOEXCEPT;
DLAF_EXTERN_C long dlaf_mi355x_dist_local_tiles(long n, int nb, int grid_size, int rank, int src_rank) DLAF_NOEXCEPT;

DLAF_EXTERN_C const char* dlaf_mi355x_version(void) DLAF_NOEXCEPT;
```

Before: 69.26.

## Backfill idle panel-stream CUs with trailing-update work via shared counters

Adds a backfill launch of the trailing update on the panel stream (new role 4) that shares the bulk launch's work-queue counters. Idle CU slots reserved for potrf/trsm can then steal update blocks. The issue order in issue_pairs is reworked so update launches are prepared first and backfilled around the panel steps, with a new event per step to order the streams. It also adds device-side tally instrumentation. The risk is contention with the panel critical path and extra synchronisation, and correctness depends on the two launches coordinating through the shared counters.

```diff
diff --git a/dla_future_amd/__init__.py b/dla_future_amd/__init__.py
--- a/dla_future_amd/__init__.py
+++ b/dla_future_amd/__init__.py
@@ -2,7 +2,7 @@
 from .cholesky import (DeviceMatrix, GeneralDeviceMatrix, Grid, cholesky_factorization, finalize, generalized_to_standard,
                        initialize, make_descriptor, potrf_trace, pxhegst, pxpotrf, pxpotrs, pxtrsm, set_random_hermitian_positive_definite, tile_gemm, tile_herk, tile_potrf,
                        tile_trsm, triangular_solver, triangular_solver_device, potrs_device, release_workspace_pool, solver_profile,
-                       update_launch_stats)
+                       update_backfill_launches, update_launch_stats, update_tally, update_tally_read)
 from . import distribution
 from .eigensolver import (band_to_tridiagonal, bt_band_to_tridiagonal, bt_reduction_to_band,
                           bt_reduction_to_band_device, eigensolver_min_band, eigensolver_profile, get_band_size, hermitian_eigensolver,
diff --git a/dla_future_amd/capi.py b/dla_future_amd/capi.py
--- a/dla_future_amd/capi.py
+++ b/dla_future_amd/capi.py
@@ -72,6 +72,9 @@
     "dlaf_mi355x_matrix_local_info": (_i, [_vp]),
     "dlaf_mi355x_potrf_trace": (_i, [C.POINTER(C.c_ulonglong)]),
     "dlaf_mi355x_update_launch_stats": (_i, [C.POINTER(C.c_long), C.POINTER(C.c_long)]),
+    "dlaf_mi355x_update_backfill_launches": (_i, [C.POINTER(C.c_long)]),
+    "dlaf_mi355x_update_tally": (_i, [_i]),
+    "dlaf_mi355x_update_tally_read": (_l, [C.POINTER(C.c_long), _l]),
     "dlaf_mi355x_cholesky_start": (_i, [_vp]),
     "dlaf_mi355x_cholesky_wait": (_i, [_vp]),
     "dlaf_mi355x_cholesky_factorization_device": (_i, [_vp]),
diff --git a/dla_future_amd/cholesky.py b/dla_future_amd/cholesky.py
--- a/dla_future_amd/cholesky.py
+++ b/dla_future_amd/cholesky.py
@@ -235,6 +235,25 @@
     return a.value, b.value
 
 
+def update_backfill_launches() -> int:
+    a = C.c_long(0)
+    lib().dlaf_mi355x_update_backfill_launches(C.byref(a))
+    return a.value
+
+
+def update_tally(enable: bool) -> None:
+    lib().dlaf_mi355x_update_tally(1 if enable else 0)
+
+
+def update_tally_read(max_records: int = 4096):
+    buf = (C.c_long * (5 * max_records))()
+    n = lib().dlaf_mi355x_update_tally_read(buf, max_records)
+    if n < 0:
+        raise RuntimeError("update tally is off")
+    return [dict(items=buf[5 * r], bulk=buf[5 * r + 1], backfill=buf[5 * r + 2], bulk_seen=bool(buf[5 * r + 3]),
+                 backfill_seen=bool(buf[5 * r + 4])) for r in range(min(n, max_records))]
+
+
 class DeviceMatrix:
 
     def __init__(self, grid: Grid, dtype, uplo: str, n: int, nb: int, isrc: int = 0, jsrc: int = 0):
diff --git a/dla_future_amd/csrc/device/device_api.hpp b/dla_future_amd/csrc/device/device_api.hpp
--- a/dla_future_amd/csrc/device/device_api.hpp
+++ b/dla_future_amd/csrc/device/device_api.hpp
@@ -46,6 +46,9 @@
 void launch_update(const UpdateArgs<T>& args, hipStream_t stream, int role = 0, long max_blocks = 0,
                    unsigned* counters = nullptr, bool counters_are_zero = false, long excl_slots = 0);
 template <class T>
+bool launch_update_backfill(const UpdateArgs<T>& args, hipStream_t stream, long max_blocks, unsigned* counters,
+                            long excl_slots, long slots);
+template <class T>
 int update_blocks_per_cu();
 
 template <class T>
@@ -78,7 +81,9 @@
 template <class T>
 void launch_potrf_coop(T* tile, int ld, int kb, T* winv, int* info, int info_base, unsigned* sync,
                        hipStream_t stream, bool sync_is_zero = false, bool count_strips = true);
-void update_launch_stats(long* persistent, long* exclusive);
+void update_launch_stats(long* persistent, long* exclusive, long* backfill = nullptr);
+void update_tally_enable(bool on);
+long update_tally_read(long* out, long max_records);
 unsigned long long* potrf_coop_trace_buffer();
 inline size_t potrf_coop_sync_words(int kb) {
   const size_t g = (size_t) ((kb + kDiagBlock - 1) / kDiagBlock);
diff --git a/dla_future_amd/csrc/device/kernels_update.hip b/dla_future_amd/csrc/device/kernels_update.hip
--- a/dla_future_amd/csrc/device/kernels_update.hip
+++ b/dla_future_amd/csrc/device/kernels_update.hip
@@ -66,6 +66,7 @@
   unsigned excl_budget;
   int steal;
   int* cu_busy;
+  unsigned* tally;
 };
 
 __device__ unsigned char g_cu_rank[8][256];
@@ -405,6 +406,8 @@
   __shared__ int next_s0;
   const int nslab = p.K / UpdateCfg<T>::type::BK;
   int q = q0, tried = 1;
+  constexpr bool kBulk = ROLE == 0 || ROLE == 4;
+  unsigned taken = 0;
   int* my_busy = nullptr;
   if (mp.cu_busy != nullptr && threadIdx.x == 0) {
     unsigned xcc;
@@ -431,8 +434,11 @@
 #endif
     __syncthreads();
     if (i >= per_q) {
-      if (!mp.steal || tried >= nq)
+      if (!mp.steal || tried >= nq) {
+        if (mp.tally != nullptr && threadIdx.x == 0 && taken > 0)
+          atomicAdd(&mp.tally[ROLE == 4 ? 1 : 0], taken);
         break;
+      }
       ++tried;
       q = (q + 1) % nq;
       continue;
@@ -446,10 +452,11 @@
       }
       __syncthreads();
     }
+    ++taken;
 #ifdef DLAF_UPD_LEAN
-    update_block<T, VEC, ROLE == 0, (ROLE == 0 ? 1 : 0)>(p, mp, (long) q * per_q + i, lds, s0);
+    update_block<T, VEC, kBulk, (kBulk ? 1 : 0)>(p, mp, (long) q * per_q + i, lds, s0);
 #else
-    update_block<T, VEC, ROLE == 0>(p, mp, (long) q * per_q + i, lds, s0);
+    update_block<T, VEC, kBulk>(p, mp, (long) q * per_q + i, lds, s0);
 #endif
     if (mp.lockstep && threadIdx.x == 0)
       __hip_atomic_fetch_add(&mp.counters[8 + q], 1u, __ATOMIC_RELAXED, __HIP_MEMORY_SCOPE_AGENT);
@@ -513,10 +520,77 @@
 
 static int g_probe_xcds = 0, g_probe_cus_per_xcd = 0, g_probe_engines = 1;
 
-static long g_launch_stats[2] = {0, 0};
-void update_launch_stats(long* persistent, long* exclusive) {
+static long g_launch_stats[3] = {0, 0, 0};
+void update_launch_stats(long* persistent, long* exclusive, long* backfill) {
   *persistent = g_launch_stats[0];
   *exclusive = g_launch_stats[1];
+  if (backfill)
+    *backfill = g_launch_stats[2];
+}
+
+namespace {
+struct TallyRecord {
+  const unsigned* counters;
+  long total;
+  bool bulk, backfill;
+};
+constexpr long kTallyRecords = 4096;
+unsigned* g_tally = nullptr;
+std::vector<TallyRecord> g_tally_rec;
+bool g_tally_on = false;
+}
+
+void update_tally_enable(bool on) {
+  g_tally_on = false;
+  g_tally_rec.clear();
+  if (!on)
+    return;
+  if (g_tally == nullptr && hipMalloc(reinterpret_cast<void**>(&g_tally), 2 * kTallyRecords * sizeof(unsigned)) != hipSuccess) {
+    (void) hipGetLastError();
+    g_tally = nullptr;
+    return;
+  }
+  if (zero_device_now(g_tally, 2 * kTallyRecords * sizeof(unsigned)) != hipSuccess) {
+    (void) hipGetLastError();
+    return;
+  }
+  g_tally_on = true;
+}
+
+long update_tally_read(long* out, long max_records) {
+  if (!g_tally_on)
+    return -1;
+  std::vector<unsigned> t(2 * g_tally_rec.size());
+  if (hipDeviceSynchronize() != hipSuccess ||
+      (!t.empty() && hipMemcpy(t.data(), g_tally, t.size() * sizeof(unsigned), hipMemcpyDeviceToHost) != hipSuccess)) {
+    (void) hipGetLastError();
+    return -1;
+  }
+  const long n = std::min<long>(max_records, (long) g_tally_rec.size());
+  for (long r = 0; r < n; ++r) {
+    out[5 * r + 0] = g_tally_rec[r].total;
+    out[5 * r + 1] = t[2 * r];
+    out[5 * r + 2] = t[2 * r + 1];
+    out[5 * r + 3] = g_tally_rec[r].bulk ? 1 : 0;
+    out[5 * r + 4] = g_tally_rec[r].backfill ? 1 : 0;
+  }
+  return (long) g_tally_rec.size();
+}
+
+static unsigned* tally_slot(const unsigned* counters, long total, bool backfill) {
+  if (!g_tally_on)
+    return nullptr;
+  for (size_t r = g_tally_rec.size(); r-- > 0;) {
+    TallyRecord& rec = g_tally_rec[r];
+    if (rec.counters == counters && (backfill ? !rec.backfill : !rec.bulk) && rec.total == total) {
+      (backfill ? rec.backfill : rec.bulk) = true;
+      return g_tally + 2 * r;
+    }
+  }
+  if ((long) g_tally_rec.size() >= kTallyRecords)
+    return nullptr;
+  g_tally_rec.push_back(TallyRecord{counters, total, !backfill, backfill});
+  return g_tally + 2 * (g_tally_rec.size() - 1);
 }
 
 static bool update_steal() {
@@ -528,12 +602,11 @@
 }
 
 template <class T>
-void launch_update(const UpdateArgs<T>& a, hipStream_t stream, int role, long max_blocks, unsigned* counters,
-                   bool counters_are_zero, long excl_slots) {
+static bool update_map(const UpdateArgs<T>& a, int role, long max_blocks, unsigned* counters, long excl_slots,
+                       UpdateMap& mp, long& grid) {
   using Cfg = typename UpdateCfg<T>::type;
   if (a.il1 <= a.il0 || a.jl1 <= a.jl0 || a.K <= 0 || a.nb <= 0)
-    return;
-  UpdateMap mp;
+    return false;
   mp.bpt_m = (a.nb + Cfg::BM - 1) / Cfg::BM;
   mp.bpt_n = (a.nb + Cfg::BN - 1) / Cfg::BN;
   mp.RB = (a.il1 - a.il0) * mp.bpt_m;
@@ -567,11 +640,11 @@
     }
     npatch = mp.colstart[mp.PC];
     if (npatch == 0)
-      return;
+      return false;
   }
   mp.total = npatch << (mp.ps + mp.psc);
   mp.xcd = (mp.ps > 0) ? 1 : 0;
-  long grid = mp.total;
+  grid = mp.total;
   mp.persist = 0;
   mp.lockstep = 0;
   mp.kphase_ticks = 0;
@@ -579,6 +652,8 @@
   mp.excl_rank = 0;
   mp.excl_budget = 0;
   mp.steal = 0;
+  mp.cu_busy = nullptr;
+  mp.tally = nullptr;
   long excl_rank = 0;
   if (excl_slots > 0) {
     static const int per_cu = update_blocks_per_cu<T>();
@@ -601,15 +676,17 @@
     mp.kphase_ticks = kphase_ticks<T>((int) (grid));
     mp.steal = (update_steal() && !mp.lockstep) ? 1 : 0;
     mp.cu_busy = (role == 0) ? g_cu_busy : nullptr;
-    ++g_launch_stats[0];
     if (excl_rank > 0) {
       mp.excl_rank = (int) excl_rank;
       mp.excl_budget = (unsigned) excl_slots;
-      ++g_launch_stats[1];
-    }
-    if (!counters_are_zero)
-      (void) hipMemsetAsync(counters, 0, 16 * sizeof(unsigned), stream);
-  }
+    }
+  }
+  return true;
+}
+
+template <class T>
+static void update_go(const UpdateArgs<T>& a, const UpdateMap& mp, long grid, hipStream_t stream, int role) {
+  using Cfg = typename UpdateCfg<T>::type;
   const bool vec = aligned16<T>(a.a, a.lda) && aligned16<T>(a.a, a.a_ts) && aligned16<T>(a.b, a.ldb) &&
                    aligned16<T>(a.b, a.b_ts) && aligned16<T>(a.b, a.b_ts2) &&
                    (a.K1 == 0 || (aligned16<T>(a.a2, 0) && aligned16<T>(a.b2, 0)));
@@ -623,6 +700,7 @@
       case 0: go(vtag, std::integral_constant<int, 0>{}); break;
       case 1: go(vtag, std::integral_constant<int, 1>{}); break;
       case 3: go(vtag, std::integral_constant<int, 3>{}); break;
+      case 4: go(vtag, std::integral_constant<int, 4>{}); break;
       default: go(vtag, std::integral_constant<int, 2>{}); break;
     }
   };
@@ -630,6 +708,41 @@
     by_role(std::true_type{});
   else
     by_role(std::false_type{});
+}
+
+template <class T>
+void launch_update(const UpdateArgs<T>& a, hipStream_t stream, int role, long max_blocks, unsigned* counters,
+                   bool counters_are_zero, long excl_slots) {
+  UpdateMap mp;
+  long grid = 0;
+  if (!update_map(a, role, max_blocks, counters, excl_slots, mp, grid))
+    return;
+  if (mp.persist) {
+    ++g_launch_stats[0];
+    if (mp.excl_rank > 0)
+      ++g_launch_stats[1];
+    if (!counters_are_zero)
+      (void) hipMemsetAsync(counters, 0, 16 * sizeof(unsigned), stream);
+    if (role == 0 && !mp.lockstep)
+      mp.tally = tally_slot(counters, mp.total, false);
+  }
+  update_go(a, mp, grid, stream, role);
+}
+
+template <class T>
+bool launch_update_backfill(const UpdateArgs<T>& a, hipStream_t stream, long max_blocks, unsigned* counters,
+                            long excl_slots, long slots) {
+  UpdateMap mp;
+  long grid = 0;
+  if (slots <= 0 || !update_map(a, 0, max_blocks, counters, excl_slots, mp, grid) || !mp.persist || mp.lockstep)
+    return false;
+  grid = mp.xcd ? std::max<long>(8, (slots / 8) * 8) : slots;
+  mp.excl_rank = 0;
+  mp.excl_budget = 0;
+  mp.tally = tally_slot(counters, mp.total, true);
+  ++g_launch_stats[2];
+  update_go(a, mp, grid, stream, 4);
+  return true;
 }
 
 template <class T>
@@ -652,10 +765,12 @@
   SET_ONE(true, 1);
   SET_ONE(true, 2);
   SET_ONE(true, 3);
+  SET_ONE(true, 4);
   SET_ONE(false, 0);
   SET_ONE(false, 1);
   SET_ONE(false, 2);
   SET_ONE(false, 3);
+  SET_ONE(false, 4);
 #undef SET_ONE
 }
 
@@ -754,11 +869,15 @@
 
 template void launch_update<float>(const UpdateArgs<float>&, hipStream_t, int, long, unsigned*, bool, long);
 template int update_blocks_per_cu<float>();
+template bool launch_update_backfill<float>(const UpdateArgs<float>&, hipStream_t, long, unsigned*, long, long);
 template void launch_update<double>(const UpdateArgs<double>&, hipStream_t, int, long, unsigned*, bool, long);
 template int update_blocks_per_cu<double>();
+template bool launch_update_backfill<double>(const UpdateArgs<double>&, hipStream_t, long, unsigned*, long, long);
 template void launch_update<cfloat>(const UpdateArgs<cfloat>&, hipStream_t, int, long, unsigned*, bool, long);
 template int update_blocks_per_cu<cfloat>();
+template bool launch_update_backfill<cfloat>(const UpdateArgs<cfloat>&, hipStream_t, long, unsigned*, long, long);
 template void launch_update<cdouble>(const UpdateArgs<cdouble>&, hipStream_t, int, long, unsigned*, bool, long);
 template int update_blocks_per_cu<cdouble>();
-
-}
+template bool launch_update_backfill<cdouble>(const UpdateArgs<cdouble>&, hipStream_t, long, unsigned*, long, long);
+
+}
diff --git a/dla_future_amd/csrc/host/c_api.cpp b/dla_future_amd/csrc/host/c_api.cpp
--- a/dla_future_amd/csrc/host/c_api.cpp
+++ b/dla_future_amd/csrc/host/c_api.cpp
@@ -899,6 +899,20 @@
     *exclusive = b;
   return 0;
 }
+int dlaf_mi355x_update_backfill_launches(long* backfill) noexcept {
+  long a = 0, b = 0, c = 0;
+  update_launch_stats(&a, &b, &c);
+  if (backfill)
+    *backfill = c;
+  return 0;
+}
+int dlaf_mi355x_update_tally(int enable) noexcept {
+  update_tally_enable(enable != 0);
+  return 0;
+}
+long dlaf_mi355x_update_tally_read(long* out, long max_records) noexcept {
+  return update_tally_read(out, max_records);
+}
 int dlaf_mi355x_potrf_trace(unsigned long long* out) noexcept {
   unsigned long long* tb = potrf_coop_trace_buffer();
   if (tb == nullptr || out == nullptr)
diff --git a/dla_future_amd/csrc/host/cholesky.cpp b/dla_future_amd/csrc/host/cholesky.cpp
--- a/dla_future_amd/csrc/host/cholesky.cpp
+++ b/dla_future_amd/csrc/host/cholesky.cpp
@@ -191,6 +191,7 @@
   long potrf_slots = 0, comm_slots = 0;
   long grid_reserve = 0;
   size_t next_update_slice = 0;
+  int backfill_mode = 1;
 
   explicit CholeskyIssue(DeviceMatrix<T>& mat)
       : m(mat), tr(grid_transport(*mat.grid)), dist(mat.grid->nranks > 1), tile_bytes(mat.tile_elems * sizeof(T)),
@@ -208,6 +209,8 @@
     else
       comm_slots = (dist && tr->device_side()) ? 32 : 0;
     grid_reserve = potrf_slots + comm_slots;
+    if (const char* e = std::getenv("DLAF_MI355X_BACKFILL"))
+      backfill_mode = std::atoi(e);
   }
 
   StepT one_panel(long k, long il_n, long jl_n, const T* a_base) const {
@@ -241,15 +244,32 @@
     return f;
   }
 
+  struct UpdateLaunch {
+    bool valid = false;
+    UpdateArgs<T> ua;
+    hipStream_t s = nullptr;
+    int role = 0, pk = 0;
+    long max_blocks = 0, excl = 0;
+    unsigned* cnt = nullptr;
+    bool own_slice = false;
+    double fl = 0, by = 0;
+  };
+
   void update(const StepT& st, long j0, long j1, hipStream_t s, int role, long reserve, long il_from = -1,
               long il_to = -1, int kind = -1) {
+    issue(prepare(st, j0, j1, s, role, reserve, il_from, il_to, kind));
+  }
+
+  UpdateLaunch prepare(const StepT& st, long j0, long j1, hipStream_t s, int role, long reserve, long il_from = -1,
+                       long il_to = -1, int kind = -1) {
+    UpdateLaunch L;
     if (!st.valid || j0 >= j1)
-      return;
+      return L;
     const long il0 = std::max(std::max(st.il_n, il_from), m.rows.next_local(m.cols.global_of(j0)));
     const long il1 = il_to < 0 ? m.ltr : std::min(il_to, m.ltr);
     if (il0 >= il1)
-      return;
-    UpdateArgs<T> ua;
+      return L;
+    UpdateArgs<T>& ua = L.ua;
     ua.c = m.tiles;
     ua.c_tsr = (long) m.tile_elems;
     ua.c_tsc = (long) (m.tile_elems * m.ltr);
@@ -281,28 +301,46 @@
     ua.nt = (int) m.nt;
     ua.last_rows = last_rows;
     ua.info = m.info;
-    double fl, by;
-    update_work(il0, il1, j0, j1, st.kb, fl, by);
-    const int pk = kind < 0 ? role : kind;
-    m.prof_begin(pk, s);
-    unsigned* cnt = m.coop_sync;
-    bool zero = false;
+    update_work(il0, il1, j0, j1, st.kb, L.fl, L.by);
+    L.valid = true;
+    L.s = s;
+    L.role = role;
+    L.pk = kind < 0 ? role : kind;
+    L.cnt = m.coop_sync;
     if (reserve > 0) {
       const size_t sl = std::min(next_update_slice, m.coop_sync_update_slices - 1);
-      cnt = m.coop_sync + 16 * sl;
-      zero = next_update_slice < m.coop_sync_update_slices - 1;
+      L.cnt = m.coop_sync + 16 * sl;
+      L.own_slice = next_update_slice < m.coop_sync_update_slices - 1;
       ++next_update_slice;
     }
     static const bool exclusive = [] {
       const char* e = std::getenv("DLAF_MI355X_EXCLUSIVE_CUS");
       return e ? std::atoi(e) != 0 : true;
     }();
-    if (reserve > 0 && exclusive)
-      launch_update(ua, s, role, m.bulk_slots, cnt, zero, reserve);
-    else
-      launch_update(ua, s, role, reserve > 0 ? std::max<long>(8, m.bulk_slots - reserve) : 0, cnt, zero);
+    if (reserve > 0 && exclusive) {
+      L.max_blocks = m.bulk_slots;
+      L.excl = reserve;
+    }
+    else {
+      L.max_blocks = reserve > 0 ? std::max<long>(8, m.bulk_slots - reserve) : 0;
+    }
+    return L;
+  }
+
+  void issue(const UpdateLaunch& L) {
+    if (!L.valid)
+      return;
+    m.prof_begin(L.pk, L.s);
+    launch_update(L.ua, L.s, L.role, L.max_blocks, L.cnt, L.own_slice, L.excl);
     DLAF_HIP_CHECK(hipGetLastError());
-    m.prof_end(pk, s, fl, by);
+    m.prof_end(L.pk, L.s, L.fl, L.by);
+  }
+
+  void backfill(const UpdateLaunch& L, long slots) {
+    if (backfill_mode == 0 || !L.valid || !L.own_slice || L.max_blocks <= 0)
+      return;
+    launch_update_backfill(L.ua, s_panel, L.max_blocks, L.cnt, L.excl, slots);
+    DLAF_HIP_CHECK(hipGetLastError());
   }
 
   void trsm(long il0, long il1, long klc, const T* Lkk, const T* Wkk, int kb, hipStream_t ts = nullptr) {
@@ -449,6 +487,7 @@
 template <class T>
 void CholeskyIssue<T>::issue_pairs() {
   constexpr double kSplitFrac = 0.3;
+  constexpr bool cx = TypeInfo<T>::is_complex;
   const long nt = m.nt, ltr = m.ltr, ltc = m.ltc;
   StepT prev;
   for (long k = 0; k < nt; k += 2) {
@@ -456,13 +495,8 @@
       tr->mark(k);
     if (k >= 2)
       DLAF_HIP_CHECK(hipStreamWaitEvent(s_panel, m.ev_high[k - 2], 0));
-    potrf(k);
     const bool second = k + 1 < nt;
     const bool more = k + 2 < nt;
-    if (second) {
-      trsm(k + 1, ltr, k, m.tile(k, k), winv_of(k), m.rows.tile_extent(k), s_panel);
-      panel_done(k, s_panel);
-    }
     const bool bulk = prev.valid && prev.rest0 < ltc;
     std::vector<double> colfl;
     double bulk_flops = 0;
@@ -478,7 +512,17 @@
       while (splitA < ltc && acc < kSplitFrac * bulk_flops)
         acc += colfl[(size_t) (splitA++ - prev.rest0)];
     }
-    update(prev, prev.rest0, splitA, s_main, 0, slots);
+    const UpdateLaunch restA = prepare(prev, prev.rest0, splitA, s_main, 0, slots);
+    const UpdateLaunch restB = prepare(prev, splitA, ltc, s_main, 0, slots);
+    const bool late = backfill_mode == 2;
+    potrf(k);
+    if (cx && !late)
+      backfill(restA.valid ? restA : restB, slots);
+    if (second) {
+      trsm(k + 1, ltr, k, m.tile(k, k), winv_of(k), m.rows.tile_extent(k), s_panel);
+      panel_done(k, s_panel);
+    }
+    issue(restA);
     if (second) {
       const StepT u1 = one_panel(k, k + 1, k + 1, m.tile(k + 1 < ltr ? k + 1 : 0, k));
       if (u1_main) {
@@ -491,17 +535,27 @@
         update(u1, k + 1, k + 2, s_panel, 1, 0);
       }
       potrf(k + 1);
+      if (cx && restA.valid && !late)
+        backfill(restB, slots);
       if (more) {
         trsm(k + 2, ltr, k + 1, m.tile(k + 1, k + 1), winv_of(k + 1), m.rows.tile_extent(k + 1), s_panel);
         panel_done(k + 1, s_panel);
       }
     }
-    update(prev, splitA, ltc, s_main, 0, slots);
+    if (!cx && !late)
+      backfill(restB, slots);
+    issue(restB);
+    if (late && restB.valid) {
+      DLAF_HIP_CHECK(hipEventRecord(m.ev_fill[k], s_main));
+      DLAF_HIP_CHECK(hipStreamWaitEvent(s_panel, m.ev_fill[k], 0));
+      backfill(restB, slots);
+    }
     if (!more) {
       join_last_diag(k);
       break;
     }
-    DLAF_HIP_CHECK(hipStreamWaitEvent(s_main, m.ev_panel[k + 1], 0));
+    DLAF_HIP_CHECK(hipEventRecord(m.ev_fill[k], s_panel));
+    DLAF_HIP_CHECK(hipStreamWaitEvent(s_main, m.ev_fill[k], 0));
     StepT cur = StepT::two_panels(m.rows.tile_extent(k), m.rows.tile_extent(k + 1), k + 2, m.tile(k + 2, k),
                                   m.tile(k + 2, k + 1), m.tile_elems);
     update(cur, k + 2, std::min<long>(k + 4, ltc), s_main, 1, 0);
diff --git a/dla_future_amd/csrc/host/runtime.cpp b/dla_future_amd/csrc/host/runtime.cpp
--- a/dla_future_amd/csrc/host/runtime.cpp
+++ b/dla_future_amd/csrc/host/runtime.cpp
@@ -435,6 +435,7 @@
   ev_bcast = make_events(ne);
   ev_head = make_events(ne);
   ev_headb = make_events(ne);
+  ev_fill = make_events(ne);
   ev_start = make_events(2);
 }
 
@@ -443,7 +444,7 @@
   if (!tiles)
     return;
   (void) hipDeviceSynchronize();
-  for (auto* v : {&ev_panel, &ev_done, &ev_high, &ev_diag, &ev_bcast, &ev_start, &ev_head, &ev_headb}) {
+  for (auto* v : {&ev_panel, &ev_done, &ev_high, &ev_diag, &ev_bcast, &ev_start, &ev_head, &ev_headb, &ev_fill}) {
     for (auto e : *v)
       (void) hipEventDestroy(e);
     v->clear();
diff --git a/dla_future_amd/csrc/host/runtime.hpp b/dla_future_amd/csrc/host/runtime.hpp
--- a/dla_future_amd/csrc/host/runtime.hpp
+++ b/dla_future_amd/csrc/host/runtime.hpp
@@ -115,7 +115,7 @@
   int* info_host = nullptr;
 
   hipStream_t s_high = nullptr, s_low = nullptr, s_comm = nullptr;
-  std::vector<hipEvent_t> ev_panel, ev_high, ev_diag, ev_bcast, ev_head, ev_headb, ev_start, ev_done;
+  std::vector<hipEvent_t> ev_panel, ev_high, ev_diag, ev_bcast, ev_head, ev_headb, ev_fill, ev_start, ev_done;
 
   struct ProfSlot {
     std::vector<hipEvent_t> start, stop;
diff --git a/include/dlaf_mi355x/dlaf_mi355x.h b/include/dlaf_mi355x/dlaf_mi355x.h
--- a/include/dlaf_mi355x/dlaf_mi355x.h
+++ b/include/dlaf_mi355x/dlaf_mi355x.h
@@ -43,6 +43,9 @@
 DLAF_EXTERN_C int dlaf_mi355x_cholesky_factorization_device(dlaf_mi355x_matrix_t m) DLAF_NOEXCEPT;
 DLAF_EXTERN_C int dlaf_mi355x_matrix_local_info(dlaf_mi355x_matrix_t m) DLAF_NOEXCEPT;
 DLAF_EXTERN_C int dlaf_mi355x_update_launch_stats(long* persistent, long* exclusive) DLAF_NOEXCEPT;
+DLAF_EXTERN_C int dlaf_mi355x_update_backfill_launches(long* backfill) DLAF_NOEXCEPT;
+DLAF_EXTERN_C int dlaf_mi355x_update_tally(int enable) DLAF_NOEXCEPT;
+DLAF_EXTERN_C long dlaf_mi355x_update_tally_read(long* out, long max_records) DLAF_NOEXCEPT;
 DLAF_EXTERN_C int dlaf_mi355x_potrf_trace(unsigned long long* out_32_words) DLAF_NOEXCEPT;
 DLAF_EXTERN_C int dlaf_mi355x_cholesky_residual(dlaf_mi355x_matrix_t original, dlaf_mi355x_matrix_t factor,
                                                 double* max_diff, double* max_a) DLAF_NOEXCEPT;
```

Result: no change. 69.53, median of 6 (+0.4%).
